# achinastone/Tensorium

Hardware: AMD Instinct MI355X
Metric: fp32 SGEMM GFLOP/s (M=N=K=4096) + YOLOv3 conv-fwd images/s (higher is better)
Workload: dtype fp32; 1 GPU; sgemm_nn_4096x4096x4096; M=4096, N=4096, K=4096, parallelism=1 independent replicas, one process per GPU, no data-path collective

## Files before the change

### include/tns.h

```cpp
#ifndef TNS_H
#define TNS_H

#include <stdint.h>
#include <stddef.h>

#ifdef __cplusplus
extern "C" {
#endif

#define TNS_ABI_VERSION 1

enum { TNS_CblasRowMajor = 101, TNS_CblasColMajor = 102 };
enum { TNS_CblasNoTrans = 111, TNS_CblasTrans = 112 };

enum {
  TNS_acLOGISTIC = 0, TNS_acRELU = 1, TNS_acRELU6 = 2, TNS_acRELIE = 3,
  TNS_acLINEAR = 4, TNS_acRAMP = 5, TNS_acTANH = 6, TNS_acPLSE = 7,
  TNS_acREVLEAKY = 8, TNS_acLEAKY = 9, TNS_acELU = 10, TNS_acLOGGY = 11,
  TNS_acSTAIR = 12, TNS_acHARDTAN = 13, TNS_acLHTAN = 14, TNS_acSELU = 15
};

enum {
  TNS_OK = 0,
  TNS_ERR_ARG = 1,
// ... 128 lines not shown
                       int64_t n, float* biases, float* bias_updates, float* scales,
                       float* scale_updates, float lrOverBatch, float negDecayTimesBatch,
                       float momentum);
int tns_hip_fill(tns_ctx* ctx, int64_t N, float* x, int64_t offset, float val, int64_t stride);
int tns_hip_copy(tns_ctx* ctx, int64_t N, const float* src, int64_t srcOffset, int64_t inca,
                 float* dst, int64_t dstOffset, int64_t incb);
int tns_hip_clamp(tns_ctx* ctx, int64_t N, float alpha, const float* src, float* dst,
                  int64_t stride, int64_t offset);
int tns_hip_addvv(tns_ctx* ctx, int64_t N, const float* src1, int64_t src1Offset, int64_t inca,
                  const float* src2, int64_t src2Offset, int64_t incb, float* dst,
                  int64_t dstOffset, int64_t incc);
int tns_hip_subvv(tns_ctx* ctx, int64_t N, const float* src1, int64_t src1Offset, int64_t inca,
                  const float* src2, int64_t src2Offset, int64_t incb, float* dst,
                  int64_t dstOffset, int64_t incc);
int tns_hip_mulvv(tns_ctx* ctx, int64_t N, const float* src1, int64_t src1Offset, int64_t inca,
                  const float* src2, int64_t src2Offset, int64_t incb, float* dst,
                  int64_t dstOffset, int64_t incc);
int tns_hip_fmavv(tns_ctx* ctx, int64_t N, const float* src1, int64_t src1Offset, int64_t inca,
                  const float* src2, int64_t src2Offset, int64_t incb, const float* src3,
                  int64_t src3Offset, int64_t incc, float* dst, int64_t dstOffset,
                  int64_t incd);
int tns_hip_fmavss(tns_ctx* ctx, int64_t N, const float* src, int64_t offset, float scalar,
                   float bias, float* dst);
int tns_hip_inverse_sqrt(tns_ctx* ctx, int64_t N, float alpha, const float* src, float* dst,
                         int64_t stride, int64_t offset);

int tns_hip_shortcut(tns_ctx* ctx, int64_t N, const float* a, int64_t aOffset, const float* b,
                     int64_t bOffset, float* out, int64_t outOffset, int32_t activation);
int tns_hip_upsample(tns_ctx* ctx, int64_t aBatch, int64_t aChannels, int64_t outHeight,
                     int64_t outWidth, float* in, int64_t stride, int32_t isForward, float scale,
                     float* out, int32_t zeroIn);
int tns_hip_yolo_forward(tns_ctx* ctx, int64_t batch, int64_t anchors, int64_t classes,
                         int64_t hw, const float* in, float* out);
int tns_hip_yolo_loss(tns_ctx* ctx, int64_t batch, int64_t anchors, int64_t classes, int64_t h,
                      int64_t w, int64_t total, const int64_t* mask, const float* biases,
                      int64_t maxBoxes, int64_t netW, int64_t netH, float ignoreThresh,
                      float truthThresh, float iouThresh, float iouNormalizer,
                      float objNormalizer, float* output, const float* truth, float* delta,
                      float* cost, float* stats, int64_t* counters);
int tns_hip_yolo_detections(tns_ctx* ctx, int64_t batch, int64_t anchors, int64_t classes,
                            int64_t h, int64_t w, int64_t total, const int64_t* mask,
                            const float* biases, int64_t netW, int64_t netH, int64_t imW,
                            int64_t imH, float thresh, int32_t relative, int32_t letter,
                            const float* output, int64_t capacity, int64_t* counts, float* boxes,
                            float* objectness, float* probs);
int tns_hip_nms_sort(tns_ctx* ctx, int64_t batch, int64_t capacity, int64_t classes,
                     const int64_t* counts, const float* boxes, const float* objectness,
                     float* probs, float thresh);

int tns_image_bytes_to_input(tns_ctx* ctx, int64_t count, const uint8_t* src, const int64_t* geom,
                             int64_t channels, int64_t pixelStride, int32_t tableKind,
                             const float* table, int64_t netW, int64_t netH, int32_t letter,
                             float* dst, int64_t* placed);
int tns_image_floats_to_input(tns_ctx* ctx, int64_t count, const float* src, const int64_t* geom,
                              int64_t channels, int64_t netW, int64_t netH, int32_t letter,
                              float* dst, int64_t* placed);

int tns_hip_maxpool_forward(tns_ctx* ctx, int64_t aBatch, int64_t outC, int64_t outH,
                            int64_t outW, const float* input, int64_t c, int64_t h, int64_t w,
                            int64_t stride_x, int64_t stride_y, int64_t padding,
                            int64_t kernelSize, int64_t* indexes, float* output);
int tns_hip_maxpool_backward(tns_ctx* ctx, int64_t aBatch, int64_t outC, int64_t outH,
                             int64_t outW, float* output, const int64_t* indexes,
                             const float* delta, int64_t h, int64_t w, int64_t stride_x,
                             int64_t stride_y, int64_t padding, int64_t kernelSize);
int tns_hip_avgpool_forward(tns_ctx* ctx, int64_t aBatch, int64_t outC, int64_t outH,
                            int64_t outW, const float* input, int64_t c, int64_t h, int64_t w,
                            int64_t stride_x, int64_t stride_y, int64_t padding,
                            int64_t kernelSize, float* output);
int tns_hip_avgpool_backward(tns_ctx* ctx, int64_t aBatch, int64_t outC, int64_t outH,
                             int64_t outW, float* output, const float* delta, int64_t h,
                             int64_t w, int64_t stride_x, int64_t stride_y, int64_t padding,
                             int64_t kernelSize);

int tns_hip_dropout_forward(tns_ctx* ctx, int64_t N, int64_t seed, float probability,
                            float scale, const float* src, float* rnd, float* dst);
int tns_hip_dropout_backward(tns_ctx* ctx, int64_t N, float probability, float scale,
                             const float* src, const float* rnd, float* dst);
int tns_hip_cost_l2(tns_ctx* ctx, int64_t N, const float* pred, const float* truth,
                    float* delta, float* error);
int tns_hip_cross_entropy_logistic(tns_ctx* ctx, int64_t N, const float* pred,
                                   const float* truth, float* delta, float* error);

int tns_hip_lstm_gates_forward(tns_ctx* ctx, int64_t N, const float* wf, const float* wi,
                               const float* wg, const float* wo, const float* uf,
                               const float* ui, const float* ug, const float* uo,
                               float* c_state, float* h_state, float* cell_slice,
                               float* out_slice);
int tns_hip_lstm_gates_backward(tns_ctx* ctx, int64_t N, const float* wf, const float* wi,
                                const float* wg, const float* wo, const float* uf,
                                const float* ui, const float* ug, const float* uo,
                                const float* cell_i, const float* cprev, const float* delta_i,
                                float* dc, float* dwf, float* dwi, float* dwg, float* dwo,
                                float* duf, float* dui, float* dug, float* duo);

int tns_hip_rnn_state_forward(tns_ctx* ctx, int64_t N, int64_t H, float* in_slice,
                              const float* in_bias, int32_t in_act, float* self_slice,
                              const float* self_bias, int32_t self_act,
                              const float* state_prev, float* state_next);
int tns_hip_rnn_delta_backward(tns_ctx* ctx, int64_t N, float* delta, const float* out,
                               int32_t act, float* delta2, const float* out2, int32_t act2);

int tns_hip_means_and_vars(tns_ctx* ctx, int64_t srcSize, int64_t dstSize, int64_t groups,
                           const float* src, int64_t offset, float* means, float* vars);
int tns_hip_means(tns_ctx* ctx, int64_t srcSize, int64_t dstSize, int64_t groups,
                  const float* src, int64_t offset, float* means);
int tns_hip_variances(tns_ctx* ctx, int64_t srcSize, int64_t dstSize, int64_t groups,
                      const float* src, int64_t offset, const float* means, float* vars);
int tns_hip_normalize(tns_ctx* ctx, int64_t srcSize, int64_t dstSize, int64_t groups,
                      const float* means, int64_t meansStride, const float* vars,
                      int64_t varsStride, float* dst, int64_t dstOffset);
int tns_hip_forward_scale(tns_ctx* ctx, int64_t dstSize, float* dst, int64_t offset,
                          int64_t scaleSize, const float* scale, int64_t incb, int64_t batch);
int tns_hip_forward_scale_add(tns_ctx* ctx, int64_t dstSize, float* dst, int64_t offset,
                              int64_t scaleSize, const float* scales, const float* biases,
                              int64_t incb, int64_t batch);
int tns_hip_means_and_vars_delta(tns_ctx* ctx, int64_t srcSize, int64_t dstSize, int64_t groups,
                                 const float* delta, const float* x, int64_t offset,
                                 const float* mean, const float* variance, float* mean_delta,
                                 float* variance_delta);
int tns_hip_normalize_delta(tns_ctx* ctx, int64_t deltaSize, int64_t meanSize, int64_t groups,
                            float* delta, const float* x, int64_t offset, const float* mean,
                            const float* variance, const float* mean_delta,
                            const float* variance_delta);
int tns_hip_add_dots(tns_ctx* ctx, int64_t N, int64_t dstSize, int64_t groups,
                     const float* src1, const float* src2, int64_t srcOffset, float* dst);
int tns_hip_softmax_batch(tns_ctx* ctx, int64_t N, const float* input, int64_t iOffset,
                          int64_t batch, int64_t batch_size, int64_t groups, int64_t group_size,
                          int64_t stride, float temp, float* output, int64_t oOffset);
int tns_hip_cross_entropy_softmax(tns_ctx* ctx, int64_t N, const float* pred, const float* truth,
                                  float* delta, float* error);
int tns_hip_sum(tns_ctx* ctx, int64_t N, const float* src, int64_t offset, float* out);

int64_t tns_mlp_buffer_floats(int32_t nlayers, const int64_t* widths, int32_t bn, int64_t batch);
int tns_hip_mlp_train_step(tns_ctx* ctx, int32_t nlayers, const int64_t* widths,
                           const int32_t* acts, int32_t bn, int64_t batch, const float* X,
                           const float* truth, float learningRate, float momentum, float decay,
                           float* buf, float* cost);


int tns_hip_conv2d(tns_ctx* ctx, int64_t batch, int64_t C, int64_t H, int64_t W,
                   const float* input, const float* weights, int64_t filters,
                   int64_t kH, int64_t kW, int64_t wPadding, int64_t hPadding,
                   int64_t xStride, int64_t yStride, int64_t xDilation, int64_t yDilation,
                   float* workspace, float* out);

enum { TNS_CONV_UNFUSED = 0, TNS_CONV_FUSED = 1, TNS_CONV_IM2COL = 2, TNS_CONV_IMPLICIT = 3 };
int tns_hip_conv_forward(tns_ctx* ctx, int64_t batch, int64_t C, int64_t H, int64_t W,
                         const float* input, const float* weights, const float* biases,
                         int64_t filters, int64_t kSize, int64_t stride, int64_t padding,
                         int64_t dilation, int32_t activation, float* workspace,
                         float* out, int32_t fused);

int tns_hip_conv_forward_train(tns_ctx* ctx, int64_t batch, int64_t C, int64_t H, int64_t W,
                               const float* input, const float* weights, int64_t filters,
                               int64_t kSize, int64_t stride, int64_t padding, int64_t dilation,
                               int32_t activation, const float* scales, const float* biases,
                               float* rolling_mean, float* rolling_variance, float bnMomentum,
                               int32_t training, float* mean, float* variance, float* x,
                               float* x_norm, float* workspace, float* out);

int tns_hip_conv_backward(tns_ctx* ctx, int64_t batch, int64_t C, int64_t H, int64_t W,
                          const float* input, const float* weights, int64_t filters,
                          int64_t kSize, int64_t stride, int64_t padding, int64_t dilation,
                          int32_t activation, const float* output, float* delta,
                          float* bias_updates, float* weight_updates, float* workspace,
                          float* state_delta);
int tns_hip_conv_backward_bn(tns_ctx* ctx, int64_t batch, int64_t C, int64_t H, int64_t W,
                             const float* input, const float* weights, int64_t filters,
                             int64_t kSize, int64_t stride, int64_t padding, int64_t dilation,
                             int32_t activation, const float* output, float* delta,
                             const float* scales, const float* x, const float* x_norm,
                             const float* mean, const float* variance, float* scale_updates,
                             float* mean_delta, float* variance_delta, float* weight_updates,
                             float* workspace, float* state_delta);

int tns_hip_sgemm_strided_batched_multi(const int32_t* devices, int32_t n, uint8_t transA,
                                        uint8_t transB, int64_t M, int64_t N, int64_t K,
                                        float alpha, const float* A, int64_t lda,
                                        int64_t strideA, const float* B, int64_t ldb,
                                        int64_t strideB, float beta, float* C, int64_t ldc,
                                        int64_t strideC, int64_t batchCount);
int tns_set_op_devices(const int32_t* devices, int32_t n);

int    tns_hip_set_telemetry(tns_ctx* ctx, int32_t enable);
double tns_hip_op_ms(tns_ctx* ctx, int32_t op);
enum { TNS_OP_GEMM = 0, TNS_OP_IM2COL = 1, TNS_OP_COL2IM = 2, TNS_OP_BIAS = 3,
       TNS_OP_ACTIVATE = 4, TNS_OP_COUNT = 5 };

int         tns_gemm_variant_count(void);
int         tns_conv_dx_tile_count(void);
int         tns_conv_dx_conv_count(void);
int         tns_conv_dw_res_count(void);
int         tns_conv_dw_tile_count(void);
int         tns_conv_tile_variant_count(void);
const char* tns_conv_tile_variant_name(int32_t variant);
int         tns_conv_slab_count(void);
const char* tns_conv_slab_name(int32_t variant);
int         tns_conv1x1_count(void);
const char* tns_conv1x1_name(int32_t variant);
int         tns_sdot_chains_variant_count(void);
const char* tns_sdot_chains_variant_name(int32_t variant);
int         tns_sdot_rc_variant_count(void);
const char* tns_sdot_rc_variant_name(int32_t variant);
const char* tns_gemm_variant_name(int32_t variant);
int tns_hip_gemm_variant(tns_ctx* ctx, int32_t variant, uint8_t transA, uint8_t transB,
                         int64_t M, int64_t N, int64_t K, float ALPHA,
                         const float* A, int64_t aOffset, int64_t lda, int64_t strideA,
                         const float* B, int64_t bOffset, int64_t ldb, int64_t strideB,
                         float BETA, float* C, int64_t cOffset, int64_t ldc, int64_t strideC,
                         int64_t batchCount);
enum { TNS_GP_TRANS_A = 0, TNS_GP_TRANS_B = 1, TNS_GP_M = 2, TNS_GP_N = 3, TNS_GP_K = 4,
       TNS_GP_LDA = 5, TNS_GP_LDB = 6, TNS_GP_LDC = 7, TNS_GP_STRIDE_A = 8, TNS_GP_STRIDE_B = 9,
       TNS_GP_STRIDE_C = 10, TNS_GP_BATCH = 11, TNS_GP_ALPHA_IS_ONE = 12, TNS_GP_BETA_MODE = 13,
       TNS_GP_EPI = 14, TNS_GP_A_ALIGNED16 = 15, TNS_GP_B_ALIGNED16 = 16, TNS_GP_NT_SDOT = 17,
       TNS_GP_TT_EXACT = 18, TNS_GP_SDOT_FORM = 19, TNS_GP_COUNT = 20 };
int         tns_gemm_plan(int32_t variant, const int64_t* in, char* out, int64_t out_len);
int         tns_gemm_plan_leaf_count(void);
const char* tns_gemm_plan_leaf_name(int32_t leaf);

enum { TNS_OPT_STRICT_BETA0 = 0, TNS_OPT_CONV_VARIANT = 1, TNS_OPT_CONV_PAD = 2,
       TNS_OPT_NT_SDOT = 3, TNS_OPT_SRSS_QUIRK = 4, TNS_OPT_TT_EXACT = 5,
       TNS_OPT_SDOT_FORM = 6, TNS_OPT_DX_FUSED = 7, TNS_OPT_DX_TILE = 8,
       TNS_OPT_DW_TILE = 9, TNS_OPT_BWD_OVERLAP = 10, TNS_OPT_DX_CONV = 11,
       TNS_OPT_DW_RES = 12, TNS_OPT_DERIVE_SUMS = 13, TNS_OPT_SCRATCH_CAP = 14 };
int tns_set_option(int32_t opt, int64_t value);

#ifdef __cplusplus
}
#endif
#endif
```

### tensorium_amd/_abi.py

```python
from __future__ import annotations

import ctypes as C
import os
import re
from pathlib import Path

PKG = Path(__file__).resolve().parent
ROOT = PKG.parent
LIB_PATH = PKG / "libtensorium_hip.so"
HEADER = ROOT / "include" / "tns.h"

i32, i64, u8, f32 = C.c_int32, C.c_int64, C.c_uint8, C.c_float
fptr = C.c_void_p
vp = C.c_void_p

CblasRowMajor, CblasColMajor = 101, 102
CblasNoTrans, CblasTrans = 111, 112
ACT = dict(LOGISTIC=0, RELU=1, RELU6=2, RELIE=3, LINEAR=4, RAMP=5, TANH=6, PLSE=7,
           REVLEAKY=8, LEAKY=9, ELU=10, LOGGY=11, STAIR=12, HARDTAN=13, LHTAN=14, SELU=15)
TNS_OK = 0
TNS_OP_GEMM, TNS_OP_IM2COL, TNS_OP_COL2IM, TNS_OP_BIAS, TNS_OP_ACTIVATE = range(5)
TNS_OPT_STRICT_BETA0 = 0
TNS_OPT_CONV_VARIANT, TNS_OPT_CONV_PAD, TNS_OPT_NT_SDOT, TNS_OPT_SRSS_QUIRK = 1, 2, 3, 4
TNS_OPT_TT_EXACT = 5
TNS_OPT_SDOT_FORM = 6
TNS_OPT_DX_FUSED = 7
TNS_OPT_DX_TILE = 8
TNS_OPT_DW_TILE = 9
TNS_OPT_BWD_OVERLAP = 10
TNS_OPT_DX_CONV = 11
TNS_OPT_DW_RES = 12
TNS_OPT_DERIVE_SUMS = 13
TNS_OPT_SCRATCH_CAP = 14

_CONV = [i64] * 11

PROTOTYPES: dict[str, tuple] = {
    "tns_abi_version": (C.c_int, []),
    "tns_last_error": (C.c_char_p, []),
    "tns_clear_error": (None, []),
    "tns_set_error_hook": (None, [vp]),
    "tns_device_count": (C.c_int, []),
    "tns_set_option": (C.c_int, [i32, i64]),
    "tns_cblas_sgemm": (None, [i32, i32, i32, i64, i64, i64, f32, fptr, i64, fptr, i64, f32,
                               fptr, i64]),
    "tns_cblas_sgemm_batch_strided": (None, [i32, i32, i32, i64, i64, i64, f32, fptr, i64, i64,
                                             fptr, i64, i64, f32, fptr, i64, i64, i64]),
    "tns_im2col": (None, [*_CONV, fptr, i64, fptr, i64, u8]),
    "tns_col2im": (None, [*_CONV, fptr, i64, fptr, i64, i64, u8]),
    "tns_im2col_strided_batched": (None, [*_CONV, fptr, i64, i64, fptr, i64, i64, i64]),
    "tns_col2im_strided_batched": (None, [*_CONV, fptr, i64, i64, fptr, i64, i64, i64]),
    "tns_hip_create": (C.c_int, [i32, C.POINTER(vp)]),
    "tns_hip_destroy": (C.c_int, [vp]),
    "tns_hip_set_stream": (C.c_int, [vp, vp]),
    "tns_hip_get_stream": (vp, [vp]),
    "tns_hip_pending_dw": (C.c_int, [vp]),
    "tns_hip_finish": (C.c_int, [vp]),
    "tns_hip_malloc": (C.c_int, [vp, i64, C.POINTER(vp)]),
    "tns_hip_free": (C.c_int, [vp, vp]),
    "tns_hip_write_buffer": (C.c_int, [vp, fptr, i64, vp]),
    "tns_hip_read_buffer": (C.c_int, [vp, fptr, i64, vp]),
    "tns_hip_gemm": (C.c_int, [vp, u8, u8, i64, i64, i64, f32, fptr, i64, i64, fptr, i64, i64,
                               f32, fptr, i64, i64]),
    "tns_hip_gemm_strided_batched": (C.c_int, [vp, u8, u8, i64, i64, i64, f32, fptr, i64, i64,
                                               i64, fptr, i64, i64, i64, f32, fptr, i64, i64,
                                               i64, i64]),
    "tns_hip_im2col": (C.c_int, [vp, *_CONV, fptr, i64, fptr, i64]),
    "tns_hip_im2col_strided_batched": (C.c_int, [vp, *_CONV, fptr, i64, i64, fptr, i64, i64,
                                                 i64]),
    "tns_hip_col2im": (C.c_int, [vp, *_CONV, fptr, i64, fptr, i64]),
    "tns_hip_col2im_strided_batched": (C.c_int, [vp, *_CONV, fptr, i64, i64, fptr, i64, i64,
                                                 i64]),
    "tns_hip_forward_bias": (C.c_int, [vp, i64, fptr, i64, i64, fptr, i64, i64]),
    "tns_hip_backward_bias": (C.c_int, [vp, i64, fptr, i64, fptr, i64, i64, i64]),
    "tns_hip_activate_array": (C.c_int, [vp, i64, fptr, i64, i32]),
    "tns_hip_derive_array": (C.c_int, [vp, i64, fptr, i64, i32, fptr]),
    "tns_hip_axpy": (C.c_int, [vp, i64, f32, fptr, i64, i64, fptr, i64, i64]),
    "tns_hip_sgd_update": (C.c_int, [vp, i64, fptr, fptr, i64, fptr, fptr, fptr, fptr, f32, f32,
                                     f32]),
    "tns_hip_scale": (C.c_int, [vp, i64, f32, fptr, i64]),
    "tns_hip_fill": (C.c_int, [vp, i64, fptr, i64, f32, i64]),
    "tns_hip_copy": (C.c_int, [vp, i64, fptr, i64, i64, fptr, i64, i64]),
    "tns_hip_clamp": (C.c_int, [vp, i64, f32, fptr, fptr, i64, i64]),
    "tns_hip_conv2d": (C.c_int, [vp, i64, i64, i64, i64, fptr, fptr, i64, i64, i64, i64, i64,
                                 i64, i64, i64, i64, fptr, fptr]),
    "tns_hip_conv_forward": (C.c_int, [vp, i64, i64, i64, i64, fptr, fptr, fptr, i64, i64, i64,
                                       i64, i64, i32, fptr, fptr, i32]),
    "tns_hip_conv_backward": (C.c_int, [vp, i64, i64, i64, i64, fptr, fptr, i64, i64, i64, i64,
                                        i64, i32, fptr, fptr, fptr, fptr, fptr, fptr]),
    "tns_hip_conv_forward_train": (C.c_int, [vp, i64, i64, i64, i64, fptr, fptr, i64, i64, i64,
                                             i64, i64, i32, fptr, fptr, fptr, fptr, f32, i32,
                                             fptr, fptr, fptr, fptr, fptr, fptr]),
    "tns_hip_conv_backward_bn": (C.c_int, [vp, i64, i64, i64, i64, fptr, fptr, i64, i64, i64,
                                           i64, i64, i32, fptr, fptr, fptr, fptr, fptr, fptr,
                                           fptr, fptr, fptr, fptr, fptr, fptr, fptr]),
    "tns_hip_set_telemetry": (C.c_int, [vp, i32]),
    "tns_gemm_variant_count": (C.c_int, []),
    "tns_sdot_chains_variant_count": (C.c_int, []),
    "tns_sdot_rc_variant_count": (C.c_int, []),
    "tns_conv_tile_variant_count": (C.c_int, []),
    "tns_conv_dx_tile_count": (C.c_int, []),
    "tns_conv_dx_conv_count": (C.c_int, []),
    "tns_conv_dw_res_count": (C.c_int, []),
    "tns_conv_dw_tile_count": (C.c_int, []),
    "tns_conv_tile_variant_name": (C.c_char_p, [C.c_int32]),
    "tns_conv_slab_count": (C.c_int, []),
    "tns_conv1x1_count": (C.c_int, []),
    "tns_conv1x1_name": (C.c_char_p, [C.c_int32]),
    "tns_conv_slab_name": (C.c_char_p, [C.c_int32]),
    "tns_sdot_chains_variant_name": (C.c_char_p, [C.c_int32]),
    "tns_sdot_rc_variant_name": (C.c_char_p, [C.c_int32]),
    "tns_gemm_variant_name": (C.c_char_p, [i32]),
    "tns_hip_gemm_variant": (C.c_int, [vp, i32, u8, u8, i64, i64, i64, f32, fptr, i64, i64, i64,
                                       fptr, i64, i64, i64, f32, fptr, i64, i64, i64, i64]),
    "tns_hip_op_ms": (C.c_double, [vp, i32]),
    "tns_gemm_plan": (C.c_int, [i32, C.POINTER(i64), C.c_char_p, i64]),
    "tns_gemm_plan_leaf_count": (C.c_int, []),
    "tns_gemm_plan_leaf_name": (C.c_char_p, [i32]),
}


class TnsError(RuntimeError):
    pass


_lib = None


def header_symbols() -> list[str]:
    text = HEADER.read_text()
    text = re.sub(r"/\*.*?\*/", "", text, flags=re.S)
    names = re.findall(r"\b(tns_[a-z0-9_]+)\s*\(", text)
    seen: list[str] = []
    for n in names:
        if n not in seen and not n.endswith("_t"):
            seen.append(n)
    return seen


def load(path: str | os.PathLike | None = None) -> C.CDLL:
    global _lib
    if _lib is not None and path is None:
        return _lib
    p = Path(path) if path else Path(os.environ.get("TNS_LIB") or LIB_PATH)
    if not p.exists():
        raise TnsError(f"{p} not built — run `python -m tensorium_amd.build` "
                       "(the HIP backend has no CPU fallback)")
    lib = C.CDLL(str(p), mode=C.RTLD_GLOBAL)
    older = bool(os.environ.get("TNS_LIB")) and path is None
    for name, (res, args) in PROTOTYPES.items():
        if older and not hasattr(lib, name):
            continue
        fn = getattr(lib, name)
        fn.restype = res
        fn.argtypes = args
    if path is None:
        _lib = lib
    return lib


GEMM_PLAN_FIELDS = ("transA", "transB", "M", "N", "K", "lda", "ldb", "ldc", "strideA", "strideB",
                    "strideC", "batch", "alpha1", "beta_mode", "epi", "a16", "b16", "nt_sdot",
                    "tt_exact", "sdot_form")
_GEMM_PLAN_DEFAULTS = dict(strideA=0, strideB=0, strideC=0, batch=1, alpha1=1, beta_mode=2, epi=0,
                           a16=1, b16=1, nt_sdot=1, tt_exact=1, sdot_form=-1)


def gemm_plan(variant: int = -1, **shape) -> dict:
    import json
    v = dict(_GEMM_PLAN_DEFAULTS, **shape)
    v.setdefault("lda", v["M"] if v["transA"] else v["K"])
    v.setdefault("ldb", v["K"] if v["transB"] else v["N"])
    v.setdefault("ldc", v["N"])
    arr = (i64 * len(GEMM_PLAN_FIELDS))(*(int(v[k]) for k in GEMM_PLAN_FIELDS))
    buf = C.create_string_buffer(1024)
    check(load().tns_gemm_plan(int(variant), arr, buf, len(buf)))
    return json.loads(buf.value.decode())


def check(rc: int) -> None:
    if rc != TNS_OK:
        lib = load()
        msg = lib.tns_last_error().decode(errors="replace")
        lib.tns_clear_error()
        raise TnsError(f"tns status {rc}: {msg}")


PROTOTYPES.update({
    "tns_hip_shortcut": (C.c_int, [vp, i64, fptr, i64, fptr, i64, fptr, i64, i32]),
    "tns_hip_upsample": (C.c_int, [vp, i64, i64, i64, i64, fptr, i64, i32, f32, fptr, i32]),
    "tns_hip_addvv": (C.c_int, [vp, i64, fptr, i64, i64, fptr, i64, i64, fptr, i64, i64]),
    "tns_hip_subvv": (C.c_int, [vp, i64, fptr, i64, i64, fptr, i64, i64, fptr, i64, i64]),
    "tns_hip_mulvv": (C.c_int, [vp, i64, fptr, i64, i64, fptr, i64, i64, fptr, i64, i64]),
    "tns_hip_fmavv": (C.c_int, [vp, i64, fptr, i64, i64, fptr, i64, i64, fptr, i64, i64, fptr,
                                i64, i64]),
    "tns_hip_fmavss": (C.c_int, [vp, i64, fptr, i64, f32, f32, fptr]),
    "tns_hip_inverse_sqrt": (C.c_int, [vp, i64, f32, fptr, fptr, i64, i64]),
    "tns_hip_sgemm_strided_batched_multi": (C.c_int, [C.POINTER(i32), i32, u8, u8, i64, i64, i64,
                                                      f32, fptr, i64, i64, fptr, i64, i64, f32,
                                                      fptr, i64, i64, i64]),
    "tns_set_op_devices": (C.c_int, [C.POINTER(i32), i32]),
    "tns_hip_yolo_forward": (C.c_int, [vp, i64, i64, i64, i64, fptr, fptr]),
    "tns_hip_yolo_loss": (C.c_int, [vp, i64, i64, i64, i64, i64, i64, C.POINTER(i64),
                                    C.POINTER(f32), i64, i64, i64, f32, f32, f32, f32, f32, fptr,
                                    fptr, fptr, fptr, fptr, vp]),
    "tns_hip_yolo_detections": (C.c_int, [vp, i64, i64, i64, i64, i64, i64, C.POINTER(i64),
                                          C.POINTER(f32), i64, i64, i64, i64, f32, i32, i32, fptr,
                                          i64, vp, fptr, fptr, fptr]),
    "tns_hip_nms_sort": (C.c_int, [vp, i64, i64, i64, vp, fptr, fptr, fptr, f32]),
    "tns_image_bytes_to_input": (C.c_int, [vp, i64, vp, C.POINTER(i64), i64, i64, i32,
                                           C.POINTER(f32), i64, i64, i32, fptr, C.POINTER(i64)]),
    "tns_image_floats_to_input": (C.c_int, [vp, i64, fptr, C.POINTER(i64), i64, i64, i64, i32,
                                            fptr, C.POINTER(i64)]),
    "tns_hip_maxpool_forward": (C.c_int, [vp, i64, i64, i64, i64, fptr, i64, i64, i64, i64, i64,
                                          i64, i64, vp, fptr]),
    "tns_hip_maxpool_backward": (C.c_int, [vp, i64, i64, i64, i64, fptr, vp, fptr, i64, i64, i64,
                                           i64, i64, i64]),
    "tns_hip_avgpool_forward": (C.c_int, [vp, i64, i64, i64, i64, fptr, i64, i64, i64, i64, i64,
                                          i64, i64, fptr]),
    "tns_hip_avgpool_backward": (C.c_int, [vp, i64, i64, i64, i64, fptr, fptr, i64, i64, i64,
                                           i64, i64, i64]),
    "tns_hip_dropout_forward": (C.c_int, [vp, i64, i64, f32, f32, fptr, fptr, fptr]),
    "tns_hip_dropout_backward": (C.c_int, [vp, i64, f32, f32, fptr, fptr, fptr]),
    "tns_hip_cost_l2": (C.c_int, [vp, i64, fptr, fptr, fptr, fptr]),
    "tns_hip_cross_entropy_logistic": (C.c_int, [vp, i64, fptr, fptr, fptr, fptr]),
    "tns_hip_lstm_gates_forward": (C.c_int, [vp, i64] + [fptr] * 12),
    "tns_hip_lstm_gates_backward": (C.c_int, [vp, i64] + [fptr] * 20),
    "tns_hip_rnn_state_forward": (C.c_int, [vp, i64, i64, fptr, fptr, i32, fptr, fptr, i32, fptr,
                                            fptr]),
    "tns_hip_rnn_delta_backward": (C.c_int, [vp, i64, fptr, fptr, i32, fptr, fptr, i32]),
    "tns_hip_means_and_vars": (C.c_int, [vp, i64, i64, i64, fptr, i64, fptr, fptr]),
    "tns_hip_means": (C.c_int, [vp, i64, i64, i64, fptr, i64, fptr]),
    "tns_hip_variances": (C.c_int, [vp, i64, i64, i64, fptr, i64, fptr, fptr]),
    "tns_hip_gemm_batched": (C.c_int, [vp, u8, u8, i64, i64, i64, f32, vp, i64, i64, vp, i64, i64,
                                       f32, vp, i64, i64, i64]),
    "tns_hip_normalize": (C.c_int, [vp, i64, i64, i64, fptr, i64, fptr, i64, fptr, i64]),
    "tns_hip_forward_scale": (C.c_int, [vp, i64, fptr, i64, i64, fptr, i64, i64]),
    "tns_hip_forward_scale_add": (C.c_int, [vp, i64, fptr, i64, i64, fptr, fptr, i64, i64]),
    "tns_hip_means_and_vars_delta": (C.c_int, [vp, i64, i64, i64, fptr, fptr, i64, fptr, fptr,
                                               fptr, fptr]),
# ... 12 lines not shown
```

### tensorium_amd/csrc/conv_api.cpp

```cpp
#include <algorithm>
#include <cstdarg>
#include <cstdio>

#include "tns_ctx.hpp"

using namespace tns;

namespace tns {
namespace {
template <class Plan>
Plan& refuse(Plan& p, int code, const char* fmt, ...) {
  va_list ap;
  va_start(ap, fmt);
  vsnprintf(p.msg, sizeof p.msg, fmt, ap);
  va_end(ap);
  p.err = code;
  return p;
}

int64_t images_per_launch(int64_t img, int64_t outImg) {
  return std::max<int64_t>(
      1, std::min<int64_t>(0x7fffffffLL / (4 * img), 0x7fffffffLL / std::max<int64_t>(outImg, 1)));
}

DwArgs dw_tile_args(const ConvBwdPlan& p, const float* delta, const float* input) {
  const ConvShape& s = p.s;
  DwArgs da{};
  da.delta = delta; da.x = input; da.part = nullptr;
  da.M = (int)p.i_m; da.N = (int)p.i_n; da.HW = (int)p.i_k;
  da.C = (int)s.C; da.H = (int)s.H; da.W = (int)s.W; da.oW = (int)p.g.ow;
  da.stride = (int)s.stride; da.pad = (int)(s.padding * s.dilation); da.dil = (int)s.dilation;
  da.va = p.i_k % 4 == 0 && p.delta_aligned16;
  da.alpha = 1.0f;
  da.strideA = p.i_m * p.i_k; da.strideX = s.C * s.H * s.W; da.strideP = p.i_m * p.i_n;
  da.batch = s.batch;
  return da;
}
}

ConvFwdPlan plan_conv_forward(const ConvShape& s, int fused, bool bias_act, const Options& o) {
  ConvFwdPlan p;
  const int64_t batch = s.batch, C = s.C, H = s.H, W = s.W, filters = s.filters, kSize = s.kSize,
                stride = s.stride, padding = s.padding, dilation = s.dilation;
  p.s = s;
  p.oh = out_dim(H, padding, kSize, dilation, stride);
  p.ow = out_dim(W, padding, kSize, dilation, stride);
  p.bias_act = bias_act;
  p.conv_variant = o.conv_variant;
  p.srss_quirk = (int)o.srss_quirk;
  const bool transc = act_transcendental(s.activation);
  p.epi_act = transc ? 4 : s.activation;
  p.act_tail = bias_act && transc;
  if (!fused) {
    p.path = FWD_UNFUSED;
    return p;
  }
  if (fused < TNS_CONV_UNFUSED || fused > TNS_CONV_IMPLICIT)
    return refuse(p, TNS_ERR_ARG, "conv_forward: unknown schedule %d", fused);
  if (const char* m = geom_error(geom(C, H, W, kSize, kSize, padding, padding, stride, stride,
                                      dilation, dilation)))
    return refuse(p, TNS_ERR_ARG, "%s", m);
  const int64_t outImg = p.oh * p.ow, k = C * kSize * kSize, N = batch * outImg;
  if (p.oh <= 0 || p.ow <= 0 || batch <= 0) return p;
  p.needs_col = kSize != 1 || dilation != 1 || stride != 1;
  const bool direct_ok = p.needs_col || padding == 0;
  const int64_t Hpad = H + 2 * padding, Wpad = W + 2 * padding;
  const bool fits = !(k > 0x0fffffffLL - KTAB_PAD || C * Hpad * Wpad * 4 > 0x7fffffffLL ||
                      (kSize - 1) * dilation >= 0x8000);
  if (!(direct_ok && (fused == TNS_CONV_IMPLICIT || (fused == TNS_CONV_FUSED && fits)))) {
    p.path = FWD_IM2COL;
    if (p.needs_col) p.col_elems = batch * k * outImg;
    return p;
  }
  p.implicit = true;
  const int64_t cvar = o.conv_variant;
  if (cvar >= 200 && cvar < 500)
    return refuse(p, TNS_ERR_UNSUPPORTED,
                  "conv variant %lld: the ping-pong, LDS-DMA-ring and input-patch tile "
                  "families (200..499) were removed",
                  (long long)cvar);
  if (cvar < 0 && conv_direct_applies(C, kSize, filters)) {
    p.path = FWD_DIRECT;
    return p;
  }
  if (kSize == 1 && stride == 1 && padding == 0 && dilation == 1) {
    const int cv = cvar >= 600 ? (int)(cvar - 600)
                   : cvar < 0  ? conv1x1_pick(filters, N, k, outImg)
                               : -1;
    if (cv >= 0) {
      p.path = FWD_CONV1X1;
      p.form = cv;
      return p;
    }
  } else if (cvar >= 600) {
    return refuse(p, TNS_ERR_UNSUPPORTED, "conv1x1 forms need a 1x1 stride-1 unpadded layer");
  }
  const int sv = cvar >= 500 && cvar < 600    ? (int)(cvar - 500)
                 : cvar < 0 && dilation == 1 ? conv_slab_pick(filters, N, k, kSize)
                                              : -1;
  if (sv >= 0) {
    p.col_elems = conv_slab_floats(sv, N, k);
    if (p.col_elems < 0) return refuse(p, TNS_ERR_ARG, "no conv slab form %d", sv);
    p.path = FWD_SLAB;
    p.form = sv;
    return p;
  }
  const int64_t img0 = C * H * W;
  if ((kSize == 1 || kSize == 3) && k % 32 == 0 && img0 * 4 <= 0x7fffffffLL) {
    int tv = -1;
    if (cvar >= 100) {
      tv = (int)(cvar - 100);
    } else if (cvar < 0) {
      GemmArgs probe{};
      probe.M = filters; probe.N = N; probe.K = k;
      probe.conv_sY = (int)stride;
      probe.A = reinterpret_cast<const float*>(uintptr_t(s.weights_aligned16 ? 16 : 4));
      probe.lda = k;
      tv = conv_tile_pick(probe, (int)kSize);
    }
    if (tv >= 0) {
      p.path = FWD_TILE;
      p.form = tv;
      p.chunk = images_per_launch(img0, outImg);
      return p;
    }
  }
  const double flops = 2.0 * (double)filters * (double)N * (double)k;
  p.padded = padding == 0 ||
             (o.conv_pad < 0 ? 8.0 * (double)(batch * C * Hpad * Wpad) * 400.0 < flops
                             : o.conv_pad == 1);
  const int64_t img = p.padded ? C * Hpad * Wpad : img0;
  if (k > 0x0fffffffLL - KTAB_PAD || img * 4 > 0x7fffffffLL || (kSize - 1) * dilation >= 0x8000)
    return refuse(p, TNS_ERR_ARG, "conv_forward: image too large for the implicit GEMM");
  p.path = FWD_IMPLICIT;
  p.form = cvar == 99 ? -1 : (int)cvar;
  if (p.padded && padding > 0) p.stage1_elems = batch * img;
  p.chunk = images_per_launch(img, outImg);
  return p;
}

ConvBwdPlan plan_conv_backward(const ConvShape& s, bool has_bn, bool has_state_delta,
                               bool delta_aligned16, const Options& o) {
  ConvBwdPlan p;
  const int64_t batch = s.batch, C = s.C, H = s.H, W = s.W, filters = s.filters, kSize = s.kSize,
                stride = s.stride, padding = s.padding, dilation = s.dilation;
  p.s = s;
  p.has_bn = has_bn; p.has_state_delta = has_state_delta; p.delta_aligned16 = delta_aligned16;
  p.srss_quirk = (int)o.srss_quirk;
  p.sched = o.bwd_overlap == 2 ? BWD_PIPELINED : o.bwd_overlap ? BWD_JOINED : BWD_SEQUENTIAL;
  const ConvGeom g = p.g = geom(C, H, W, kSize, kSize, padding * dilation, padding * dilation,
                                stride, stride, dilation, dilation);
  if (const char* m = geom_error(g)) return refuse(p, TNS_ERR_ARG, "%s", m);
  const int64_t lh = (H + 2 * padding - kSize) / stride + 1;
  const int64_t lw = (W + 2 * padding - kSize) / stride + 1;
  if (g.oh != lh || g.ow != lw)
    return refuse(p, TNS_ERR_UNSUPPORTED,
                  "conv_backward: dilation %lld with padding %lld gives %lldx%lld im2col "
                  "columns but the layer's output is %lldx%lld (nConvolutionLayer.pas:92-100, "
                  "640)",
                  (long long)dilation, (long long)padding, (long long)g.oh, (long long)g.ow,
                  (long long)lh, (long long)lw);
  const int64_t i_m = p.i_m = filters, i_n = p.i_n = kSize * kSize * C, i_k = p.i_k = g.oh * g.ow;
  p.colSize = i_n * i_k;
  if (batch <= 0 || i_k <= 0 || filters <= 0) return p;
  p.empty = false;
  p.bn_elems = 3 * batch * filters;
  p.bn_fused = has_bn && o.bn_fused;
  p.derive_sums = !has_bn && o.derive_sums;
  const bool needs_col = p.needs_col = kSize != 1 || stride != 1 || padding != 0 || dilation != 1;
  const int dx1 = has_state_delta && o.dx_c1 && o.dx_fused != 2 && !needs_col
                      ? conv1x1_pick(C, batch * i_k, filters, i_k)
                      : -1;
  const bool fused_dx =
      dx1 < 0 && has_state_delta && dilation == 1 &&
      ((o.dx_fused == 1 && conv_dx_fused_applies(C, H, W, kSize, stride, filters, g.oh, g.ow)) ||
       (o.dx_fused == 2 && conv_dx_fused_fits(C, H, W, stride, filters, g.oh, g.ow)));
  int dwv = -1;
  if (o.nt_sdot && o.dw_tile != -2 && (kSize == 1 || kSize == 3) && C * H * W < (1LL << 27) &&
      i_n <= 0x7fffffffLL && i_k <= 0x7fffffffLL && batch <= 65535)
    dwv = o.dw_tile >= 0 ? (int)o.dw_tile
                         : dw_tile_pick(dw_tile_args(p, nullptr, nullptr), (int)kSize);
  ConvDwChoice& fb = p.dw_fallback;
  fb.path = dwv >= 0 ? DW_TILE : o.nt_sdot && batch > 1 ? DW_SDOT : DW_GEMM;
  fb.form = dwv;
  fb.col = needs_col && dwv < 0;
  fb.part_elems = fb.path == DW_GEMM ? 0 : batch * i_m * i_n;
  p.dw = fb;
  int dwr = -1;
  if (o.nt_sdot && o.dw_res != -2 && o.dw_tile < 0 && batch <= 65535 && i_k >= 64) {
    if (o.dw_res >= 0)
      dwr = (int)o.dw_res;
    else if (kSize == 3)
      dwr = dw_res_pick(i_m, i_n, i_k, batch);
  }
  if (dwr >= 0) {
    const int64_t rowlen = 8 * dw_res_k4(i_k);
    p.dw = ConvDwChoice{DW_RES, dwr, false,
                        std::max<int64_t>(1, batch * dw_res_groups(dwr) * i_m * i_n)};
    p.dw_res_forced = o.dw_res >= 0;
    p.res_a_elems = batch * i_m * rowlen + 32;
    p.res_b_elems = batch * dw_res_b_rows(dwr, i_n) * rowlen + 32;
  }
  if (has_state_delta) {
    p.dx_direct = !needs_col && !fused_dx;
    int dxc = -1;
    if (!fused_dx && kSize == 3 && (stride == 1 || stride == 2) && dilation == 1 &&
        o.dx_conv != -2)
      dxc = o.dx_conv >= 0 ? (int)o.dx_conv
            : stride == 2  ? conv_tile4_dx3s2_pick(batch, C, H, W, filters, kSize, padding)
                           : conv_tile4_dx3_pick(batch, C, H, W, filters, kSize, padding);
    p.dx_col = !fused_dx && !p.dx_direct && dxc < 0;
    if (fused_dx) {
      p.dx = DX_FUSED;
    } else if (dxc >= 0) {
      p.dx = stride == 2 ? DX_CONV3S2 : DX_CONV3;
      p.dx_form = dxc;
    } else {
      if (o.dx_tile != -2)
        p.dx_tile = o.dx_tile >= 0 ? (int)o.dx_tile
                                   : conv_tile4_dx_pick(i_n, batch * i_k, i_m, kSize);
      p.dx_tile_forced = o.dx_tile >= 0;
      p.dx = dx1 >= 0 ? DX_CONV1X1 : p.dx_tile >= 0 ? DX_TILE : DX_TN;
      p.dx_form = dx1 >= 0 ? dx1 : p.dx_tile;
    }
    if (fused_dx || dxc >= 0 || dx1 >= 0) p.wt_elems = filters * C * kSize * kSize;
  }
  if (p.dw.col || fb.col || p.dx_col) p.col_elems = batch * p.colSize;
  return p;
}

}

int tns_hip_conv2d(tns_ctx* c, int64_t batch, int64_t C, int64_t H, int64_t W,
                   const float* input, const float* weights, int64_t filters, int64_t kH,
                   int64_t kW, int64_t wPadding, int64_t hPadding, int64_t xStride,
                   int64_t yStride, int64_t xDilation, int64_t yDilation, float* workspace,
                   float* out) {
  if (int r = check_ctx(c)) return r;
  if (wPadding < 0) wPadding = xDilation + kW / 2 - 1;
  if (hPadding < 0) hPadding = yDilation + kH / 2 - 1;
  ConvGeom g = geom(C, H, W, kH, kW, hPadding, wPadding, yStride, xStride, xDilation, yDilation);
  if (int r = check_geom(g)) return r;
  const int64_t oh = out_dim(H, hPadding, kH, yDilation, yStride);
  const int64_t ow = out_dim(W, wPadding, kW, xDilation, xStride);
  const int64_t outImg = oh * ow, kSize = kH * kW, k = C * kSize;
  if (g.oh != oh || g.ow != ow)
    return set_error(TNS_ERR_UNSUPPORTED,
                     "conv2d: xDilation %lld, yDilation %lld give %lldx%lld im2col columns but "
                     "the layer's output is %lldx%lld (ntensors.pas:8303)",
                     (long long)xDilation, (long long)yDilation, (long long)g.oh,
                     (long long)g.ow, (long long)oh, (long long)ow);
  if (oh <= 0 || ow <= 0 || batch <= 0) return TNS_OK;
  const float* Bp;
  int64_t strideB;
  if (kSize != 1 || xDilation * yDilation != 1 || xStride * yStride != 1) {
    strideB = k * outImg;
    float* ws = workspace;
    if (!ws)
      if (int r = ensure_scratch(c, SLOT_COL, batch * strideB, &ws)) return r;
    {
      OpTimer t(c, TNS_OP_IM2COL);
      if (int r = hip_status(launch_im2col(g, input, C * H * W, ws, strideB, batch, c->stream),
                             "im2col launch"))
        return r;
    }
    Bp = ws;
  } else {
    strideB = C * H * W;
    Bp = input;
  }
  return do_gemm(c, false, false, filters, outImg, k, 1.0f, weights, k, 0, Bp, outImg, strideB,
                 0.0f, out, outImg, outImg * filters, batch, EPI_NONE, nullptr, 0, true);
}

namespace {
struct ConvFwdOps {
  const float *input, *weights, *biases;
  float *workspace, *out;
};

int activate_tail(tns_ctx* c, const ConvFwdPlan& p, const ConvFwdOps& o) {
  if (!p.act_tail) return TNS_OK;
  OpTimer t(c, TNS_OP_ACTIVATE);
  return hip_status(launch_activate(o.out, p.s.batch * p.s.filters * p.oh * p.ow, p.s.activation,
                                    c->stream),
                    "activate launch");
}

GemmArgs conv_args(const ConvFwdPlan& p, const ConvFwdOps& o, const float* src, int64_t img,
                   int64_t Hs, int64_t Ws, int mode, const int* kt, int64_t pad, int64_t b0,
                   int64_t nb) {
  const int64_t outImg = p.oh * p.ow, k = p.s.C * p.s.kSize * p.s.kSize;
  GemmArgs a{};
  a.M = p.s.filters; a.N = nb * outImg; a.K = k;
  a.alpha = 1.0f; a.beta = 0.0f; a.beta_mode = BETA_ZERO;
  a.A = o.weights; a.lda = k; a.strideA = 0;
  a.B = src + b0 * img; a.ldb = outImg; a.strideB = img;
  a.C = o.out + b0 * outImg * p.s.filters; a.ldc = outImg; a.strideC = outImg * p.s.filters;
  a.batch = 1; a.epi = p.bias_act ? EPI_BIAS_ACT : EPI_NONE; a.bias = o.biases;
  a.act = p.epi_act;
  a.conv = mode; a.ktab = kt; a.ktab_n = kt ? (int)(k + KTAB_PAD) : 0;
  a.conv_H = (int)Hs; a.conv_W = (int)Ws; a.conv_ow = (int)p.ow; a.conv_ohw = (int)outImg;
  a.conv_sY = (int)p.s.stride; a.conv_sX = (int)p.s.stride;
  a.conv_pH = (int)pad; a.conv_pW = (int)pad;
  a.conv_bytes = (int)(4 * nb * img);
  return a;
}

int run_fwd_unfused(tns_ctx* c, const ConvFwdPlan& p, const ConvFwdOps& o) {
  const ConvShape& s = p.s;
  if (int r = tns_hip_conv2d(c, s.batch, s.C, s.H, s.W, o.input, o.weights, s.filters, s.kSize,
                             s.kSize, s.padding, s.padding, s.stride, s.stride, s.dilation,
                             s.dilation, o.workspace, o.out))
    return r;
  if (!p.bias_act) return TNS_OK;
  OpTimer t(c, TNS_OP_BIAS);
  return hip_status(launch_bias_activate(o.out, s.filters, p.oh * p.ow, o.biases, s.batch,
                                         s.activation, c->stream),
                    "bias+activate launch");
}

int run_fwd_direct(tns_ctx* c, const ConvFwdPlan& p, const ConvFwdOps& o) {
  const ConvShape& s = p.s;
  OpTimer t(c, TNS_OP_GEMM);
  return hip_status(launch_conv_direct(o.input, o.weights, o.biases, o.out, s.batch, s.C, s.H, s.W,
                                       s.filters, s.kSize, s.stride, s.padding, s.dilation, p.oh,
                                       p.ow, s.activation, c->stream),
                    "direct conv launch");
}

int run_fwd_conv1x1(tns_ctx* c, const ConvFwdPlan& p, const ConvFwdOps& o) {
  {
    OpTimer t(c, TNS_OP_GEMM);
    const hipError_t e = launch_conv1x1(p.form, o.weights, o.input, o.biases, o.out, p.s.batch,
                                        p.s.filters, p.s.C, p.oh * p.ow, p.epi_act, c->stream);
    if (e == hipErrorInvalidValue)
      return set_error(TNS_ERR_UNSUPPORTED, "conv1x1 form %d does not fit this layer", p.form);
    if (int r = hip_status(e, "conv1x1 launch")) return r;
  }
  return activate_tail(c, p, o);
}

int run_fwd_slab(tns_ctx* c, const ConvFwdPlan& p, const ConvFwdOps& o) {
  const ConvShape& s = p.s;
  float* slab = nullptr;
  if (int r = ensure_scratch(c, SLOT_COL, p.col_elems, &slab)) return r;
  ConvSlabArgs sa{};
  sa.input = o.input; sa.weights = o.weights; sa.bias = o.biases; sa.out = o.out;
  sa.batch = s.batch; sa.C = s.C; sa.H = s.H; sa.W = s.W; sa.M = s.filters;
  sa.K = s.C * s.kSize * s.kSize; sa.ks = s.kSize;
  sa.stride = s.stride; sa.pad = s.padding; sa.dil = s.dilation; sa.ow = p.ow; sa.ohw = p.oh * p.ow;
  sa.act = p.epi_act;
  {
    OpTimer t(c, TNS_OP_GEMM);
    const hipError_t e = launch_conv_slab(p.form, sa, slab, c->stream);
    if (e == hipErrorInvalidValue)
      return set_error(TNS_ERR_UNSUPPORTED, "conv slab form %d does not fit this layer", p.form);
    if (int r = hip_status(e, "conv slab launch")) return r;
  }
  return activate_tail(c, p, o);
}

int run_fwd_tile(tns_ctx* c, const ConvFwdPlan& p, const ConvFwdOps& o) {
  const ConvShape& s = p.s;
  for (int64_t b0 = 0; b0 < s.batch; b0 += p.chunk) {
    const GemmArgs a = conv_args(p, o, o.input, s.C * s.H * s.W, s.H, s.W, 2, nullptr, s.padding,
                                 b0, std::min(p.chunk, s.batch - b0));
    OpTimer t(c, TNS_OP_GEMM);
    const hipError_t e = launch_conv_tile(p.form, a, (int)s.kSize, (int)s.dilation, c->stream);
    if (e == hipErrorInvalidValue)
      return set_error(TNS_ERR_UNSUPPORTED, "conv tile %d does not fit this layer", p.form);
    if (int r = hip_status(e, "conv tile launch")) return r;
  }
  return activate_tail(c, p, o);
}

int run_fwd_implicit(tns_ctx* c, const ConvFwdPlan& p, const ConvFwdOps& o) {
  const ConvShape& s = p.s;
  const int64_t border = p.padded ? 2 * s.padding : 0;
  const int64_t Hs = s.H + border, Ws = s.W + border, img = s.C * Hs * Ws;
  const int* kt = nullptr;
  if (int r = get_ktab(c, s.C, Hs, Ws, s.kSize, s.kSize, s.dilation, s.dilation, &kt)) return r;
  const float* src = o.input;
  if (p.stage1_elems) {
    float* pbuf = nullptr;
    if (int r = ensure_scratch(c, SLOT_STAGE1, p.stage1_elems, &pbuf)) return r;
    OpTimer t(c, TNS_OP_IM2COL);
    if (int r = hip_status(launch_pad_images(o.input, s.batch, s.C, s.H, s.W, s.padding, s.padding,
                                             pbuf, c->stream), "pad launch"))
      return r;
    src = pbuf;
  }
  for (int64_t b0 = 0; b0 < s.batch; b0 += p.chunk) {
    const GemmArgs a = conv_args(p, o, src, img, Hs, Ws, p.padded ? 1 : 2, kt,
                                 p.padded ? 0 : s.padding, b0, std::min(p.chunk, s.batch - b0));
    OpTimer t(c, TNS_OP_GEMM);
    hipError_t e = launch_sgemm_conv_variant(p.form, a, c->stream);
    if (e == hipErrorInvalidValue)
      return set_error(TNS_ERR_UNSUPPORTED, "conv variant %lld unsupported",
                       (long long)p.conv_variant);
    if (int r = hip_status(e, "implicit conv launch")) return r;
  }
  return activate_tail(c, p, o);
}

int run_fwd_im2col(tns_ctx* c, const ConvFwdPlan& p, const ConvFwdOps& o) {
  const ConvShape& s = p.s;
  const int64_t outImg = p.oh * p.ow, k = s.C * s.kSize * s.kSize;
  const float* Bp = o.input;
  int64_t strideB = s.C * s.H * s.W;
  if (p.needs_col) {
    strideB = k * outImg;
    float* ws = o.workspace;
    if (!ws)
      if (int r = ensure_scratch(c, SLOT_COL, p.col_elems, &ws)) return r;
    OpTimer t(c, TNS_OP_IM2COL);
    const ConvGeom g = geom(s.C, s.H, s.W, s.kSize, s.kSize, s.padding, s.padding, s.stride,
                            s.stride, s.dilation, s.dilation);
    if (int r = hip_status(launch_im2col(g, o.input, s.C * s.H * s.W, ws, strideB, s.batch,
                                         c->stream), "im2col launch"))
      return r;
    Bp = ws;
  }
  if (int r = do_gemm(c, false, false, s.filters, outImg, k, 1.0f, o.weights, k, 0, Bp, outImg,
                      strideB, 0.0f, o.out, outImg, outImg * s.filters, s.batch,
                      p.bias_act ? EPI_BIAS_ACT : EPI_NONE, o.biases, p.epi_act, true))
    return r;
  return activate_tail(c, p, o);
}

int exec_conv_forward(tns_ctx* c, const ConvFwdPlan& p, const ConvFwdOps& o) {
  if (p.path == FWD_UNFUSED) return run_fwd_unfused(c, p, o);
  if (p.err && !p.implicit) return set_error(p.err, "%s", p.msg);
  if (p.implicit && (!o.input || !o.weights || !o.out || (p.bias_act && !o.biases)))
    return set_error(TNS_ERR_ARG, "conv_forward: null operand");
  if (p.err) return set_error(p.err, "%s", p.msg);
  switch (p.path) {
    case FWD_IM2COL: return run_fwd_im2col(c, p, o);
    case FWD_DIRECT: return run_fwd_direct(c, p, o);
    case FWD_CONV1X1: return run_fwd_conv1x1(c, p, o);
    case FWD_SLAB: return run_fwd_slab(c, p, o);
    case FWD_TILE: return run_fwd_tile(c, p, o);
    case FWD_IMPLICIT: return run_fwd_implicit(c, p, o);
    default: return TNS_OK;
  }
}

bool aligned16(const void* p) { return (reinterpret_cast<uintptr_t>(p) & 15) == 0; }
}

int tns_hip_conv_forward(tns_ctx* c, int64_t batch, int64_t C, int64_t H, int64_t W,
                         const float* input, const float* weights, const float* biases,
                         int64_t filters, int64_t kSize, int64_t stride, int64_t padding,
                         int64_t dilation, int32_t activation, float* workspace, float* out,
                         int32_t fused) {
  if (int r = check_ctx(c)) return r;
  if (!act_supported(activation))
    return set_error(TNS_ERR_UNSUPPORTED, "activation %d not implemented", activation);
  const ConvShape s{batch, C, H, W, filters, kSize, stride, padding, dilation, activation,
                    aligned16(weights)};
  return exec_conv_forward(c, plan_conv_forward(s, fused, true, g_opt),
                           ConvFwdOps{input, weights, biases, workspace, out});
}

int tns_hip_conv_forward_train(tns_ctx* c, int64_t batch, int64_t C, int64_t H, int64_t W,
                               const float* input, const float* weights, int64_t filters,
                               int64_t kSize, int64_t stride, int64_t padding, int64_t dilation,
                               int32_t activation, const float* scales, const float* biases,
                               float* rolling_mean, float* rolling_variance, float bnMomentum,
                               int32_t training, float* mean, float* variance, float* x,
                               float* x_norm, float* workspace, float* out) {
  if (int r = check_ctx(c)) return r;
  if (!act_supported(activation))
    return set_error(TNS_ERR_UNSUPPORTED, "activation %d not implemented", activation);
  if (!scales || !biases || !rolling_mean || !rolling_variance || !out ||
      (training && (!mean || !variance || !x || !x_norm)))
    return set_error(TNS_ERR_ARG, "conv_forward_train: null operand");
  const int64_t oh = out_dim(H, padding, kSize, dilation, stride);
  const int64_t ow = out_dim(W, padding, kSize, dilation, stride);
  if (oh <= 0 || ow <= 0 || batch <= 0 || filters <= 0) return TNS_OK;
  const int64_t bs = oh * ow;
  const ConvShape s{batch, C, H, W, filters, kSize, stride, padding, dilation, activation,
                    aligned16(weights)};
  const ConvFwdPlan p = plan_conv_forward(s, TNS_CONV_FUSED, false, g_opt);
  if (int r = exec_conv_forward(c, p, ConvFwdOps{input, weights, nullptr, workspace, out}))
    return r;
  OpTimer t(c, TNS_OP_BIAS);
  if (!training)
    return hip_status(launch_bn_apply(out, nullptr, nullptr, out, batch, filters, bs,
                                      rolling_mean, rolling_variance, scales, biases, activation,
                                      c->stream),
                      "batchNorm launch");
  float* part;
  if (int r = ensure_scratch(c, SLOT_BN, 2 * batch * filters, &part)) return r;
  if (int r = hip_status(launch_means_vars(out, batch, filters, bs, mean, variance, p.srss_quirk,
                                           part, c->stream),
                         "meansAndVars launch"))
    return r;
  if (int r = hip_status(launch_rolling_update(filters, rolling_mean, rolling_variance, mean,
                                               variance, bnMomentum, c->stream),
                         "rolling update launch"))
    return r;
  return hip_status(launch_bn_apply(out, x, x_norm, out, batch, filters, bs, mean, variance,
                                    scales, biases, activation, c->stream),
                    "batchNorm launch");
}

namespace {
struct ConvBN {
  const float *scales, *x, *x_norm, *mean, *variance;
  float *scale_updates, *mean_delta, *variance_delta;
};
struct ConvBwdOps {
  const float *input, *weights, *output;
  float *delta, *bias_updates, *weight_updates, *workspace, *state_delta;
  ConvBN bn;
};
struct ConvBwdRun {
  bool pipe = false, overlap = false;
  const ConvDwChoice* dw = nullptr;
  DwResArgs dres{};
  float* part = nullptr;
  float* ws = nullptr;
  float* dx_ws = nullptr;
  float* wt = nullptr;
};

int run_bwd_prologue(tns_ctx* c, const ConvBwdPlan& p, const ConvBwdOps& o, float* part) {
  const ConvBN& bn = o.bn;
  const int64_t batch = p.s.batch, filters = p.s.filters, i_k = p.i_k;
  const int act = p.s.activation;
  float* delta = o.delta;
  hipError_t fe = hipErrorNotSupported;
  if (p.bn_fused)
    fe = launch_bn_backward_fused(bn.scale_updates, bn.x_norm, delta, o.output, act, bn.x, bn.mean,
                                  bn.variance, bn.scales, bn.mean_delta, bn.variance_delta, batch,
                                  filters, i_k, p.srss_quirk, part, c->stream);
  if (fe != hipErrorNotSupported) return hip_status(fe, "batchNormBack launch");
  if (p.has_bn) {
    if (int r = hip_status(launch_add_dots_derive(bn.scale_updates, bn.x_norm, delta, o.output, act,
                                                  batch, filters, i_k, part, c->stream),
                           "derive + addDots launch"))
      return r;
    const float* fold = bn_folds_scale(i_k) ? bn.scales : nullptr;
    if (!fold)
      if (int r = hip_status(launch_scale_add(delta, batch, filters, i_k, bn.scales, nullptr, 1,
                                              c->stream), "forwardScale launch"))
        return r;
    if (int r = hip_status(launch_mean_var_delta(delta, bn.x, bn.mean, bn.variance, batch, filters,
                                                 i_k, bn.mean_delta, bn.variance_delta,
                                                 p.srss_quirk, part, c->stream, fold),
                           "meansAndVarsDelta launch"))
      return r;
    return hip_status(launch_normalize_delta(bn.x, bn.mean, bn.variance, bn.mean_delta,
                                             bn.variance_delta, delta, batch, filters, i_k,
                                             c->stream, fold), "normalizeDelta launch");
  }
  if (p.derive_sums)
    return hip_status(launch_derive_add_sums(o.bias_updates, delta, o.output, act, batch, filters,
                                             i_k, part, c->stream),
                      "derive + addSums launch");
  if (int r = hip_status(launch_derive(o.output, batch * filters * i_k, act, delta, c->stream),
                         "derive launch"))
    return r;
  return hip_status(launch_add_sums(o.bias_updates, delta, batch, filters, i_k, part, c->stream),
                    "addSums launch");
}

int acquire_bwd_scratch(tns_ctx* c, const ConvBwdPlan& p, const ConvBwdOps& o, ConvBwdRun& r) {
  r.dw = &p.dw;
  if (p.dw.path == DW_RES) {
    int e = ensure_scratch(c, SLOT_RES_A, p.res_a_elems, &r.dres.dA, r.pipe);
    if (!e) e = ensure_scratch(c, SLOT_RES_B, p.res_b_elems, &r.dres.dB, r.pipe);
    if (!e) e = ensure_scratch(c, SLOT_DW, p.dw.part_elems, &r.dres.part, r.pipe);
    if (e) {
      if (p.dw_res_forced) return e;
      tns_clear_error();
      release_scratch(c, SLOT_RES_A);
      release_scratch(c, SLOT_RES_B);
      r.dw = &p.dw_fallback;
    }
  }
  r.overlap = !r.pipe && p.has_state_delta && p.sched != BWD_SEQUENTIAL && !c->telemetry &&
              ensure_side_stream(c);
  if (r.overlap && r.dw->col && p.dx_col &&
      ensure_scratch(c, SLOT_COL_DX, p.col_elems, &r.dx_ws)) {
    tns_clear_error();
    r.overlap = false;
  }
  if (r.pipe && p.dx_col && ensure_scratch(c, SLOT_COL_DX, p.col_elems, &r.dx_ws)) {
    tns_clear_error();
    r.dx_ws = nullptr;
    r.pipe = false;
    if (int e = join_side(c)) return e;
  }
  r.ws = o.workspace;
  if (!r.ws && (r.dw->col || (p.dx_col && !r.dx_ws && !(r.overlap && r.dw->col))))
    if (int e = ensure_scratch(c, SLOT_COL, p.col_elems, &r.ws, r.pipe)) return e;
  if (!r.dx_ws) r.dx_ws = r.ws;
  if (p.wt_elems)
    if (int e = ensure_scratch(c, SLOT_WT, p.wt_elems, &r.wt)) return e;
  return TNS_OK;
}

int run_dw(tns_ctx* c, const ConvBwdPlan& p, const ConvBwdOps& o, const ConvBwdRun& r) {
  const ConvShape& s = p.s;
  const int64_t batch = s.batch, i_m = p.i_m, i_n = p.i_n, i_k = p.i_k;
  const ConvDwChoice& dw = *r.dw;
  if (dw.path == DW_RES) {
    DwResArgs d = r.dres;
    d.g = p.g;
    d.x = o.input; d.xStride = s.C * s.H * s.W;
    d.delta = o.delta; d.weight_updates = o.weight_updates;
    d.M = i_m; d.N = i_n; d.K = i_k; d.batch = batch;
    d.direct = !p.needs_col; d.alpha = 1.0f;
// ... 237 lines not shown
```

### tensorium_amd/csrc/conv_slab.hip

```cpp
#include <algorithm>
#include <type_traits>

#include "tns_act.hpp"
#include "tns_internal.hpp"

namespace tns {
namespace {

typedef float floatx4 __attribute__((ext_vector_type(4)));

__device__ __forceinline__ void slab_dma16(const float* sbase, unsigned voff, unsigned lds) {
  unsigned keep;
  asm volatile(
      "s_mov_b32 %0, m0\n\ts_mov_b32 m0, %3\n\ts_nop 0\n\t"
      "global_load_lds_dwordx4 %1, %2\n\ts_mov_b32 m0, %0"
      : "=&s"(keep)
      : "v"(voff), "s"(sbase), "s"(lds)
      : "memory");
}

struct SlabFillArgs {
  const float* x;
  int64_t strideX;
  float* slab;
// ... 14 lines not shown
__global__ __launch_bounds__(256) void slab_fill_kernel(SlabFillArgs a) {
  constexpr int NG = BK / 16, KK = KS * KS;
  const int64_t x = (int64_t)blockIdx.x * 256 + threadIdx.x;
  if (x >= a.units) return;
  const int c = (int)(x % BN);
  const int64_t r1 = x / BN;
  const int g = (int)(r1 % NG);
  const int64_t r2 = r1 / NG;
  const int t = (int)(r2 % a.KT), ct = (int)(r2 / a.KT);
  const int n = ct * BN + c;
  float v[16];
  const __amdgpu_buffer_rsrc_t rsrc =
      __builtin_amdgcn_make_buffer_rsrc(const_cast<float*>(a.x), 0, a.bytes, 0x00020000);
  {
    const int nn = n < a.N ? n : a.N - 1;
    const int img = slab_div(nn, a.ohw, a.inv_ohw), pix = nn - img * a.ohw;
    const int oy = slab_div(pix, a.ow, a.inv_ow), ox = pix - oy * a.ow;
    const int iy0 = oy * a.stride - a.pad, ix0 = ox * a.stride - a.pad;
    const int HW = a.H * a.W;
    unsigned mask = 0;
    int toff[KK];
#pragma unroll
    for (int kr = 0; kr < KS; ++kr)
#pragma unroll
      for (int kc = 0; kc < KS; ++kc) {
        const int iy = iy0 + kr * a.dil, ix = ix0 + kc * a.dil;
        mask |= (unsigned)(((unsigned)iy < (unsigned)a.H) & ((unsigned)ix < (unsigned)a.W))
                << (kr * KS + kc);
        toff[kr * KS + kc] = 4 * (kr * a.dil * a.W + kc * a.dil);
      }
    if (n >= a.N) mask = 0;
    const unsigned base = 4u * (unsigned)(img * (int)a.strideX + iy0 * a.W + ix0);
    const int k0 = t * BK + 16 * g;
    int ch = k0 / KK, tap = k0 - ch * KK;
#pragma unroll
    for (int e = 0; e < 16; ++e) {
      int off = toff[0];
#pragma unroll
      for (int u = 1; u < KK; ++u) off = tap == u ? toff[u] : off;
      const unsigned o = ((mask >> tap) & 1u) ? base + 4u * (unsigned)(ch * HW) + (unsigned)off
                                              : 0x80000000u;
      v[e] = __builtin_bit_cast(float, __builtin_amdgcn_raw_buffer_load_b32(rsrc, o, 0, 0));
      if (++tap == KK) {
        tap = 0;
        ++ch;
      }
    }
  }
  float* dst = a.slab + ((r2 * NG + g) * 4 * BN + c) * 4;
#pragma unroll
  for (int q = 0; q < 4; ++q)
    *reinterpret_cast<floatx4*>(dst + q * BN * 4) = floatx4{v[q], v[4 + q], v[8 + q], v[12 + q]};
}

template <int KS, int BK, int BN>
__global__ __launch_bounds__((BN + 63) / 64 * 64) void slab_fill_u_kernel(SlabFillArgs a) {
  constexpr int NG = BK / 16, KK = KS * KS;
  const int c = threadIdx.x;
  if (c >= BN) return;
  const int64_t r1 = blockIdx.x;
  const int g = (int)(r1 % NG);
  const int64_t r2 = r1 / NG;
  const int t = (int)(r2 % a.KT), ct = (int)(r2 / a.KT);
  const int n = ct * BN + c;
  float v[16];
  const __amdgpu_buffer_rsrc_t rsrc =
      __builtin_amdgcn_make_buffer_rsrc(const_cast<float*>(a.x), 0, a.bytes, 0x00020000);
  {
    const int nn = n < a.N ? n : a.N - 1;
    const int img = slab_div(nn, a.ohw, a.inv_ohw), pix = nn - img * a.ohw;
    const int oy = slab_div(pix, a.ow, a.inv_ow), ox = pix - oy * a.ow;
    const int iy0 = oy * a.stride - a.pad, ix0 = ox * a.stride - a.pad;
    const int HW = a.H * a.W;
    unsigned mask = 0;
#pragma unroll
    for (int kr = 0; kr < KS; ++kr)
#pragma unroll
      for (int kc = 0; kc < KS; ++kc) {
        const int iy = iy0 + kr * a.dil, ix = ix0 + kc * a.dil;
        mask |= (unsigned)(((unsigned)iy < (unsigned)a.H) & ((unsigned)ix < (unsigned)a.W))
                << (kr * KS + kc);
      }
    if (n >= a.N) mask = 0;
    const unsigned base = 4u * (unsigned)(img * (int)a.strideX + iy0 * a.W + ix0);
    const int k0 = __builtin_amdgcn_readfirstlane(t * BK + 16 * g);
    int ch = k0 / KK, tap = k0 - ch * KK;
    int kr = tap / KS, kc = tap - kr * KS;
#pragma unroll
    for (int e = 0; e < 16; ++e) {
      const unsigned uoff = 4u * (unsigned)(ch * HW + kr * a.dil * a.W + kc * a.dil);
      const unsigned o = ((mask >> tap) & 1u) ? base + uoff : 0x80000000u;
      v[e] = __builtin_bit_cast(float, __builtin_amdgcn_raw_buffer_load_b32(rsrc, o, 0, 0));
      ++tap;
      if (++kc == KS) {
        kc = 0;
        ++kr;
      }
      if (tap == KK) {
        tap = 0;
        kr = 0;
        ++ch;
      }
    }
  }
  float* dst = a.slab + ((r2 * NG + g) * 4 * BN + c) * 4;
#pragma unroll
  for (int q = 0; q < 4; ++q)
    *reinterpret_cast<floatx4*>(dst + q * BN * 4) = floatx4{v[q], v[4 + q], v[8 + q], v[12 + q]};
}

struct SlabGemmArgs {
  const float* A;
  const float* slab;
  float* C;
  const float* bias;
  int M, N, K, KT, tiles_m, ohw, act;
  bool fuse;
};

template <int BM_, int BN_, int BK_, int WM_, int WN_, int JA_, int NA_, int NS_, int DG_ = 0,
          int MAP_ = 0>
struct SG {
  static constexpr int BM = BM_, BN = BN_, BK = BK_, WM = WM_, WN = WN_, JA = JA_, NA = NA_;
  static constexpr int NS = NS_;
  static constexpr int DG = DG_, MAP = MAP_;
  static constexpr int NW = WM * WN, NT = 64 * NW, J = BN / 16, NG = BK / 16, ROWS = BK / 4;
  static constexpr int JB = NA < WN ? (J - NA * JA) / (WN - NA) : 0;
  static constexpr int A_TILE = ROWS * BM * 4, B_TILE = ROWS * BN * 4, STAGE = A_TILE + B_TILE;
  static constexpr int AU = BM * BK / 4 / NT;
  static constexpr int BDMA = 4 * BK * BN / 1024;
  static constexpr int DPW = (BDMA + NW - 1) / NW;
  static_assert(BM == 16 * WM && BN % 16 == 0 && BK % 16 == 0, "geometry");
  static_assert(NA * JA + (WN - NA) * JB == J && NA >= 1 && NA <= WN, "wave column split");
  static_assert(AU >= 1 && BM * BK / 4 % NT == 0, "A units");
  static_assert(4 * BK * BN % 1024 == 0, "whole DMA instructions");
  static_assert(NS >= 2 && NS * STAGE * 4 <= 163840, "LDS");
  static_assert(NG >= 2 && NG % 2 == 0, "groups: f0 holds group 0 at every tile start");
  static_assert(DPW * (NS - 2) <= 63 && DPW <= 63, "vmcnt immediates");
};

template <int JW>
struct SFrag {
  floatx4 a, b[JW];
};

template <int N>
__device__ __forceinline__ void wait_vm(bool keep_n) {
  if (keep_n)
    asm volatile("s_waitcnt vmcnt(%0)" ::"n"(N) : "memory");
  else
    asm volatile("s_waitcnt vmcnt(0)" ::: "memory");
}

template <class G>
__global__ __launch_bounds__(G::NT, 1) void slab_gemm_kernel(SlabGemmArgs p) {
  constexpr int BM = G::BM, BN = G::BN, BK = G::BK, NG = G::NG, NS = G::NS;
  constexpr int A_TILE = G::A_TILE, STAGE = G::STAGE, AU = G::AU, DPW = G::DPW;
  __shared__ __attribute__((aligned(16))) float smem[NS * STAGE];
  const int tid = threadIdx.x, lane = tid & 63;
  const int w = __builtin_amdgcn_readfirstlane(tid >> 6), wm = w % G::WM, wn = w / G::WM;
  const int r16 = lane & 15, q = lane >> 4;
  int tm, tn;
  {
    const int nb = gridDim.x, bid = blockIdx.x;
    const int xcd = bid & 7, qq = nb >> 3, rr = nb & 7;
    const int wg = (xcd < rr ? xcd * (qq + 1) : rr * (qq + 1) + (xcd - rr) * qq) + (bid >> 3);
    if constexpr (G::MAP == 1) {
      const int tiles_n = (p.N + BN - 1) / BN;
      tn = wg % tiles_n;
      tm = wg / tiles_n;
    } else {
      tm = wg % p.tiles_m;
      tn = wg / p.tiles_m;
    }
  }
  const int m0 = tm * BM, n0 = tn * BN;
  const int N = p.N, K = p.K, nt = p.KT;
  const float* slabT = p.slab + (int64_t)tn * K * BN;
  const unsigned lds0 = (unsigned)(uintptr_t)(__attribute__((address_space(3))) float*)smem;
  const unsigned voff = 16u * (unsigned)lane;
  auto dma_b = [&](int t, int st, int v) {
    if constexpr (G::DG & 1) return;
    int u = w + G::NW * v;
    if (G::BDMA % G::NW != 0 && u >= G::BDMA) u -= G::NW;
    slab_dma16(slabT + (int64_t)t * (BK * BN) + 256 * u, voff,
               lds0 + 4u * (unsigned)(st * STAGE + A_TILE) + 1024u * (unsigned)u);
  };
  auto dma_all = [&](int t, int st) {
#pragma unroll
    for (int v = 0; v < DPW; ++v) dma_b(t, st, v);
  };
  unsigned a_off[AU];
  int a_dst[AU];
#pragma unroll
  for (int u = 0; u < AU; ++u) {
    const int idx = tid + G::NT * u;
    const int lo = idx & 7, rest = idx >> 3;
    const int m = rest % BM, kq4 = lo + 8 * (rest / BM);
    a_off[u] = 4u * (unsigned)(m * K + 4 * kq4);
    a_dst[u] = (4 * (kq4 >> 2)) * BM * 4 + m * 4 + (kq4 & 3);
  }
  const float* a_row0 = p.A + (int64_t)m0 * K;
  floatx4 ra[AU];
  auto load_a = [&](int t) {
    if constexpr (G::DG & 2) return;
    const float* sb = a_row0 + t * BK;
#pragma unroll
    for (int u = 0; u < AU; ++u)
      asm volatile("global_load_dwordx4 %0, %1, %2" : "=v"(ra[u]) : "v"(a_off[u]), "s"(sb) : "memory");
  };
  auto store_a = [&](int st) {
    if constexpr (G::DG & 2) return;
    float* as = smem + st * STAGE;
#pragma unroll
    for (int u = 0; u < AU; ++u) {
      asm volatile("" : "+v"(ra[u]));
      as[a_dst[u]] = ra[u][0];
      as[a_dst[u] + BM * 4] = ra[u][1];
      as[a_dst[u] + 2 * BM * 4] = ra[u][2];
      as[a_dst[u] + 3 * BM * 4] = ra[u][3];
    }
  };

  auto run = [&](auto JWC, const int coff) {
    constexpr int JW = decltype(JWC)::value;
    floatx4 acc[JW];
#pragma unroll
    for (int j = 0; j < JW; ++j) acc[j] = floatx4{0.f, 0.f, 0.f, 0.f};
    using Frag = SFrag<JW>;
    auto frag = [&](int st, int g, Frag& f) {
      const float* ap = smem + st * STAGE + ((4 * g + q) * BM + wm * 16 + r16) * 4;
      f.a = *reinterpret_cast<const floatx4*>(ap);
      const float* bp = smem + st * STAGE + A_TILE + ((4 * g + q) * BN + coff * 16 + r16) * 4;
#pragma unroll
      for (int j = 0; j < JW; ++j) f.b[j] = *reinterpret_cast<const floatx4*>(bp + 64 * j);
    };
    auto mma = [&](const Frag& f) {
#pragma unroll
      for (int i = 0; i < 4; ++i)
#pragma unroll
        for (int j = 0; j < JW; ++j)
          acc[j] = __builtin_amdgcn_mfma_f32_16x16x4f32(f.a[i], f.b[j][i], acc[j], 0, 0, 0);
    };
    auto mma_dma = [&](const Frag& f, int tb, int st) {
      constexpr int NM = 4 * JW, STEP = NM / DPW > 0 ? NM / DPW : 1;
#pragma unroll
      for (int x = 0; x < NM; ++x) {
        const int i = x / JW, j = x % JW;
        acc[j] = __builtin_amdgcn_mfma_f32_16x16x4f32(f.a[i], f.b[j][i], acc[j], 0, 0, 0);
        if (x % STEP == 0 && x / STEP < DPW) dma_b(tb, st, x / STEP);
        __builtin_amdgcn_sched_barrier(0);
      }
      if constexpr (NM / STEP < DPW) {
#pragma unroll
        for (int v = NM / STEP; v < DPW; ++v) dma_b(tb, st, v);
      }
    };

    Frag f0, f1;
    load_a(0);
#pragma unroll
    for (int t = 0; t < NS; ++t) {
      if (t == 1 && nt > 1) {
        wait_vm<0>(false);
        store_a(0);
        load_a(1);
      }
      if (t < nt) dma_all(t, t);
    }
    if (nt == 1) {
      wait_vm<0>(false);
      store_a(0);
    } else {
      if (nt >= NS)
        asm volatile("s_waitcnt vmcnt(%0)" ::"n"(AU + (NS - 1) * DPW) : "memory");
      else
        wait_vm<0>(false);
    }
    __syncthreads();
    frag(0, 0, f0);
    for (int t = 0; t < nt; ++t) {
      const int cur = t % NS;
#pragma unroll
      for (int g = 0; g + 1 < NG; ++g) {
        Frag& fc = (g & 1) ? f1 : f0;
        Frag& fn = (g & 1) ? f0 : f1;
        frag(cur, g + 1, fn);
        __builtin_amdgcn_sched_barrier(0);
        mma(fc);
        __builtin_amdgcn_sched_barrier(0);
      }
      if (t + 1 < nt) {
        const int nxt = (t + 1) % NS;
        if constexpr (NS == 2)
          wait_vm<0>(false);
        else
          wait_vm<DPW>(t + NS - 1 < nt);
        store_a(nxt);
        if constexpr (!(G::DG & 4))
          __syncthreads();
        frag(nxt, 0, f0);
        if (t + 2 < nt) load_a(t + 2);
        __builtin_amdgcn_sched_barrier(0);
        if (t + NS < nt)
          mma_dma(f1, t + NS, cur);
        else
          mma(f1);
      } else {
        mma(f1);
      }
    }

    const int row0 = m0 + wm * 16 + 4 * q;
    float bias[4];
#pragma unroll
    for (int e = 0; e < 4; ++e) bias[e] = p.fuse ? p.bias[row0 + e] : 0.0f;
#pragma unroll
    for (int j = 0; j < JW; ++j) {
      const int n = n0 + coff * 16 + 16 * j + r16;
      if (n >= N) continue;
      const int img = n / p.ohw, pix = n - img * p.ohw;
      float* cp = p.C + ((int64_t)img * p.M + row0) * p.ohw + pix;
#pragma unroll
      for (int e = 0; e < 4; ++e) {
        float v = acc[j][e];
        if (p.fuse) v = act_apply_cheap(v + bias[e], p.act);
        cp[(int64_t)e * p.ohw] = v;
      }
    }
  };
  if constexpr (G::NA == G::WN) {
    run(std::integral_constant<int, G::JA>{}, wn * G::JA);
  } else {
    if (wn < G::NA)
      run(std::integral_constant<int, G::JA>{}, wn * G::JA);
    else
      run(std::integral_constant<int, G::JB>{}, G::NA * G::JA + (wn - G::NA) * G::JB);
  }
}

struct SlabForm {
  int bm, bn, bk;
  hipError_t (*gemm)(const SlabGemmArgs&, hipStream_t);
  hipError_t (*fill)(const SlabFillArgs&, int ks, hipStream_t);
  const char* name;
};

template <class G>
hipError_t launch_slab_gemm(const SlabGemmArgs& a, hipStream_t s) {
  const int64_t blocks = (int64_t)(a.M / G::BM) * ((a.N + G::BN - 1) / G::BN);
  hipLaunchKernelGGL((slab_gemm_kernel<G>), dim3((unsigned)blocks), dim3(G::NT), 0, s, a);
  return hipGetLastError();
}

template <int BK, int BN>
hipError_t launch_slab_fill(const SlabFillArgs& a, int ks, hipStream_t s) {
#ifndef TNS_SLAB_FILL_LANE
  {
    constexpr int NT = (BN + 63) / 64 * 64;
    const int64_t nb = a.units / BN;
    if (nb > 0x7fffffffLL) return hipErrorInvalidValue;
    if (ks == 3)
      hipLaunchKernelGGL((slab_fill_u_kernel<3, BK, BN>), dim3((unsigned)nb), dim3(NT), 0, s, a);
    else if (ks == 1)
      hipLaunchKernelGGL((slab_fill_u_kernel<1, BK, BN>), dim3((unsigned)nb), dim3(NT), 0, s, a);
    else
      return hipErrorInvalidValue;
    return hipGetLastError();
  }
#endif
  const unsigned blocks = (unsigned)((a.units + 255) / 256);
  if (ks == 3)
    hipLaunchKernelGGL((slab_fill_kernel<3, BK, BN>), dim3(blocks), dim3(256), 0, s, a);
  else if (ks == 1)
    hipLaunchKernelGGL((slab_fill_kernel<1, BK, BN>), dim3(blocks), dim3(256), 0, s, a);
  else
    return hipErrorInvalidValue;
  return hipGetLastError();
}

#define TNS_SLAB(BMv, BNv, BKv, WMv, WNv, JAv, NAv, NSv)                                       \
  {BMv, BNv, BKv, launch_slab_gemm<SG<BMv, BNv, BKv, WMv, WNv, JAv, NAv, NSv>>,                   \
   launch_slab_fill<BKv, BNv>,                                                                   \
   "conv_slab<" #BMv "x" #BNv "x" #BKv ",w" #WMv "x" #WNv ",j" #JAv "x" #NAv ",s" #NSv ">"}
#define TNS_SLABD(BMv, BNv, BKv, WMv, WNv, JAv, NAv, NSv, DGv, MAPv)                             \
  {BMv, BNv, BKv, launch_slab_gemm<SG<BMv, BNv, BKv, WMv, WNv, JAv, NAv, NSv, DGv, MAPv>>,       \
   launch_slab_fill<BKv, BNv>,                                                                   \
   "conv_slab<" #BMv "x" #BNv "x" #BKv ",w" #WMv "x" #WNv ",j" #JAv "x" #NAv ",s" #NSv ",dg" #DGv \
   ",map" #MAPv ">"}
const SlabForm kSlab[] = {
    TNS_SLAB(32, 176, 64, 2, 4, 3, 3, 3),
    TNS_SLAB(64, 176, 32, 4, 2, 6, 1, 3),
    TNS_SLAB(64, 176, 32, 4, 2, 6, 1, 4),
    TNS_SLAB(32, 176, 64, 2, 4, 3, 3, 2),
    TNS_SLAB(64, 176, 64, 4, 2, 6, 1, 2),
    TNS_SLAB(32, 176, 32, 2, 2, 6, 1, 4),
    TNS_SLABD(32, 176, 64, 2, 4, 3, 3, 2, 0, 1),
    TNS_SLABD(64, 176, 64, 4, 2, 6, 1, 2, 0, 1),
};
#undef TNS_SLAB
#undef TNS_SLABD
constexpr int kNumSlab = sizeof(kSlab) / sizeof(kSlab[0]);

}

int conv_slab_count() { return kNumSlab; }
const char* conv_slab_name(int v) { return v >= 0 && v < kNumSlab ? kSlab[v].name : ""; }

int conv_slab_pick(int64_t M, int64_t N, int64_t K, int64_t ks) {
  if (ks != 3 || K % 64) return -1;
  if (M == 1024 && N >= 1024) return 3;
  if (M == 512 && N >= 4096) return 4;
  return -1;
}

int64_t conv_slab_floats(int v, int64_t N, int64_t K) {
  if (v < 0 || v >= kNumSlab) return -1;
  const int64_t bn = kSlab[v].bn;
  return (N + bn - 1) / bn * bn * K;
}

hipError_t launch_conv_slab(int v, const ConvSlabArgs& c, float* slab, hipStream_t s) {
  if (v < 0 || v >= kNumSlab) return hipErrorInvalidValue;
  const SlabForm& f = kSlab[v];
  const int64_t N = c.batch * c.ohw;
  if (c.M % f.bm || c.K % f.bk || (c.ks != 1 && c.ks != 3) || N >= (1LL << 22) ||
      4 * c.batch * c.C * c.H * c.W > 0x7fffffffLL ||
      c.K > 0x7fffffffLL / f.bn || (reinterpret_cast<uintptr_t>(c.weights) & 15) || c.K % 4 ||
      (reinterpret_cast<uintptr_t>(slab) & 15) || c.M * c.K > 0x7fffffffLL)
    return hipErrorInvalidValue;
  const int64_t CT = (N + f.bn - 1) / f.bn, KT = c.K / f.bk;
  if (CT * (c.M / f.bm) > 0x7fffffffLL) return hipErrorInvalidValue;
  SlabFillArgs fa{};
  fa.x = c.input; fa.strideX = c.C * c.H * c.W; fa.slab = slab;
  fa.C = (int)c.C; fa.H = (int)c.H; fa.W = (int)c.W; fa.stride = (int)c.stride;
  fa.pad = (int)c.pad; fa.dil = (int)c.dil; fa.ow = (int)c.ow; fa.ohw = (int)c.ohw;
  fa.N = (int)N; fa.K = (int)c.K; fa.KT = (int)KT;
  fa.inv_ohw = (float)((1.0 + 1.0 / 1048576.0) / (double)c.ohw);
  fa.inv_ow = (float)((1.0 + 1.0 / 1048576.0) / (double)c.ow);
  fa.bytes = (unsigned)(4 * c.batch * c.C * c.H * c.W);
  fa.units = CT * KT * (f.bk / 16) * f.bn;
  if (hipError_t e = f.fill(fa, (int)c.ks, s)) return e;
  SlabGemmArgs ga{};
  ga.A = c.weights; ga.slab = slab; ga.C = c.out; ga.bias = c.bias;
  ga.M = (int)c.M; ga.N = (int)N; ga.K = (int)c.K; ga.KT = (int)KT;
  ga.tiles_m = (int)(c.M / f.bm); ga.ohw = (int)c.ohw; ga.act = c.act; ga.fuse = c.bias != nullptr;
  return f.gemm(ga, s);
}

}
```

### tensorium_amd/csrc/conv_tile.hip

```cpp
#include <type_traits>

#include "tns_act.hpp"
#include "tns_internal.hpp"

namespace tns {
namespace {

typedef float floatx4 __attribute__((ext_vector_type(4)));

constexpr int BK = 32;

template <int BM_, int BN_, int WM_, int SS_, bool PIN_ = true>
struct CGeo {
  static constexpr int BM = BM_, BN = BN_, WM = WM_;
  static constexpr bool PIN = PIN_;
  static constexpr int SS = SS_;
  static constexpr int NT = 64 * WM;
  static constexpr int WTM = BM / WM, TM = WTM / 16, J = BN / 16;
  static constexpr int LDA = BM + (TM == 2 ? 32 : 16);
  static constexpr int LDB = BN % 32 == 16 ? BN : BN + 16;
  static constexpr int A_TILE = BK * LDA, STAGE = BK * (LDA + LDB);
  static constexpr int AU = BM * BK / 4 / NT;
  static constexpr int KI = BK / 4 / WM;
  static_assert(TM == 1 || TM == 2, "strips read as one b32 / b64");
// ... 145 lines not shown
    const float* bp = st + A_TILE + k * LDB + r16;
#pragma unroll
    for (int j = 0; j < J; ++j) b[j] = bp[16 * j];
  };
  auto mma = [&](const float (&a)[TM], const float (&b)[J]) {
#pragma unroll
    for (int i = 0; i < TM; ++i)
#pragma unroll
      for (int j = 0; j < J; ++j)
        acc[i][j] = __builtin_amdgcn_mfma_f32_16x16x4f32(a[i], b[j], acc[i][j], 0, 0, 0);
  };

  const int nt = K / BK;
  if (nt > 0) {
    load_a(0);
    gather_b(0);
    store_a(smem);
    store_b(smem + A_TILE);
    __syncthreads();
  }
  auto tile = [&](int t, auto MORE) {
    constexpr bool more = decltype(MORE)::value;
    const float* cur = smem + (t & 1) * STAGE;
    float* nxt = smem + ((t + 1) & 1) * STAGE;
    if constexpr (more) {
      advance();
      load_a((t + 1) * BK);
      gather_b((t + 1) * BK);
      __builtin_amdgcn_sched_barrier(0);
    }
    float a0[TM], b0[J], a1[TM], b1[J];
    frag(cur, 0, a0, b0);
#pragma unroll
    for (int s = 0; s < BK / 4; s += 2) {
      frag(cur, s + 1, a1, b1);
      if constexpr (G::PIN) __builtin_amdgcn_sched_barrier(0);
      mma(a0, b0);
      if (s + 2 < BK / 4) frag(cur, s + 2, a0, b0);
      if constexpr (G::PIN) __builtin_amdgcn_sched_barrier(0);
      if constexpr (more)
        if (s == G::SS) {
          __builtin_amdgcn_sched_barrier(0);
#if !defined(TNS_CT_NOSTORE)
          store_a(nxt);
          store_b(nxt + A_TILE);
#endif
        }
      mma(a1, b1);
    }
#if !defined(TNS_CT_NOBAR)
    if constexpr (more) __syncthreads();
#endif
  };
  for (int t = 0; t + 1 < nt; ++t) tile(t, std::true_type{});
  if (nt > 0) tile(nt - 1, std::false_type{});

  const bool fuse = p.epi == EPI_BIAS_ACT;
  const int act = p.act;
#pragma unroll
  for (int i = 0; i < TM; ++i)
#pragma unroll
    for (int e = 0; e < 4; ++e) {
      const int64_t row = m0 + wm * WTM + 16 * i + 4 * q + e;
      const float bias = fuse ? p.bias[row] : 0.0f;
      float* crow = p.C + row * p.ldc;
#pragma unroll
      for (int j = 0; j < J; ++j) {
        if (n0 + 16 * j + r16 >= N) continue;
        float v = acc[i][j][e];
        if (fuse) v = act_apply_cheap(v + bias, act);
        crow[cofs[j]] = v;
      }
    }
}

template <class G>
hipError_t launch_g(const GemmArgs& a, int ks, int dil, hipStream_t s) {
  if (a.M % G::BM || a.K % BK || a.K <= 0 || a.lda % 4 ||
      (reinterpret_cast<uintptr_t>(a.A) & 15))
    return hipErrorInvalidValue;
  const int64_t tiles = (a.M / G::BM) * ((a.N + G::BN - 1) / G::BN);
  if (tiles > 0x7fffffff || a.N > 0x7fffffff || a.K > 0x7fffffff) return hipErrorInvalidValue;
  if (ks == 3)
    hipLaunchKernelGGL((conv_tile_kernel<G, 3>), dim3((unsigned)tiles), dim3(G::NT), 0, s, a, dil);
  else if (ks == 1)
    hipLaunchKernelGGL((conv_tile_kernel<G, 1>), dim3((unsigned)tiles), dim3(G::NT), 0, s, a, dil);
  else
    return hipErrorInvalidValue;
  return hipGetLastError();
}

struct TileInfo {
  int bm, bn;
  hipError_t (*fn)(const GemmArgs&, int, int, hipStream_t);
  const char* name;
};
#define TNS_CT(BMv, BNv, WMv, SSv, PINv)                                               \
  {BMv, BNv, launch_g<CGeo<BMv, BNv, WMv, SSv, PINv>>,                                 \
   "conv_tile<" #BMv "x" #BNv ",w" #WMv ",s" #SSv ">"}
const TileInfo kTiles[] = {
    TNS_CT(128, 176, 8, 4, true),
    TNS_CT(64, 96, 4, 6, false),
    TNS_CT(128, 96, 8, 4, true),
    TNS_CT(128, 176, 4, 4, true),
};
#undef TNS_CT
constexpr int kNumTiles = sizeof(kTiles) / sizeof(kTiles[0]);
#ifndef TNS_CT4_NO_PF
constexpr int kT4Big = 3;
constexpr int kT4Small = 8;
constexpr int kT4OneByOne = 13;
constexpr int kT4Uneven = 27;
constexpr int kT4UnevenS2 = 26;
constexpr int kT4OneByOnePF = 25;
constexpr int kT4Narrow = 21;
#else
constexpr int kT4OneByOnePF = 13;
constexpr int kT4UnevenS2 = 18;
constexpr int kT4Big = 3;
constexpr int kT4Small = 8;
constexpr int kT4OneByOne = 13;
constexpr int kT4Uneven = 18;
constexpr int kT4Narrow = 21;
#endif

}

int conv_tile_count() { return kNumTiles + conv_tile4_count(); }
const char* conv_tile_name(int v) {
  return v >= 0 && v < kNumTiles ? kTiles[v].name : conv_tile4_name(v - kNumTiles);
}

int conv_tile_pick(const GemmArgs& a, int ks) {
  if (a.K % BK || a.lda % 4 || (reinterpret_cast<uintptr_t>(a.A) & 15)) return -1;
  if (ks == 1) {
    if (a.M % 64 || a.M > 256 || a.N < 5408) return -1;
    return kNumTiles + (a.N < 16384 ? kT4OneByOnePF : kT4OneByOne);
  }
  if (ks != 3) return -1;
  if ((a.M == 128 || a.M == 256) && a.K % conv_tile4_bk(kT4Big) == 0) return kNumTiles + kT4Big;
  if ((a.M == 128 || a.M == 256) && a.conv_sY == 1) return 0;
  if (a.M == 64) return kNumTiles + kT4Small;
  if (a.M == 512) return kNumTiles + (a.conv_sY == 1 ? kT4Uneven : kT4UnevenS2);
  if (a.M == 1024 && a.K % conv_tile4_bk(kT4Narrow) == 0) return kNumTiles + kT4Narrow;
  return -1;
}

hipError_t launch_conv_tile(int v, const GemmArgs& a, int ks, int dil, hipStream_t s) {
  if (v >= kNumTiles) return launch_conv_tile4(v - kNumTiles, a, ks, dil, s);
  if (v < 0) return hipErrorInvalidValue;
  return kTiles[v].fn(a, ks, dil, s);
}

}
```

### tensorium_amd/csrc/conv_tile4.hip

```cpp
#include <type_traits>

#include "tns_act.hpp"
#include "tns_internal.hpp"

namespace tns {
namespace {

typedef float floatx4 __attribute__((ext_vector_type(4)));

template <int I, int N, class F>
__device__ __forceinline__ void cfor(F&& f) {
  if constexpr (I < N) {
    f(std::integral_constant<int, I>{});
    cfor<I + 1, N>(f);
  }
}

template <int JW>
struct Frag4 {
  floatx4 a, b[JW];
};

template <int BM_, int BN_, int WM_, int WN_, int BK_, int SG_, int IL_ = 0, bool SI_ = false,
          int RI_ = 0, bool ST_ = false, int JA_ = 0, int NA_ = 0, bool TA_ = false,
          bool DX_ = false, bool PF_ = false>
struct Geo4 {
  static constexpr bool PF = PF_;
  static constexpr bool DX = DX_;
  static constexpr bool TA = TA_;
  static constexpr int BM = BM_, BN = BN_, WM = WM_, WN = WN_, BK = BK_, SG = SG_;
  static constexpr int IL = IL_, RI = RI_;
  static constexpr bool SI = SI_, ST = ST_;
  static constexpr int NW = WM * WN, NT = 64 * NW;
  static constexpr int J = BN / 16;
  static constexpr int JA = JA_ > 0 ? JA_ : J / WN;
  static constexpr int NA = JA_ > 0 ? NA_ : WN;
  static constexpr int JB = NA < WN ? (J - NA * JA) / (WN - NA) : 0;
  static constexpr int NG = BK / 16;
  static constexpr int ROWS = BK / 4;
  static constexpr int A_TILE = ROWS * BM * 4;
  static constexpr int STAGE = ROWS * (BM + BN) * 4;
  static constexpr int AU = BM * BK / 4 / NT;
  static constexpr int KI = BK / 4 / NW;
  static_assert(BM == 16 * WM, "one 16-row strip per wave");
  static_assert(BM % 16 == 0 && BN % 16 == 0, "b128 slot rows: 64-dword multiples");
  static_assert(BK % 16 == 0 && SG <= NG - 2, "stores precede the barrier");
  static_assert(!(IL && SI) || SG >= 1 || PF_, "interleaved stores need a group after the loads");
  static_assert(!ST || (!IL && !SI && SG + 1 <= NG - 2 && NW % 2 == 0), "staggered staging");
  static_assert(AU >= 1 && BM * BK / 4 % NT == 0 && KI >= 1 && BK / 4 % NW == 0, "geometry");
  static_assert(NA * JA + (WN - NA) * JB == J && NA >= 1 && NA <= WN, "wave column split");
  static_assert(2 * STAGE * 4 + 64 <= 163840, "LDS");
  static_assert(!DX || TA, "DX: k-major weights");
  static_assert(!PF || !ST, "PF: register staging, no staggered halves");
  static constexpr int AST = 4 * AU;
  static constexpr int BLD = KI * J;
  static constexpr int BST = KI * J;
};

template <class G, int KS>
__global__ __launch_bounds__(G::NT) void conv_tile4_kernel(GemmArgs p, int dil) {
  constexpr int BM = G::BM, BN = G::BN, BK = G::BK, J = G::J, NG = G::NG;
  constexpr int A_TILE = G::A_TILE, STAGE = G::STAGE, AU = G::AU, KI = G::KI;
  __shared__ __attribute__((aligned(16))) float smem[2 * STAGE];
#ifdef TNS_CT4_STAMPS
  const unsigned long long rt_entry = __builtin_amdgcn_s_memrealtime();
#endif
  auto a_st = [&](int st) -> float* { return smem + st * STAGE; };
  auto b_st = [&](int st) -> float* { return smem + st * STAGE + A_TILE; };

  const int tid = threadIdx.x, lane = tid & 63, w = tid >> 6, wm = w % G::WM, wn = w / G::WM;
  const int half = __builtin_amdgcn_readfirstlane(w >= G::NW / 2 ? 1 : 0);
  const int r16 = lane & 15, q = lane >> 4;
  const int tiles_m = (int)(p.M / BM);
  int tm, tn;
  {
    const int nb = gridDim.x, bid = blockIdx.x;
    const int xcd = bid & 7, qq = nb >> 3, rr = nb & 7;
    const int wg = (xcd < rr ? xcd * (qq + 1) : rr * (qq + 1) + (xcd - rr) * qq) + (bid >> 3);
#if defined(TNS_CT4_MAP) && TNS_CT4_MAP == 1
    const int tiles_n = (int)((p.N + BN - 1) / BN);
    tn = wg % tiles_n;
    tm = wg / tiles_n;
#elif defined(TNS_CT4_MAP) && TNS_CT4_MAP == 2
    const int tiles_n = (int)((p.N + BN - 1) / BN);
    const int gm = min(4, tiles_m), per = gm * tiles_n, grp = wg / per;
    const int gs = min(gm, tiles_m - grp * gm), in = wg - grp * per;
    tm = grp * gm + in % gs;
    tn = in / gs;
#else
    tm = wg % tiles_m;
    tn = wg / tiles_m;
#endif
  }
  const int64_t m0 = (int64_t)tm * BM;
  const int n0 = tn * BN;
  const int N = (int)p.N, K = (int)p.K;
  const int H = p.conv_H, W = p.conv_W, HW = H * W;
  auto dx_pix = [&](int pix) -> int {
    if (!p.dx_cls) return pix;
    const int qy = pix / p.conv_ow, qx = pix - qy * p.conv_ow;
    return (2 * qy + ((p.dx_cls >> 1) & 1)) * p.dx_imgW + 2 * qx + ((p.dx_cls >> 2) & 1);
  };

  auto col_geo = [&](int n, unsigned& vb, unsigned& m) {
    n = n < N ? n : N - 1;
    const int img = n / p.conv_ohw, pix = n - img * p.conv_ohw;
    const int orow = pix / p.conv_ow, ocol = pix - orow * p.conv_ow;
    const int ir0 = orow * p.conv_sY - p.conv_pH, ic0 = ocol * p.conv_sX - p.conv_pW;
    vb = 4u * (unsigned)(img * (int)p.strideB + ir0 * W + ic0);
    m = 0;
#pragma unroll
    for (int kr = 0; kr < KS; ++kr)
#pragma unroll
      for (int kc = 0; kc < KS; ++kc)
        m |= (unsigned)(((unsigned)(ir0 + kr * dil) < (unsigned)H) &
                        ((unsigned)(ic0 + kc * dil) < (unsigned)W))
             << (kr * KS + kc);
  };
  unsigned vbase[J], tmask[J];
#pragma unroll
  for (int j = 0; j < J; ++j) col_geo(n0 + (16 * j + r16), vbase[j], tmask[j]);
  const __amdgpu_buffer_rsrc_t rsrc =
      __builtin_amdgcn_make_buffer_rsrc(const_cast<float*>(p.B), 0, p.conv_bytes, 0x00020000);

  int kc_[KI], kr_[KI], cc_[KI];
#pragma unroll
  for (int ii = 0; ii < KI; ++ii) {
    const int sl = w * KI + ii;
    const int k = 16 * (sl >> 2) + 4 * q + (sl & 3);
    if constexpr (G::DX) {
      cc_[ii] = k;
      kr_[ii] = kc_[ii] = 0;
      continue;
    }
    cc_[ii] = k / (KS * KS);
    const int rem = k - cc_[ii] * KS * KS;
    kr_[ii] = rem / KS;
    kc_[ii] = rem - kr_[ii] * KS;
  }
  const int F_ = G::DX ? K / (p.dx_cls ? (p.dx_taps >> 16) : KS * KS) : 0;
  int d_f0 = 0, d_t = 0;
  auto advance = [&]() {
    if constexpr (G::DX) {
      d_f0 += BK;
      if (d_f0 == F_) {
        d_f0 = 0;
        ++d_t;
      }
      return;
    }
#pragma unroll
    for (int ii = 0; ii < KI; ++ii) {
      if constexpr (KS == 1) {
        cc_[ii] += BK;
      } else {
        constexpr int DC = BK / (KS * KS), DR = BK % (KS * KS);
        int rem = kr_[ii] * KS + kc_[ii] + DR;
        int c = cc_[ii] + DC;
        if (rem >= KS * KS) { rem -= KS * KS; ++c; }
        cc_[ii] = c;
        kr_[ii] = rem >= 2 * KS ? 2 : (rem >= KS ? 1 : 0);
        kc_[ii] = rem - kr_[ii] * KS;
      }
    }
  };
  using S0 = std::integral_constant<int, 0>;
  using S1 = std::integral_constant<int, 1>;
  float rbs[G::PF ? 2 : 1][KI][J];
  auto gather_b = [&](auto SET) {
    auto& rb = rbs[decltype(SET)::value];
#pragma unroll
    for (int ii = 0; ii < KI; ++ii) {
      int y = kr_[ii] * dil, z = kc_[ii] * dil, tap = kr_[ii] * KS + kc_[ii], cc = cc_[ii];
      if constexpr (G::DX) {
        int fr = KS - 1 - d_t / KS, fc = KS - 1 - d_t % KS;
        if (p.dx_cls) {
          const int fb = (p.dx_taps >> (4 * d_t)) & 15;
          fr = fb / KS;
          fc = fb - fr * KS;
        }
        y = fr;
        z = fc;
        tap = fr * KS + fc;
        cc = d_f0 + cc_[ii];
      }
      const unsigned x = 4u * (unsigned)(cc * HW + y * W + z);
#pragma unroll
      for (int j = 0; j < J; ++j) {
#if defined(TNS_CT4_DIAG) && (TNS_CT4_DIAG & 1)
        rb[ii][j] = (float)(x + j);
#else
        const bool ok = __builtin_amdgcn_ubfe(tmask[j], tap, 1) != 0;
        const unsigned off = ok ? vbase[j] + x : 0x80000000u;
        rb[ii][j] = __builtin_bit_cast(float, __builtin_amdgcn_raw_buffer_load_b32(rsrc, off, 0, 0));
#endif
      }
    }
  };
  int b_dst[KI];
#pragma unroll
  for (int ii = 0; ii < KI; ++ii) b_dst[ii] = (w * KI + ii) * BN * 4 + r16 * 4 + q;
  auto store_b = [&](float* bs, auto SET) {
    auto& rb = rbs[decltype(SET)::value];
#if defined(TNS_CT4_DIAG) && (TNS_CT4_DIAG & 2)
    return;
#endif
#pragma unroll
    for (int ii = 0; ii < KI; ++ii)
#pragma unroll
      for (int j = 0; j < J; ++j) bs[b_dst[ii] + 64 * j] = rb[ii][j];
  };

  const float* a_src[AU];
// ... 128 lines not shown
    store_b(b_st(0), S0{});
    __syncthreads();
    frag(0, 0, f0);
  }
  auto tile = [&](int t, auto MORE, auto PAR) {
    constexpr bool more = decltype(MORE)::value;
    constexpr int par = decltype(PAR)::value;
    using SL = std::integral_constant<int, G::PF ? par : 0>;
    using SS = std::integral_constant<int, G::PF ? par ^ 1 : 0>;
    const int tc = t & 1, tx = (t + 1) & 1;
    TNS_PH(5);
    if constexpr (more && G::PF && !G::IL) {
      advance();
      load_a(min((t + 2) * BK, K - BK), SL{});
      gather_b(SL{});
      __builtin_amdgcn_sched_barrier(0);
    } else if constexpr (more && !G::IL && !G::ST && !G::PF) {
      advance();
      load_a((t + 1) * BK, S0{});
      gather_b(S0{});
      __builtin_amdgcn_sched_barrier(0);
    }
    TNS_PH(0);
#pragma unroll
    for (int g = 0; g < NG; ++g) {
      Frag& fc = (g & 1) ? f1 : f0;
      Frag& fn = (g & 1) ? f0 : f1;
      if constexpr (more)
        if (g == NG - 1) {
          TNS_PH(3);
#ifdef TNS_CT4_STAMPS
          if (t == 8 && lane == 0 && p.stamps != nullptr && blockIdx.x < (1u << 16) && w < 16)
            p.stamps[32 * blockIdx.x + 16 + w] =
                (unsigned)(__builtin_amdgcn_s_memtime() & 0xffffffffu);
#endif
          __syncthreads();
          TNS_PH(4);
        }
      __builtin_amdgcn_sched_barrier(0);
      if constexpr (more && G::ST)
        if (g < 2 && half == g) {
          advance();
          load_a((t + 1) * BK, S0{});
          gather_b(S0{});
          __builtin_amdgcn_sched_barrier(0);
        }
      const bool reads = g + 1 < NG || more;
      if (g + 1 < NG)
        frag(tc, g + 1, fn);
      else if (more)
        frag(tx, 0, fn);
      if constexpr (more && G::IL) {
        if (g == 0) {
          advance();
          if constexpr (G::PF) {
            load_a(min((t + 2) * BK, K - BK), SL{});
            gather_b(SL{});
          } else {
            load_a((t + 1) * BK, S0{});
            gather_b(S0{});
          }
        }
      }
      if constexpr (more && G::SI) {
        if (g == G::SG) {
          store_a(a_st(tx), SS{});
          store_b(b_st(tx), SS{});
        }
      }
      mma(fc);
      if constexpr (G::RI > 0 || G::IL > 0 || G::SI) {
#pragma unroll
        for (int i = 0; i < 4 * JW; ++i) {
          __builtin_amdgcn_sched_group_barrier(0x008, 1, 0);
          if constexpr (G::RI > 0)
            if (reads && i % G::RI == 0 && i / G::RI < JW + 1)
              __builtin_amdgcn_sched_group_barrier(0x100, 1, 0);
          if constexpr (more && G::IL > 0)
            if (g == 0) {
              __builtin_amdgcn_sched_group_barrier(0x002, G::IL, 0);
              if (i < AU + G::BLD) __builtin_amdgcn_sched_group_barrier(0x020, 1, 0);
            }
          if constexpr (more && G::SI)
            if (g == G::SG && i < G::AST + G::BST)
              __builtin_amdgcn_sched_group_barrier(0x200, 1, 0);
        }
      }
      __builtin_amdgcn_sched_barrier(0);
      if constexpr (more && G::ST)
        if (g >= G::SG && g <= G::SG + 1 && g == G::SG + half) {
          store_a(a_st(tx), S0{});
          store_b(b_st(tx), S0{});
          __builtin_amdgcn_sched_barrier(0);
        }
      if constexpr (more && !G::SI && !G::ST)
        if (g == G::SG) {
          TNS_PH(1);
          store_a(a_st(tx), SS{});
          store_b(b_st(tx), SS{});
          __builtin_amdgcn_sched_barrier(0);
          TNS_PH(2);
        }
    }
    if constexpr (G::DX) flush();
  };
  static_assert(NG % 2 == 0, "f0 holds group 0 at every tile start");
  if constexpr (G::PF) {
    int t = 0;
    for (; t + 2 < nt; t += 2) {
      tile(t, std::true_type{}, S0{});
      tile(t + 1, std::true_type{}, S1{});
    }
    if (t + 1 < nt) {
      tile(t, std::true_type{}, S0{});
      tile(t + 1, std::false_type{}, S1{});
    } else if (t < nt) {
      tile(t, std::false_type{}, S0{});
    }
  } else {
    for (int t = 0; t + 1 < nt; ++t) tile(t, std::true_type{}, S0{});
    if (nt > 0) tile(nt - 1, std::false_type{}, S0{});
  }

#ifdef TNS_CT4_STAMPS
  TNS_PH(5);
  if (tid == 0 && p.stamps != nullptr && blockIdx.x < (1u << 16)) {
    unsigned* st = p.stamps + 32 * blockIdx.x;
    for (int i = 0; i < 6; ++i) st[i] = (unsigned)ph[i];
    st[6] = (unsigned)(tl - tk0);
    const unsigned long long rt_loop = __builtin_amdgcn_s_memrealtime();
    st[7] = (unsigned)nt | (unsigned)(rt_loop - rt0) << 8;
    st[8] = (unsigned)rt_entry;
    st[9] = (unsigned)(rt_entry >> 32);
    st[10] = (unsigned)(rt0 - rt_entry);
    st[12] = (unsigned)(rt_loop - rt_entry);
  }
#endif
#undef TNS_PH
  const bool fuse = p.epi == EPI_BIAS_ACT;
  const int act = p.act;
  if constexpr (G::DX) {
    const int64_t row0 = m0 + wm * 16 + 4 * q;
#pragma unroll
    for (int j = 0; j < JW; ++j) {
      const int n = n0 + coff * 16 + 16 * j + r16;
      if (n >= N) continue;
      const int img = n / p.conv_ohw, pix = dx_pix(n - img * p.conv_ohw);
      float* cp = p.C + (int64_t)img * p.strideC + pix + row0 * p.ldc;
#pragma unroll
      for (int e = 0; e < 4; ++e) cp[e * p.ldc] = rs[j][e];
    }
    return;
  }
  const bool add = p.epi == EPI_ADD;
  const int64_t row0 = m0 + wm * 16 + 4 * q;
  float bias[4];
#pragma unroll
  for (int e = 0; e < 4; ++e) bias[e] = fuse ? p.bias[row0 + e] : 0.0f;
#pragma unroll
  for (int j = 0; j < JW; ++j) {
    const int n = n0 + coff * 16 + 16 * j + r16;
    if (n >= N) continue;
    const int img = n / p.conv_ohw, pix = n - img * p.conv_ohw;
    float* cp = p.C + (int64_t)img * p.strideC + pix + row0 * p.ldc;
#pragma unroll
    for (int e = 0; e < 4; ++e) {
      float v = acc[j][e];
      if (fuse) v = act_apply_cheap(v + bias[e], act);
      if (add) v = cp[e * p.ldc] + v;
      cp[e * p.ldc] = v;
    }
  }
#ifdef TNS_CT4_STAMPS
  if (tid == 0 && p.stamps != nullptr && blockIdx.x < (1u << 16)) {
    asm volatile("s_waitcnt vmcnt(0)" ::: "memory");
    p.stamps[32 * blockIdx.x + 11] = (unsigned)(__builtin_amdgcn_s_memrealtime() - rt_entry);
  }
#endif
  };
  if constexpr (G::NA == G::WN) {
    run(std::integral_constant<int, G::JA>{}, wn * G::JA);
  } else {
    if (__builtin_amdgcn_readfirstlane(wn) < G::NA)
      run(std::integral_constant<int, G::JA>{}, wn * G::JA);
    else
      run(std::integral_constant<int, G::JB>{}, G::NA * G::JA + (wn - G::NA) * G::JB);
  }
}

#ifdef TNS_CT4_STAMPS
unsigned* g_ct4_stamps = nullptr;
#endif

template <class G>
hipError_t launch_g4(const GemmArgs& a_in, int ks, int dil, hipStream_t s) {
  GemmArgs a = a_in;
#ifdef TNS_CT4_STAMPS
  a.stamps = g_ct4_stamps;
#endif
  if (a.M % G::BM || a.K % G::BK || a.K <= 0) return hipErrorInvalidValue;
  if (!G::TA && (a.lda % 4 || (reinterpret_cast<uintptr_t>(a.A) & 15))) return hipErrorInvalidValue;
  if (G::TA && (a.lda < a.M || a.K * a.lda > 0x7fffffffLL)) return hipErrorInvalidValue;
  const int64_t tiles = (a.M / G::BM) * ((a.N + G::BN - 1) / G::BN);
  if (tiles > 0x7fffffff || a.N > 0x7fffffff || a.K > 0x7fffffff) return hipErrorInvalidValue;
  if (ks == 3)
    hipLaunchKernelGGL((conv_tile4_kernel<G, 3>), dim3((unsigned)tiles), dim3(G::NT), 0, s, a, dil);
  else if (ks == 1)
    hipLaunchKernelGGL((conv_tile4_kernel<G, 1>), dim3((unsigned)tiles), dim3(G::NT), 0, s, a, dil);
  else
    return hipErrorInvalidValue;
  return hipGetLastError();
}

struct TileInfo4 {
  int bm, bn, bk;
  hipError_t (*fn)(const GemmArgs&, int, int, hipStream_t);
  const char* name;
};
#define TNS_CT4(BMv, BNv, WMv, WNv, BKv, SGv, ILv, SIv, RIv, STv)                      \
  {BMv, BNv, BKv, launch_g4<Geo4<BMv, BNv, WMv, WNv, BKv, SGv, ILv, SIv, RIv, STv>>,    \
   "conv_tile4<" #BMv "x" #BNv "x" #BKv ",w" #WMv "x" #WNv ",g" #SGv ",il" #ILv ",si" #SIv \
   ",ri" #RIv ",st" #STv ">"}
#define TNS_CT4U(BMv, BNv, WMv, WNv, BKv, SGv, SIv, RIv, JAv, NAv)                      \
  {BMv, BNv, BKv, launch_g4<Geo4<BMv, BNv, WMv, WNv, BKv, SGv, 0, SIv, RIv, false, JAv, NAv>>, \
   "conv_tile4<" #BMv "x" #BNv "x" #BKv ",w" #WMv "x" #WNv ",g" #SGv ",si" #SIv ",ri" #RIv    \
   ",j" #JAv "x" #NAv ">"}
#define TNS_CT4P(BMv, BNv, WMv, WNv, BKv, SGv, SIv, RIv, JAv, NAv)                           \
  {BMv, BNv, BKv,                                                                             \
   launch_g4<Geo4<BMv, BNv, WMv, WNv, BKv, SGv, 0, SIv, RIv, false, JAv, NAv, false, false,  \
                  true>>,                                                                    \
   "conv_tile4_pf<" #BMv "x" #BNv "x" #BKv ",w" #WMv "x" #WNv ",g" #SGv ",si" #SIv ",ri" #RIv \
   ",j" #JAv "x" #NAv ">"}
#define TNS_CT4PI(BMv, BNv, WMv, WNv, BKv, SGv, ILv, SIv, RIv, JAv, NAv)                     \
  {BMv, BNv, BKv,                                                                             \
   launch_g4<Geo4<BMv, BNv, WMv, WNv, BKv, SGv, ILv, SIv, RIv, false, JAv, NAv, false, false, \
                  true>>,                                                                    \
   "conv_tile4_pf<" #BMv "x" #BNv "x" #BKv ",w" #WMv "x" #WNv ",g" #SGv ",il" #ILv ",si" #SIv  \
   ",ri" #RIv ",j" #JAv "x" #NAv ">"}
const TileInfo4 kTiles4[] = {
    TNS_CT4(128, 176, 8, 1, 32, 0, 0, false, 0, false),
    TNS_CT4(128, 176, 8, 1, 64, 2, 0, false, 0, false),
    TNS_CT4(128, 176, 8, 1, 64, 1, 0, true, 3, false),
    TNS_CT4(128, 176, 8, 1, 64, 1, 0, true, 2, false),
    TNS_CT4(128, 176, 8, 1, 64, 1, 0, false, 3, true),
    TNS_CT4(128, 176, 8, 1, 64, 1, 0, false, 0, true),
    TNS_CT4(128, 176, 8, 1, 64, 1, 0, false, 2, true),
    TNS_CT4(64, 96, 4, 1, 32, 0, 0, false, 0, false),
    TNS_CT4(64, 96, 4, 1, 32, 0, 0, false, 3, false),
    TNS_CT4(64, 192, 4, 2, 64, 1, 0, false, 3, true),
    TNS_CT4(64, 96, 4, 2, 64, 1, 0, false, 3, true),
    TNS_CT4(64, 64, 4, 2, 32, 0, 0, false, 0, false),
    TNS_CT4(64, 64, 4, 1, 32, 0, 0, false, 0, false),
    TNS_CT4(64, 32, 4, 1, 32, 0, 0, false, 0, false),
    TNS_CT4(64, 32, 4, 2, 32, 0, 0, false, 0, false),
    TNS_CT4(64, 64, 4, 1, 64, 2, 0, false, 0, false),
    TNS_CT4(64, 32, 4, 1, 64, 2, 0, false, 0, false),
    TNS_CT4U(64, 176, 4, 2, 64, 1, true, 2, 6, 1),
    TNS_CT4U(64, 176, 4, 2, 32, 0, false, 3, 6, 1),
    TNS_CT4U(32, 176, 2, 4, 64, 1, true, 2, 3, 3),
    TNS_CT4(128, 48, 8, 1, 32, 0, 0, false, 3, false),
    TNS_CT4(128, 48, 8, 1, 64, 1, 0, true, 2, false),
    TNS_CT4(64, 48, 4, 1, 32, 0, 0, false, 3, false),
    TNS_CT4(64, 48, 4, 1, 64, 1, 0, true, 2, false),
    TNS_CT4(128, 96, 8, 1, 64, 1, 0, true, 2, false),
    TNS_CT4P(64, 32, 4, 1, 32, 0, false, 0, 0, 0),
    TNS_CT4PI(64, 176, 4, 2, 32, 0, 2, false, 3, 6, 1),
    TNS_CT4PI(64, 176, 4, 2, 32, 0, 0, true, 3, 6, 1),
};
#define TNS_CT4T(BMv, BNv, WMv, WNv, BKv, SGv, SIv, RIv, JAv, NAv)                      \
  {BMv, BNv, BKv,                                                                      \
   launch_g4<Geo4<BMv, BNv, WMv, WNv, BKv, SGv, 0, SIv, RIv, false, JAv, NAv, true>>,  \
   "conv_tile4_ta<" #BMv "x" #BNv "x" #BKv ",w" #WMv "x" #WNv ",g" #SGv ",si" #SIv     \
   ",ri" #RIv ",j" #JAv "x" #NAv ">"}
#define TNS_CT4TP(BMv, BNv, WMv, WNv, BKv, SGv, SIv, RIv, JAv, NAv)                      \
  {BMv, BNv, BKv,                                                                      \
   launch_g4<Geo4<BMv, BNv, WMv, WNv, BKv, SGv, 0, SIv, RIv, false, JAv, NAv, true, false, \
                  true>>,                                                               \
   "conv_tile4_ta_pf<" #BMv "x" #BNv "x" #BKv ",w" #WMv "x" #WNv ",g" #SGv ",si" #SIv   \
   ",ri" #RIv ",j" #JAv "x" #NAv ">"}
const TileInfo4 kTiles4T[] = {
    TNS_CT4T(128, 176, 8, 1, 64, 1, true, 2, 0, 0),
    TNS_CT4T(128, 96, 8, 1, 64, 1, true, 2, 0, 0),
    TNS_CT4T(128, 48, 8, 1, 64, 1, true, 2, 0, 0),
    TNS_CT4T(64, 176, 4, 2, 32, 0, false, 3, 6, 1),
    TNS_CT4T(64, 96, 4, 1, 32, 0, false, 3, 0, 0),
    TNS_CT4T(64, 32, 4, 1, 32, 0, false, 0, 0, 0),
    TNS_CT4T(128, 176, 8, 1, 32, 0, false, 3, 0, 0),
    TNS_CT4T(64, 64, 4, 2, 32, 0, false, 3, 0, 0),
    TNS_CT4T(64, 64, 4, 1, 32, 0, false, 3, 0, 0),
    TNS_CT4T(128, 64, 8, 1, 32, 0, false, 3, 0, 0),
    TNS_CT4T(64, 128, 4, 2, 32, 0, false, 3, 0, 0),
    TNS_CT4TP(64, 96, 4, 1, 32, 0, false, 3, 0, 0),
    TNS_CT4TP(64, 64, 4, 2, 32, 0, false, 3, 0, 0),
    TNS_CT4TP(128, 48, 8, 1, 64, 1, true, 2, 0, 0),
};
constexpr int kNumTiles4T = sizeof(kTiles4T) / sizeof(kTiles4T[0]);
#define TNS_CT4DX(BMv, BNv, WMv, WNv, BKv, SGv, SIv, RIv, JAv, NAv)                          \
  {BMv, BNv, BKv,                                                                          \
   launch_g4<Geo4<BMv, BNv, WMv, WNv, BKv, SGv, 0, SIv, RIv, false, JAv, NAv, true, true>>, \
   "conv_tile4_dx<" #BMv "x" #BNv "x" #BKv ",w" #WMv "x" #WNv ",g" #SGv ",si" #SIv         \
   ",ri" #RIv ",j" #JAv "x" #NAv ">"}
#define TNS_CT4DXP(BMv, BNv, WMv, WNv, BKv, SGv, SIv, RIv, JAv, NAv)                         \
  {BMv, BNv, BKv,                                                                          \
   launch_g4<Geo4<BMv, BNv, WMv, WNv, BKv, SGv, 0, SIv, RIv, false, JAv, NAv, true, true,   \
                  true>>,                                                                  \
   "conv_tile4_dx_pf<" #BMv "x" #BNv "x" #BKv ",w" #WMv "x" #WNv ",g" #SGv ",si" #SIv      \
   ",ri" #RIv ",j" #JAv "x" #NAv ">"}
const TileInfo4 kTiles4DX[] = {
    TNS_CT4DX(64, 176, 4, 2, 32, 0, false, 3, 6, 1),
    TNS_CT4DX(64, 96, 4, 1, 32, 0, false, 3, 0, 0),
    TNS_CT4DX(64, 48, 4, 1, 32, 0, false, 3, 0, 0),
    TNS_CT4DX(128, 96, 8, 1, 64, 1, true, 2, 0, 0),
    TNS_CT4DX(64, 64, 4, 2, 32, 0, false, 3, 0, 0),
    TNS_CT4DX(128, 48, 8, 1, 64, 1, true, 2, 0, 0),
    TNS_CT4DX(32, 176, 2, 4, 64, 1, true, 2, 3, 3),
    TNS_CT4DXP(64, 176, 4, 2, 32, 0, false, 3, 6, 1),
    TNS_CT4DXP(64, 64, 4, 2, 32, 0, false, 3, 0, 0),
    TNS_CT4DXP(32, 176, 2, 4, 64, 1, true, 2, 3, 3),
    TNS_CT4DXP(64, 48, 4, 1, 32, 0, false, 3, 0, 0),
};
constexpr int kNumTiles4DX = sizeof(kTiles4DX) / sizeof(kTiles4DX[0]);
#undef TNS_CT4DX
#undef TNS_CT4DXP
#undef TNS_CT4
#undef TNS_CT4U
#undef TNS_CT4T
#undef TNS_CT4TP
#undef TNS_CT4P
#undef TNS_CT4PI
constexpr int kNumTiles4 = sizeof(kTiles4) / sizeof(kTiles4[0]);

}

int conv_tile4_count() { return kNumTiles4; }
const char* conv_tile4_name(int v) { return v >= 0 && v < kNumTiles4 ? kTiles4[v].name : ""; }
int conv_tile4_bk(int v) { return v >= 0 && v < kNumTiles4 ? kTiles4[v].bk : 0; }

#ifdef TNS_CT4_STAMPS
extern "C" int tns_debug_ct4_stamps(unsigned* dev_buf) {
  g_ct4_stamps = dev_buf;
  return 0;
}
#endif

int conv_tile4_ta_count() { return kNumTiles4T; }
const char* conv_tile4_ta_name(int v) { return v >= 0 && v < kNumTiles4T ? kTiles4T[v].name : ""; }

int conv_tile4_dx_pick(int64_t M, int64_t N, int64_t K, int64_t ks) {
#ifndef TNS_CT4_TA_NO_PF
  if (N < 4096 && K % 32 == 0 && M % 64 == 0) return 12;
#endif
  if (ks == 1) {
    if (N >= 4096) return (M % 64 == 0 && K % 32 == 0) ? 7 : -1;
    return (K % 64 == 0 && M % 128 == 0) ? 2 : -1;
  }
  if (K % 32 == 0 && M % 64 == 0) {
    if (N < 4096) return 4;
// ... 9 lines not shown
  if (add_into && ks != 1) return hipErrorInvalidValue;
  const int64_t M = C * ks * ks, hw = oh * ow;
  if (batch * F * hw * 4 > 0x7fffffffLL || batch * hw > 0x7fffffffLL) return hipErrorInvalidValue;
  GemmArgs a{};
  a.M = M; a.N = batch * hw; a.K = F;
  a.alpha = 1.0f; a.beta = 0.0f; a.beta_mode = BETA_ZERO;
  a.A = w; a.lda = M; a.strideA = 0;
  a.B = delta; a.ldb = hw; a.strideB = F * hw;
  a.C = col; a.ldc = hw; a.strideC = M * hw;
  a.batch = 1; a.epi = add_into ? EPI_ADD : EPI_NONE; a.bias = nullptr; a.act = 0;
  a.conv = 2;
  a.conv_H = (int)oh; a.conv_W = (int)ow; a.conv_ow = (int)ow; a.conv_ohw = (int)hw;
  a.conv_sY = 1; a.conv_sX = 1; a.conv_pH = 0; a.conv_pW = 0;
  a.conv_bytes = (int)(4 * batch * F * hw);
  return kTiles4T[v].fn(a, 1, 1, s);
}

int conv_tile4_dx3_count() { return kNumTiles4DX; }
const char* conv_tile4_dx3_name(int v) { return v >= 0 && v < kNumTiles4DX ? kTiles4DX[v].name : ""; }

namespace {
bool dx3_fits(int v, int64_t batch, int64_t C, int64_t H, int64_t W, int64_t F, int64_t ks,
              int64_t pad, int64_t oh, int64_t ow) {
  if (v < 0 || v >= kNumTiles4DX || ks != 3 || pad < 0 || pad > ks - 1) return false;
  if (oh != H + 2 * pad - ks + 1 || ow != W + 2 * pad - ks + 1 || oh <= 0 || ow <= 0) return false;
  if (F % kTiles4DX[v].bk || C % kTiles4DX[v].bm || batch <= 0) return false;
  return batch * F * oh * ow * 4 <= 0x7fffffffLL && batch * C * H * W <= 0x7fffffffLL &&
         ks * ks * F * C <= 0x7fffffffLL;
}
}

int conv_tile4_dx3_pick(int64_t batch, int64_t C, int64_t H, int64_t W, int64_t F, int64_t ks,
                        int64_t pad) {
  const int64_t N = batch * H * W, oh = H + 2 * pad - ks + 1, ow = W + 2 * pad - ks + 1;
  int v = -1;
  if (C % 64 && N >= 50000)
    v = 6;
  else if (N >= 50000)
    v = 4;
  else if (N >= 16384)
    v = 0;
  return v >= 0 && dx3_fits(v, batch, C, H, W, F, ks, pad, oh, ow) ? v : -1;
}

hipError_t launch_conv_tile4_dx3(int v, const float* wt, const float* delta, float* im,
                                 int64_t batch, int64_t C, int64_t H, int64_t W, int64_t F,
                                 int64_t ks, int64_t pad, int64_t oh, int64_t ow, hipStream_t s) {
  if (!dx3_fits(v, batch, C, H, W, F, ks, pad, oh, ow)) return hipErrorInvalidValue;
  GemmArgs a{};
  a.M = C; a.N = batch * H * W; a.K = ks * ks * F;
  a.alpha = 1.0f; a.beta = 0.0f; a.beta_mode = BETA_ZERO;
  a.A = wt; a.lda = C; a.strideA = 0;
  a.B = delta; a.ldb = oh * ow; a.strideB = F * oh * ow;
  a.C = im; a.ldc = H * W; a.strideC = C * H * W;
  a.batch = 1; a.epi = EPI_NONE; a.bias = nullptr; a.act = 0;
  a.conv = 2;
  a.conv_H = (int)oh; a.conv_W = (int)ow; a.conv_ow = (int)W; a.conv_ohw = (int)(H * W);
  a.conv_sY = 1; a.conv_sX = 1; a.conv_pH = (int)(ks - 1 - pad); a.conv_pW = (int)(ks - 1 - pad);
  a.conv_bytes = (int)(4 * batch * F * oh * ow);
  return kTiles4DX[v].fn(a, 3, 1, s);
}

namespace {
int s2_taps(int64_t pad, int py, int px, int* ref, int* fwd) {
  int n = 0;
  for (int kr = 0; kr < 3; ++kr) {
    const int dr = py + (int)pad - kr;
    if (dr & 1) continue;
    for (int kc = 0; kc < 3; ++kc) {
      const int dc = px + (int)pad - kc;
      if (dc & 1) continue;
      ref[n] = kr * 3 + kc;
      fwd[n] = (dr / 2 + 1) * 3 + (dc / 2 + 1);
      ++n;
    }
  }
  return n;
}

bool dx3s2_fits(int v, int64_t batch, int64_t C, int64_t H, int64_t W, int64_t F, int64_t pad,
                int64_t oh, int64_t ow) {
  if (v < 0 || v >= kNumTiles4DX || pad < 0 || pad > 2 || H < 2 || W < 2) return false;
  if (oh != (H + 2 * pad - 3) / 2 + 1 || ow != (W + 2 * pad - 3) / 2 + 1 || oh <= 0 || ow <= 0)
    return false;
  if (F % kTiles4DX[v].bk || C % kTiles4DX[v].bm || batch <= 0) return false;
  return batch * F * oh * ow * 4 <= 0x7fffffffLL && batch * C * H * W <= 0x7fffffffLL &&
         9 * F * C <= 0x7fffffffLL;
}
}

unsigned long long conv_tile4_dx3s2_order(int64_t pad) {
  unsigned long long o = 0;
  int sl = 0, ref[9], fwd[9];
  for (int cls = 0; cls < 4; ++cls) {
    const int n = s2_taps(pad, cls >> 1, cls & 1, ref, fwd);
    for (int i = 0; i < n; ++i, ++sl) o |= (unsigned long long)ref[i] << (4 * sl);
  }
  return o;
}

int conv_tile4_dx3s2_pick(int64_t batch, int64_t C, int64_t H, int64_t W, int64_t F, int64_t ks,
                          int64_t pad) {
  if (ks != 3) return -1;
  const int64_t N = batch * (H / 2) * (W / 2), oh = (H + 2 * pad - 3) / 2 + 1,
                ow = (W + 2 * pad - 3) / 2 + 1;
  int v = -1;
  if (C % 64 && N >= 50000)
    v = 6;
  else if (N >= 50000)
    v = 2;
  return v >= 0 && dx3s2_fits(v, batch, C, H, W, F, pad, oh, ow) ? v : -1;
}

hipError_t launch_conv_tile4_dx3s2(int v, const float* wt, const float* delta, float* im,
                                   int64_t batch, int64_t C, int64_t H, int64_t W, int64_t F,
                                   int64_t pad, int64_t oh, int64_t ow, hipStream_t s) {
  if (!dx3s2_fits(v, batch, C, H, W, F, pad, oh, ow)) return hipErrorInvalidValue;
  int sl = 0;
  for (int cls = 0; cls < 4; ++cls) {
    const int py = cls >> 1, px = cls & 1;
    int ref[9], fwd[9];
    const int T = s2_taps(pad, py, px, ref, fwd);
    const int64_t ohc = (H - py + 1) / 2, owc = (W - px + 1) / 2;
    if (T == 0 || ohc <= 0 || owc <= 0) {
      sl += T;
      continue;
    }
    GemmArgs a{};
    a.M = C; a.N = batch * ohc * owc; a.K = T * F;
    a.alpha = 1.0f; a.beta = 0.0f; a.beta_mode = BETA_ZERO;
    a.A = wt + (int64_t)sl * F * C; a.lda = C; a.strideA = 0;
    a.B = delta; a.ldb = oh * ow; a.strideB = F * oh * ow;
    a.C = im; a.ldc = H * W; a.strideC = C * H * W;
    a.batch = 1; a.epi = EPI_NONE; a.bias = nullptr; a.act = 0;
    a.conv = 2;
    a.conv_H = (int)oh; a.conv_W = (int)ow; a.conv_ow = (int)owc; a.conv_ohw = (int)(ohc * owc);
    a.conv_sY = 1; a.conv_sX = 1; a.conv_pH = 1; a.conv_pW = 1;
    a.conv_bytes = (int)(4 * batch * F * oh * ow);
    a.dx_cls = 1 | py << 1 | px << 2;
    a.dx_taps = T << 16;
    for (int i = 0; i < T; ++i) a.dx_taps |= fwd[i] << (4 * i);
    a.dx_imgW = (int)W;
    if (hipError_t e = kTiles4DX[v].fn(a, 3, 1, s); e != hipSuccess) return e;
    sl += T;
  }
  return hipSuccess;
}

hipError_t launch_conv_tile4(int v, const GemmArgs& a, int ks, int dil, hipStream_t s) {
  if (v < 0 || v >= kNumTiles4) return hipErrorInvalidValue;
  return kTiles4[v].fn(a, ks, dil, s);
}

}
```

### tensorium_amd/csrc/tns_internal.hpp

```cpp
#pragma once
#include <hip/hip_runtime.h>
#include <stdint.h>

#include "../../include/tns.h"
#include "gemm_plan.hpp"

namespace tns {

int set_error(int code, const char* fmt, ...);
const char* hip_err_str(hipError_t e);

#define TNS_HIP_TRY(expr)                                                              \
  do {                                                                                 \
    hipError_t _e = (expr);                                                            \
    if (_e != hipSuccess)                                                              \
      return ::tns::set_error(TNS_ERR_HIP, "%s failed: %s (%s:%d)", #expr,            \
                              ::tns::hip_err_str(_e), __FILE__, __LINE__);             \
  } while (0)

enum EpiKind { EPI_NONE = 0, EPI_BIAS_ACT = 1, EPI_ADD = 2 };
constexpr bool act_transcendental(int act) { return act == 0 || act == 6; }

enum BetaMode { BETA_ZERO = 0, BETA_ONE = 1, BETA_SCALE = 2, BETA_STORE = 3 };

struct GemmArgs {
  int64_t M, N, K;
  float alpha, beta;
  int beta_mode;
  const float* A;
  int64_t lda, strideA;
  const float* B;
  int64_t ldb, strideB;
  float* C;
  int64_t ldc, strideC;
  int64_t batch;
  int epi;
  const float* bias;
  int act;
  int conv;
  const int* ktab;
  int ktab_n;
  int conv_H, conv_W, conv_ow, conv_ohw, conv_sY, conv_sX, conv_pH, conv_pW;
  int conv_bytes;
  int dx_cls, dx_taps, dx_imgW;
  unsigned* stamps;
};

inline GemmShape gemm_shape(const GemmArgs& a, bool transA, bool transB) {
  GemmShape s;
  s.ta = transA; s.tb = transB;
  s.M = a.M; s.N = a.N; s.K = a.K;
  s.lda = a.lda; s.ldb = a.ldb; s.ldc = a.ldc;
  s.strideA = a.strideA; s.strideB = a.strideB; s.strideC = a.strideC;
  s.batch = a.batch;
  s.alpha1 = a.alpha == 1.0f;
  s.beta_mode = a.beta_mode;
  s.epi = a.epi;
  s.conv = a.conv != 0;
  s.a16 = (reinterpret_cast<uintptr_t>(a.A) & 15) == 0;
  s.b16 = (reinterpret_cast<uintptr_t>(a.B) & 15) == 0;
  return s;
}
hipError_t launch_gemm_plan(const GemmPlan& p, const GemmArgs& a, hipStream_t s);
hipError_t launch_sgemm(const GemmArgs& a, bool transA, bool transB, hipStream_t s);
int sgemm_nn_big_count();
const char* sgemm_nn_big_name(int v);
hipError_t launch_sgemm_nn_big(const GemmPlan& p, const GemmArgs& a, hipStream_t s);
hipError_t launch_sgemm_nn_pp(const GemmArgs& a, hipStream_t s);
hipError_t launch_sgemm_nn_w4(const GemmPlan& p, const GemmArgs& a, hipStream_t s);
hipError_t launch_sgemm_nt_sdot(const GemmArgs& a, hipStream_t s);
hipError_t launch_sdot_chains(const GemmArgs& a, int variant, hipStream_t s);
int sdot_chains_variant_count();
const char* sdot_chains_variant_name(int v);
int sdot_rc_variant_count();
const char* sdot_rc_variant_name(int v);
hipError_t launch_sdot_rc(int v, const GemmArgs& a, hipStream_t s);
void set_sdot_form(int form);
int get_sdot_form();
hipError_t launch_sgemm_nt_sdot_tn(const GemmPlan& p, const GemmArgs& a, hipStream_t s);
hipError_t launch_sgemm_tt(const GemmArgs& a, hipStream_t s);
hipError_t launch_sgemm_tt_plan(const GemmPlan& p, const GemmArgs& a, hipStream_t s);
hipError_t launch_add_in_order(float* C, const float* part, int64_t n, int64_t batch,
                               hipStream_t s);
hipError_t launch_sgemm_conv(const GemmArgs& a, hipStream_t s);
hipError_t launch_sgemm_conv_variant(int variant, const GemmArgs& a, hipStream_t s);
int conv_tile_count();
const char* conv_tile_name(int v);
int conv_tile_pick(const GemmArgs& a, int ks);
hipError_t launch_conv_tile(int v, const GemmArgs& a, int ks, int dil, hipStream_t s);
struct ConvSlabArgs {
  const float* input;
  const float* weights;
  const float* bias;
  float* out;
  int64_t batch, C, H, W, M, K, ks, stride, pad, dil, ow, ohw;
  int act;
};
int conv1x1_count();
const char* conv1x1_name(int v);
int conv1x1_pick(int64_t M, int64_t N, int64_t K, int64_t P);
hipError_t launch_conv1x1(int v, const float* weights, const float* x, const float* bias,
                          float* out, int64_t batch, int64_t M, int64_t K, int64_t P, int act,
                          hipStream_t s, bool add = false);
hipError_t launch_transpose(const float* in, float* out, int64_t rows, int64_t cols,
                            hipStream_t s);
int conv_slab_count();
const char* conv_slab_name(int v);
int conv_slab_pick(int64_t M, int64_t N, int64_t K, int64_t ks);
int64_t conv_slab_floats(int v, int64_t N, int64_t K);
hipError_t launch_conv_slab(int v, const ConvSlabArgs& c, float* slab, hipStream_t s);
int conv_tile4_count();
const char* conv_tile4_name(int v);
int conv_tile4_bk(int v);
hipError_t launch_conv_tile4(int v, const GemmArgs& a, int ks, int dil, hipStream_t s);
int conv_tile4_ta_count();
const char* conv_tile4_ta_name(int v);
int conv_tile4_dx_pick(int64_t M, int64_t N, int64_t K, int64_t ks);
hipError_t launch_conv_tile4_dx(int v, const float* w, const float* delta, float* col,
                                int64_t batch, int64_t C, int64_t ks, int64_t F, int64_t oh,
                                int64_t ow, hipStream_t s, bool add_into = false);
int conv_tile4_dx3_count();
const char* conv_tile4_dx3_name(int v);
int conv_tile4_dx3_pick(int64_t batch, int64_t C, int64_t H, int64_t W, int64_t F, int64_t ks,
                        int64_t pad);
hipError_t launch_conv_tile4_dx3(int v, const float* wt, const float* delta, float* im,
                                 int64_t batch, int64_t C, int64_t H, int64_t W, int64_t F,
                                 int64_t ks, int64_t pad, int64_t oh, int64_t ow, hipStream_t s);
hipError_t launch_transpose_taps(const float* w, float* wt, int64_t F, int64_t C, int64_t K2,
                                 hipStream_t s, unsigned long long order = ~0ULL);
unsigned long long conv_tile4_dx3s2_order(int64_t pad);
int conv_tile4_dx3s2_pick(int64_t batch, int64_t C, int64_t H, int64_t W, int64_t F, int64_t ks,
                          int64_t pad);
hipError_t launch_conv_tile4_dx3s2(int v, const float* wt, const float* delta, float* im,
                                   int64_t batch, int64_t C, int64_t H, int64_t W, int64_t F,
                                   int64_t pad, int64_t oh, int64_t ow, hipStream_t s);
struct DwArgs {
  const float* delta;
  const float* x;
  float* part;
  int M, N, HW, C, H, W, oW, stride, pad, dil;
  int va;
  float alpha;
  int64_t strideA, strideX, strideP, batch;
};
int dw_tile_count();
const char* dw_tile_name(int v);
int dw_tile_pick(const DwArgs& a, int ks);
hipError_t launch_dw_tile(int v, const DwArgs& a, int ks, hipStream_t s);
bool conv_direct_applies(int64_t C, int64_t ks, int64_t filters);
hipError_t launch_conv_direct(const float* in, const float* w, const float* bias, float* out,
                              int64_t batch, int64_t C, int64_t H, int64_t W, int64_t filters,
                              int64_t ks, int64_t stride, int64_t pad, int64_t dil, int64_t oh,
                              int64_t ow, int act, hipStream_t s);
bool conv_dx_fused_applies(int64_t C, int64_t H, int64_t W, int64_t ks, int64_t stride, int64_t F,
                           int64_t oh, int64_t ow);
bool conv_dx_fused_fits(int64_t C, int64_t H, int64_t W, int64_t stride, int64_t F, int64_t oh,
                        int64_t ow);
hipError_t launch_conv_dx_col2im(const float* w, float* wt, const float* delta, float* im,
                                 int64_t batch, int64_t C, int64_t H, int64_t W, int64_t F,
                                 int64_t ks, int64_t pad, int64_t dil, int64_t oh, int64_t ow,
                                 hipStream_t s);
constexpr int KTAB_PAD = 256;
hipError_t launch_build_ktab(int* ktab, int C, int Hs, int Ws, int kH, int kW, int dY, int dX,
                             hipStream_t s);
hipError_t launch_pad_images(const float* im, int64_t batch, int64_t C, int64_t H, int64_t W,
                             int64_t pH, int64_t pW, float* out, hipStream_t s);
hipError_t launch_sgemm_variant(int variant, const GemmArgs& a, bool transA, bool transB,
                                hipStream_t s);
int sgemm_variant_count();
const char* sgemm_variant_name(int v);

struct ConvGeom {
  int64_t C, H, W, kH, kW, padH, padW, sY, sX, dY, dX;
  int64_t oh, ow;
};
int64_t out_dim(int64_t in, int64_t pad, int64_t k, int64_t dil, int64_t stride);
hipError_t launch_im2col(const ConvGeom& g, const float* im, int64_t imStride, float* col,
                         int64_t colStride, int64_t batch, hipStream_t s);
hipError_t launch_col2im(const ConvGeom& g, const float* col, int64_t colStride, float* im,
                         int64_t imStride, int64_t batch, hipStream_t s);
struct DwResArgs {
  ConvGeom g;
  const float* x;
  int64_t xStride;
  const float* delta;
  float* weight_updates;
  float *dA, *dB, *part;
  int64_t M, N, K, batch;
  bool direct;
  float alpha;
};
int dw_res_count();
const char* dw_res_name(int v);
int64_t dw_res_k4(int64_t K);
int64_t dw_res_groups(int v);
int64_t dw_res_b_rows(int v, int64_t N);
int dw_res_pick(int64_t M, int64_t N, int64_t K, int64_t batch);
hipError_t launch_dw_res(int v, const DwResArgs& d, hipStream_t s);

bool act_supported(int act);
hipError_t launch_forward_bias(float* dst, int64_t nFilters, int64_t blockSize,
                               const float* bias, int64_t incb, int64_t batch, hipStream_t s);
hipError_t launch_backward_bias(float* dst, int64_t nDst, const float* src, int64_t blockSize,
                                int64_t batch, int64_t incb, hipStream_t s);
hipError_t launch_activate(float* x, int64_t n, int act, hipStream_t s);
hipError_t launch_shortcut(int64_t n, const float* a, const float* b, float* out, int act,
                           hipStream_t s);
hipError_t launch_upsample(int64_t planes, int H, int W, int stride, float scale, const float* in,
                           float* out, hipStream_t s);
hipError_t launch_upsample_backward(int64_t planes, int H, int W, int stride, float scale,
                                   float* in, const float* out, int zero, hipStream_t s);
struct PoolGeom {
  int h, w, outH, outW, size, sx, sy, off;
};
hipError_t launch_maxpool_forward(int64_t planes, const PoolGeom& g, const float* in, float* out,
                                  int64_t* indexes, hipStream_t s);
hipError_t launch_avgpool_forward(int64_t planes, const PoolGeom& g, const float* in, float* out,
                                  hipStream_t s);
hipError_t launch_maxpool_backward(int64_t planes, const PoolGeom& g, float* state_delta,
                                   const int64_t* indexes, const float* delta, hipStream_t s);
hipError_t launch_avgpool_backward(int64_t planes, const PoolGeom& g, float* state_delta,
                                   const float* delta, hipStream_t s);
hipError_t launch_dropout_forward(int64_t n, uint32_t seed, float probability, float scale,
                                  const float* src, float* rnd, float* dst, hipStream_t s);
hipError_t launch_dropout_backward(int64_t n, float probability, float scale, const float* src,
                                   const float* rnd, float* dst, hipStream_t s);
hipError_t launch_cost_l2(int64_t n, const float* pred, const float* truth, float* delta,
                          float* error, hipStream_t s);
hipError_t launch_xent_logistic(int64_t n, const float* pred, const float* truth, float* delta,
                                float* error, hipStream_t s);
hipError_t launch_lstm_gates_forward(int64_t n, const float* const w[4], const float* const u[4],
                                     float* c_state, float* h_state, float* cell_slice,
                                     float* out_slice, hipStream_t s);
hipError_t launch_lstm_gates_backward(int64_t n, const float* const w[4], const float* const u[4],
                                      const float* cell_i, const float* cprev,
                                      const float* delta_i, float* dc, float* const dw[4],
                                      float* const du[4], hipStream_t s);
hipError_t launch_rnn_state_forward(int64_t n, int64_t H, float* in_slice, const float* in_bias,
                                    int in_act, float* self_slice, const float* self_bias,
                                    int self_act, const float* state_prev, float* state_next,
                                    hipStream_t s);
hipError_t launch_rnn_delta_backward(int64_t n, float* delta, const float* out, int act,
                                     float* delta2, const float* out2, int act2, hipStream_t s);
hipError_t launch_vv(int op, int64_t n, const float* a, int64_t inca, const float* b, int64_t incb,
                     const float* c, int64_t incc, float* d, int64_t incd, hipStream_t s);
hipError_t launch_fmavss(int64_t n, const float* src, float scalar, float bias, float* dst,
                         hipStream_t s);
hipError_t launch_inverse_sqrt(int64_t n, const float* src, float* dst, int64_t stride,
                               hipStream_t s);
hipError_t launch_yolo(int64_t batch, int anchors, int classes, int64_t hw, const float* in,
                       float* out, hipStream_t s);
constexpr int kYoloMaxAnchors = 32;
constexpr int kYoloMaxBoxes = 2048;
struct YoloLossParams {
  int batch, n, classes, h, w, total, maxBoxes, netW, netH;
  float ignoreThresh, truthThresh, iouThresh, iouNormalizer, objNormalizer;
  int mask[kYoloMaxAnchors];
  float biases[2 * kYoloMaxAnchors];
};
int64_t yolo_loss_scratch_floats(int64_t n);
hipError_t launch_yolo_loss(const YoloLossParams& p, float* out, const float* truth, float* delta,
                            float* cost, float* stats, unsigned long long* counters,
                            float* scratch, hipStream_t s);
constexpr int kDetMaxCapacity = 1 << 22;
struct DetParams {
  int batch, n, classes, h, w, netW, netH, imW, imH, relative, letter, capacity;
  float thresh;
  int mask[kYoloMaxAnchors];
  float biases[2 * kYoloMaxAnchors];
};
int64_t detections_scratch_floats(const DetParams& p);
hipError_t launch_yolo_detections(const DetParams& p, const float* out, int64_t* counts,
                                  float* boxes, float* objectness, float* probs, float* scratch,
                                  hipStream_t s);
hipError_t launch_nms_sort(int batch, int capacity, int classes, const int64_t* counts,
                           const float* boxes, const float* objectness, float* probs,
                           float thresh, hipStream_t s);
constexpr int kImagePerLaunch = 32;
constexpr int64_t kImageMaxExtent = 32768;
struct ImageGeom {
  int64_t off, rs;
  int w, h, nw, nh, dx, dy;
  float ws, hs;
};
hipError_t launch_image_to_input(bool bytes, const ImageGeom* geom, int64_t count, const void* src,
                                 int channels, int pixelStride, const float* table, int netW,
                                 int netH, float* dst, hipStream_t s);
hipError_t launch_bias_activate(float* dst, int64_t nFilters, int64_t blockSize,
                                const float* bias, int64_t batch, int act, hipStream_t s);
hipError_t launch_derive(const float* x, int64_t n, int act, float* delta, hipStream_t s);
hipError_t launch_sgd_update(int64_t nw, float* w, float* dw, int64_t n, float* b, float* db,
                             float* sc, float* dsc, float lrb, float ndb, float mom,
                             hipStream_t s);
hipError_t launch_axpy(int64_t n, float a, const float* x, int64_t incx, float* y, int64_t incy,
                       hipStream_t s);
hipError_t launch_scale(int64_t n, float a, float* x, int64_t stride, hipStream_t s);
hipError_t launch_fill(int64_t n, float* x, float v, int64_t stride, hipStream_t s);
hipError_t launch_copy(int64_t n, const float* src, int64_t inca, float* dst, int64_t incb,
                       hipStream_t s);
hipError_t launch_clamp(int64_t n, float alpha, const float* src, float* dst, int64_t stride,
                        hipStream_t s);

hipError_t launch_means_vars(const float* x, int64_t groups, int64_t N, int64_t bs, float* means,
                             float* vars, int quirk, float* part, hipStream_t s, int what = 3);
hipError_t launch_normalize(float* x, int64_t groups, int64_t N, int64_t bs, const float* means,
                            int64_t mstride, const float* vars, int64_t vstride, hipStream_t s);
hipError_t launch_scale_add(float* x, int64_t groups, int64_t N, int64_t bs, const float* scales,
                            const float* biases, int64_t incb, hipStream_t s);
hipError_t launch_add_dots(float* dst, const float* a, const float* b, int64_t groups, int64_t N,
                           int64_t bs, float* part, hipStream_t s);
hipError_t launch_add_sums(float* dst, const float* src, int64_t groups, int64_t N, int64_t bs,
                           float* part, hipStream_t s);
hipError_t launch_derive_add_sums(float* dst, float* delta, const float* output, int act,
                                  int64_t groups, int64_t N, int64_t bs, float* part,
                                  hipStream_t s);
hipError_t launch_mean_var_delta(const float* delta, const float* x, const float* mean,
                                 const float* var, int64_t groups, int64_t N, int64_t bs,
                                 float* mean_delta, float* var_delta, int quirk, float* part,
                                 hipStream_t s, const float* scales = nullptr);
hipError_t launch_normalize_delta(const float* x, const float* mean, const float* var,
                                  const float* mean_delta, const float* var_delta, float* delta,
                                  int64_t groups, int64_t N, int64_t bs, hipStream_t s, const float* scales = nullptr); 
bool bn_folds_scale(int64_t bs);
hipError_t launch_bn_backward_fused(float* scale_updates, const float* x_norm, float* delta,
                                    const float* output, int act, const float* x,
                                    const float* mean, const float* var, const float* scales,
                                    float* mean_delta, float* var_delta, int64_t groups,
                                    int64_t N, int64_t bs, int quirk, float* part, hipStream_t s);
hipError_t launch_add_dots_derive(float* dst, const float* x_norm, float* delta,
                                  const float* output, int act, int64_t groups, int64_t N,
                                  int64_t bs, float* part, hipStream_t s);
hipError_t launch_bn_apply(const float* y, float* x, float* xn, float* out, int64_t groups,
                           int64_t N, int64_t bs, const float* means, const float* vars,
                           const float* scales, const float* biases, int act, hipStream_t s);
hipError_t launch_rolling_update(int64_t n, float* rm, float* rv, const float* mean,
                                 const float* var, float momentum, hipStream_t s);
hipError_t launch_softmax_batch(int64_t n, const float* in, int64_t batch, int64_t batch_size,
                                int64_t groups, int64_t group_size, int64_t stride, float temp,
                                float* out, hipStream_t s);
hipError_t launch_xent_softmax(int64_t n, const float* pred, const float* truth, float* delta,
                               float* error, hipStream_t s);
hipError_t launch_vssum(int64_t n, const float* a, float* out, hipStream_t s);

constexpr int MLP_MAX_LAYERS = 16;
struct MlpArgs {
  int nlayers;
  int64_t widths[MLP_MAX_LAYERS + 1];
  int acts[MLP_MAX_LAYERS];
  int bn;
  int64_t batch;
  const float* X;
  const float* truth;
  float lr, momentum, decay;
  float* buf;
  float* cost;
  int64_t off[MLP_MAX_LAYERS][16];
  int64_t softmax_off;
  int64_t stamp_off;
  int lds_chunks;
  int64_t act_off;
  float* l0part;
};
int64_t mlp_buffer_floats(int nlayers, const int64_t* widths, int bn, int64_t batch);
hipError_t launch_mlp_train_step(const MlpArgs& a, hipStream_t s);

struct Options;
struct ConvShape {
  int64_t batch, C, H, W, filters, kSize, stride, padding, dilation;
  int32_t activation;
  bool weights_aligned16;
};
constexpr int kPlanMsg = 256;

enum ConvFwdPath {
  FWD_EMPTY = 0,
  FWD_UNFUSED,
  FWD_IM2COL,
  FWD_DIRECT,
  FWD_CONV1X1,
  FWD_SLAB,
  FWD_TILE,
  FWD_IMPLICIT
};
struct ConvFwdPlan {
  int err = 0;
  char msg[kPlanMsg] = {};
  ConvShape s{};
  int64_t oh = 0, ow = 0;
  int path = FWD_EMPTY;
  int form = -1;
  bool implicit = false;
  bool bias_act = false;
  int epi_act = 0;
  bool act_tail = false;
  bool needs_col = false;
  bool padded = false;
  int64_t chunk = 0;
  int64_t col_elems = 0, stage1_elems = 0;
  int64_t conv_variant = -1;
  int srss_quirk = 0;
};
ConvFwdPlan plan_conv_forward(const ConvShape& s, int fused, bool bias_act, const Options& o);

enum ConvDwPath { DW_RES = 0, DW_TILE, DW_SDOT, DW_GEMM };
struct ConvDwChoice {
  int path = DW_GEMM;
  int form = -1;
  bool col = false;
  int64_t part_elems = 0;
};
enum ConvDxPath {
  DX_NONE = 0,
  DX_CONV1X1,
  DX_FUSED,
  DX_CONV3,
  DX_CONV3S2,
  DX_TILE,
  DX_TN
};
enum ConvBwdSched { BWD_SEQUENTIAL = 0, BWD_JOINED, BWD_PIPELINED };
struct ConvBwdPlan {
  int err = 0;
  char msg[kPlanMsg] = {};
  ConvShape s{};
  ConvGeom g{};
  bool empty = true;
  bool has_bn = false, has_state_delta = false, delta_aligned16 = false;
  int64_t i_m = 0, i_n = 0, i_k = 0, colSize = 0;
  bool bn_fused = false;
  bool derive_sums = false;
  int srss_quirk = 0;
  ConvDwChoice dw;
  ConvDwChoice dw_fallback;
  bool dw_res_forced = false;
  int dx = DX_NONE;
  int dx_form = -1;
  int dx_tile = -1;
  bool dx_tile_forced = false;
  bool dx_direct = false;
  bool needs_col = false;
  bool dx_col = false;
  int sched = BWD_SEQUENTIAL;
  int64_t bn_elems = 0, res_a_elems = 0, res_b_elems = 0, col_elems = 0, wt_elems = 0;
};
ConvBwdPlan plan_conv_backward(const ConvShape& s, bool has_bn, bool has_state_delta,
                               bool delta_aligned16, const Options& o);

}
```

### tensorium_amd/darknet.py

```python
from __future__ import annotations

import struct
from dataclasses import dataclass, field
from pathlib import Path

import numpy as np

from ._abi import ACT, TnsError

SEPS = np.float32(0.000001)


@dataclass
class Section:
    kind: str
    opts: dict = field(default_factory=dict)

    def get(self, key, default=None):
        return self.opts.get(key, default)

    def int(self, key, default=0):
        return int(self.opts.get(key, default))


# ... 875 lines not shown
                if training:
                    self._sub_bn_forward(l, L, si, i, True, activate=False)
                self._sub_bn_forward(l, L, ss, i, training, activate=False)
            hip.rnnStateForward(n, H, at(si["out"], off), None if l.bn else si["b"], si["act"],
                                at(ss["out"], off), None if l.bn else ss["b"], ss["act"],
                                at(state, off) if l.shortcut else None, at(state, off + j0 * n))
        hip.gemm(False, True, T * S, O, H, 1.0, state, j0 * n, H, so["w"], 0, H, 0.0, so["out"], 0,
                 O)
        if not l.bn:
            hip.forwardBias(T * m, so["out"], 0, O, so["b"], 1, T * S)
        elif training:
            for i in range(T):
                self._sub_bn_forward(l, L, so, i, True, activate=False)
        else:
            hip.normalize(O, T * m, T * S, so["rm"], 1, so["rv"], 1, so["out"], 0)
            hip.forwardScaleAdd(T * m, so["out"], 0, O, so["scales"], so["b"], 1, T * S)
        hip.ActivateArray(T * m, so["out"], 0, so["act"])

    def _rnn_backward(self, l, inp, sd):
        hip, L, at = self.hip, self.rnn[l.index], self._at
        S, T, n, m, H, I = L["S"], L["T"], L["n"], L["m"], l.hidden, l.in_size
        si, ss, so = (L["sub"][g] for g in RNN_SUBS)
        state = L["state"]
        inp = inp.reshape(-1)
        fused = self.rnn_fused
        for i in range(T - 1, -1, -1):
            off, offm = i * n, i * m
            hip.addvv(n, si["out"], off, 1, ss["out"], off, 1, state, off + n, 1)
            if fused:
                hip.rnnDeltaBackward(m, at(so["delta"], offm), at(so["out"], offm), so["act"])
            self._sub_backward(l, L, so, i, state, i + 1, ss["delta"], i, clamp=not fused)
            if fused:
                chain = not l.bn
                hip.rnnDeltaBackward(n, at(ss["delta"], off), at(ss["out"], off), ss["act"],
                                     at(si["delta"], off) if chain else None,
                                     at(si["out"], off) if chain else None, si["act"])
            self._sub_backward(l, L, ss, i, state, i, ss["delta"] if i else None, i - 1,
                               clamp=not fused)
            if not fused or l.bn:
                hip.copy(n, ss["delta"], off, 1, si["delta"], off, 1)
            if fused and l.bn:
                hip.rnnDeltaBackward(n, at(si["delta"], off), at(si["out"], off), si["act"])
            if i and l.shortcut:
                hip.addvv(n, ss["delta"], off - n, 1, ss["delta"], off, 1, ss["delta"], off - n, 1)
            self._sub_backward(l, L, si, i, inp, i, None if fused else sd, i, clamp=not fused)
        if not fused:
            return
        if sd is not None:
            hip.gemm(False, False, T * S, I, H, 1.0, si["delta"], 0, H, si["w"], 0, I, 1.0, sd, 0,
                     I)
        if l.bn and T > 1:
            hip.clamp((T - 1) * m, 1.0, so["delta"], so["delta"], 1, m)

    def _rnn_update(self, l, learning_rate, momentum, decay):
        for g in RNN_SUBS:
            st = self.rnn[l.index]["sub"][g]
            self.hip.sgdUpdate(st["w"], st["wu"], st["b"], st["bu"], learning_rate,
                               self.net.batch, decay, momentum, st.get("scales"), st.get("su"))


def detection_rows_to_host(torch, taken, cap, classes, boxes, obj, probs, pin=None):
    total = sum(taken)
    need = max(total * (5 + classes), 1)
    if pin is None or pin.numel() < need:
        pin = torch.empty(need, dtype=torch.float32).pin_memory()
    hb, ho, hp = pin[:4 * total], pin[4 * total:5 * total], pin[5 * total:need]
    at = 0
    for b, n in enumerate(taken):
        if n:
            hb[4 * at:4 * (at + n)].copy_(boxes[b * cap * 4:(b * cap + n) * 4], non_blocking=True)
            ho[at:at + n].copy_(obj[b * cap:b * cap + n], non_blocking=True)
            if classes:
                hp[classes * at:classes * (at + n)].copy_(
                    probs[b * cap * classes:(b * cap + n) * classes], non_blocking=True)
        at += n
    torch.cuda.current_stream().synchronize()
    res, at = [], 0
    for n in taken:
        res.append((hb[4 * at:4 * (at + n)].numpy().reshape(n, 4).copy(),
                    ho[at:at + n].numpy().copy(),
                    hp[classes * at:classes * (at + n)].numpy().reshape(n, classes).copy()))
        at += n
    return res, pin


@dataclass
class Placement:
    new_w: int
    new_h: int
    dx: int
    dy: int
    w: int
    h: int
    ratio: object = None


def images_to_input(hip, torch, images, channels, net_w, net_h, dst, letter=False, table="fpc"):
    if not images:
        return []
    on_dev = [hasattr(im, "is_cuda") for im in images]
    if any(on_dev) and not all(on_dev):
        raise ValueError("images: NumPy arrays and tensors in one call")
    kinds = {str(im.dtype).replace("torch.", "") for im in images}
    if len(kinds) != 1 or kinds & {"uint8", "float32"} != kinds:
        raise ValueError(f"images: one of uint8 / float32 for all of them, got {sorted(kinds)}")
    as_bytes = kinds == {"uint8"}
    geom, at, ps = [], 0, None
    for n, im in enumerate(images):
        if im.ndim != 3:
            raise ValueError(f"image {n}: shape {tuple(im.shape)}")
        h, w, c = im.shape if as_bytes else (im.shape[1], im.shape[2], im.shape[0])
        if (c < channels or c > 4) if as_bytes else c != channels:
            raise ValueError(f"image {n}: {c} channels for a network of {channels}")
        if as_bytes and ps not in (None, c):
            raise ValueError(f"image {n}: {c} bytes a pixel after images of {ps}")
        ps = c
        geom.append((at, w, h, w * c if as_bytes else w))
        at += h * w * c
    if all(on_dev):
        src = torch.cat([im.contiguous().reshape(-1) for im in images])
    else:
        src = torch.from_numpy(np.concatenate(
            [np.ascontiguousarray(im).reshape(-1) for im in images])).cuda()
    placed = hip.imageToInput(src, geom, channels, net_w, net_h, dst, letter=letter, table=table,
                              pixelStride=ps if as_bytes else None)
    res = []
    for (nw, nh, dx, dy), (_, w, h, _) in zip(placed, geom):
        ratio = None
        if letter:
            ratio = np.float32(net_w / w) if net_w * h < net_h * w else np.float32(net_h / h)
        res.append(Placement(nw, nh, dx, dy, w, h, ratio))
    return res


def letterbox_truth(boxes, placements, net_w, net_h, max_boxes):
    F = np.float32
    out = np.zeros((len(boxes), max_boxes, 6), F)
    for b, (objs, p) in enumerate(zip(boxes, placements)):
        if len(objs) > max_boxes:
            raise ValueError(f"image {b}: {len(objs)} objects, max_boxes {max_boxes}")
        for j, o in enumerate(objs):
            if o is None:
                continue
            left, top, right, bottom = (d + int(np.trunc(F(v) * p.ratio))
                                        for d, v in zip((p.dx, p.dy, p.dx, p.dy), o[:4]))
            out[b, j] = (F((left + right) / (2 * net_w)), F((top + bottom) / (2 * net_h)),
                         F((right - left) / net_w), F((bottom - top) / net_h), F(o[4]), 0)
    return out


class HipDarknet(_RnnLayers, _LstmLayers):

    def __init__(self, hip, net: Network, params: list[ConvParams], torch,
                 lstm_fused: bool = True, rnn_fused: bool = True):
        self.hip, self.net, self.torch = hip, net, torch
        self.lstm_fused = bool(lstm_fused)
        self.rnn_fused = bool(rnn_fused)
        B = net.batch
        dev = "cuda"
        t = lambda a: torch.from_numpy(np.ascontiguousarray(a, dtype=np.float32)).to(dev)
        self.out = []
        for l in net.layers:
            alias = l.kind == "dropout" and l.index > 0
            self.out.append(self.out[-1] if alias else torch.empty(B * l.out_size, device=dev))
        self.conv_params, self.fc_params = {}, {}
        blocks = list(zip(net.param_layers(), params))
        kind = lambda b: net.layers[b[0].index].kind if b[0].gate else ""
        self._lstm_init([b for b in blocks if kind(b) == "lstm"], training=False)
        self._rnn_init([b for b in blocks if kind(b) == "rnn"], training=False)
        for l, p in blocks:
            if l.gate:
                continue
            if l.kind == "connected":
                st = {"w": t(p.weights), "b": t(p.biases)}
                if l.bn:
                    st.update(scales=t(p.scales), rm=t(p.rolling_mean), rv=t(p.rolling_var))
                self.fc_params[l.index] = st
                continue
            f = fuse_batchnorm(l, p)
            self.conv_params[l.index] = (t(f.weights), t(f.biases))

    def forward(self, x):
        hip, B = self.hip, self.net.batch
        prev = x
        for l in self.net.layers:
            out = self.out[l.index]
            if l.kind == "convolutional":
                w, b = self.conv_params[l.index]
                hip.convForward(B, l.c, l.h, l.w, prev, w, b, l.filters, l.size, l.stride, l.pad,
                                1, l.activation, None, out, fused=True)
            elif l.kind == "shortcut":
                src = self.out[l.inputs[0]]
                hip.shortcut(B * l.out_size, prev, 0, src, 0, out, 0, l.activation)
            elif l.kind == "route":
                off = 0
                for s in l.inputs:
                    n = B * self.net.layers[s].out_size
                    hip.copy(n, self.out[s], 0, 1, out, off, 1)
                    off += n
            elif l.kind == "upsample":
                hip.upSample(B, l.c, l.h, l.w, prev, l.stride, 1, 1.0, out)
            elif l.kind == "yolo":
                hip.yoloForward(B, l.anchors, l.classes, l.h * l.w, prev, out)
            elif l.kind == "maxpool":
                hip.forwardMaxPool(B, l.out_c, l.out_h, l.out_w, prev, l.c, l.h, l.w, l.stride_x,
                                   l.stride_y, l.pad, l.size, None, out)
            elif l.kind == "local_avgpool":
                hip.forwardAvgPool(B, l.out_c, l.out_h, l.out_w, prev, l.c, l.h, l.w, l.stride_x,
                                   l.stride_y, l.pad, l.size, out)
            elif l.kind == "connected":
                st, n = self.fc_params[l.index], B * l.filters
                hip.gemm(False, True, B, l.filters, l.in_size, 1.0, prev, 0, l.in_size, st["w"], 0,
                         l.in_size, 0.0, out, 0, l.filters)
                if l.bn:
                    hip.normalize(l.filters, n, B, st["rm"], 1, st["rv"], 1, out, 0)
                    hip.forwardScaleAdd(n, out, 0, l.filters, st["scales"], st["b"], 1, B)
                else:
                    hip.forwardBias(n, out, 0, l.filters, st["b"], 1, B)
                hip.ActivateArray(n, out, 0, l.activation)
            elif l.kind == "lstm":
                self._lstm_forward(l, prev, False)
            elif l.kind == "rnn":
                self._rnn_forward(l, prev, False)
            elif l.kind == "dropout":
                out = self.out[l.index] = prev.reshape(-1)
            elif l.kind == "softmax":
                g = l.in_size // l.groups
                hip.softmaxBatch(g, prev, 0, B, l.in_size, l.groups, g, 1, l.temperature, out, 0)
            elif l.kind == "logistic":
                hip.copy(B * l.in_size, prev, 0, 1, out, 0, 1)
                hip.ActivateArray(B * l.in_size, out, 0, l.activation)
            prev = out
        return self.out

    def detections(self, im_w, im_h, thresh=0.5, relative=False, letter=False, nms=None,
                   capacity=None):
        hip, torch, B = self.hip, self.torch, self.net.batch
        yolos = [l for l in self.net.layers if l.kind == "yolo"]
        if not yolos:
            raise ValueError("detections: the network has no [yolo] layer")
        if len({l.classes for l in yolos}) > 1:
            raise ValueError("detections: the [yolo] layers disagree on classes: "
                             f"{[l.classes for l in yolos]}")
        bad = [f"layer {l.index} {k}" for l in yolos for k in l.unbuilt
               if k in ("new_coords", "embedding_layer")]
        if bad:
            raise ValueError("detections: not built: " + ", ".join(bad))
        classes = yolos[0].classes
        cap = sum(l.anchors * l.h * l.w for l in yolos) if capacity is None else int(capacity)
        if cap < 1:
            raise ValueError(f"detections: capacity {cap}")
        key = (cap, classes)
        if getattr(self, "_det_key", None) != key:
            self._det_key = key
            self._det = (torch.zeros(B, dtype=torch.int64, device="cuda"),
                         torch.empty(B * cap * 4, device="cuda"),
                         torch.empty(B * cap, device="cuda"),
                         torch.empty(B * cap * max(classes, 1), device="cuda"))
        counts, boxes, obj, probs = self._det
        hip.fill(2 * B, counts.data_ptr(), 0, 0.0, 1)
        for l in yolos:
            hip.yoloDetections(B, l.anchors, classes, l.h, l.w, l.total, l.mask, l.biases,
                               self.net.w, self.net.h, im_w, im_h, thresh, relative, letter,
                               self.out[l.index], cap, counts, boxes, obj, probs)
        if nms is not None:
            hip.nmsSort(B, cap, classes, counts, boxes, obj, probs, nms)
        hip.finish()
        taken = counts.cpu().tolist()
        for b, n in enumerate(taken):
            if n > cap:
                raise TnsError(f"detections: image {b} has {n} taken candidates, capacity {cap}")
        res, self._det_pin = detection_rows_to_host(torch, taken, cap, classes, boxes, obj, probs,
                                                    getattr(self, "_det_pin", None))
        return res

    def load_images(self, images, letter=False, table="fpc"):
        net = self.net
        if len(images) != net.batch:
            raise ValueError(f"{len(images)} images for a batch of {net.batch}")
        if getattr(self, "_input", None) is None:
            self._input = self.torch.empty((net.batch, net.c, net.h, net.w), device="cuda")
        placed = images_to_input(self.hip, self.torch, images, net.c, net.w, net.h, self._input,
                                 letter=letter, table=table)
        return self._input, placed

    def detect_images(self, images, thresh=0.5, nms=None, letter=False, relative=True,
                      table="fpc"):
        x, placed = self.load_images(images, letter=letter, table=table)
        sizes = {(p.w, p.h) for p in placed}
        if len(sizes) > 1 and (letter or not relative):
            raise ValueError("detect_images: images of differing sizes "
                             f"{sorted(sizes)} with letter=True or relative=False: the boxes' "
                             "correction takes one image extent for the whole batch")
        self.forward(x)
        im_w, im_h = (placed[0].w, placed[0].h)
        return self.detections(im_w, im_h, thresh=thresh, relative=relative, letter=letter,
                               nms=nms)


class HipDarknetTrain(_RnnLayers, _LstmLayers):

    LOSS_KINDS = ("softmax", "cost", "logistic")

    def __init__(self, hip, net: Network, params: list[ConvParams], torch, loss_scale: float = 1.0,
                 seed: int = 0, lstm_fused: bool = True, rnn_fused: bool = True,
                 yolo_loss: bool = False):
        self.hip, self.net, self.torch = hip, net, torch
        self.lstm_fused = bool(lstm_fused)
        self.rnn_fused = bool(rnn_fused)
        self.loss_scale = float(loss_scale)
        self.yolo_loss = bool(yolo_loss)
        yolos = [l for l in net.layers if l.kind == "yolo"]
        if self.yolo_loss:
            bad = [f"[net] {k}" for k in net.yolo_unbuilt]
            bad += [f"[yolo] layer {l.index} {k}" for l in yolos for k in l.unbuilt]
            if bad:
                raise ValueError("yolo_loss=True: the device loss does not build "
                                 + ", ".join(bad))
            if len({l.max_boxes for l in yolos}) > 1:
                raise ValueError("yolo_loss=True: the [yolo] layers disagree on max: "
                                 f"{[l.max_boxes for l in yolos]} (one truth tensor feeds all)")
        self.rng = np.random.default_rng(seed)
        B = net.batch
        dev = "cuda"
        t = lambda a: torch.from_numpy(np.ascontiguousarray(a, dtype=np.float32)).to(dev)
        self.out, self.delta = [], []
        for l in net.layers:
            alias = l.kind == "dropout" and l.index > 0
            self.out.append(self.out[-1] if alias else torch.zeros(B * l.out_size, device=dev))
            self.delta.append(self.delta[-1] if alias
                              else torch.zeros(B * l.out_size, device=dev))
        self.rnd = {l.index: torch.zeros(B * l.out_size, device=dev)
                    for l in net.layers if l.kind == "dropout"}
        self.loss = {l.index: torch.zeros(B * l.out_size, device=dev)
                     for l in net.layers if l.kind in ("softmax", "logistic")}
        self.costs = {l.index: torch.zeros(1, device=dev)
                      for l in net.layers if l.kind in self.LOSS_KINDS}
        self.yolo_stats = {}
        if self.yolo_loss:
            for l in yolos:
                self.costs[l.index] = torch.zeros(1, device=dev)
                self.yolo_stats[l.index] = torch.zeros(2 * B, device=dev)
            self.yolo_counters = torch.zeros(2, dtype=torch.int64, device=dev)
# ... 258 lines not shown
```

### tensorium_amd/nnhip.py

```python
from __future__ import annotations

import ctypes as C

import numpy as np

from ._abi import TnsError, check, load

try:
    import torch
except Exception:
    torch = None


CONV_UNFUSED, CONV_FUSED, CONV_IM2COL, CONV_IMPLICIT = 0, 1, 2, 3


def _ptr(x):
    if x is None:
        return None
    if isinstance(x, int):
        return x
    if torch is not None and isinstance(x, torch.Tensor):
        if not x.is_cuda:
            raise TnsError("TNNHip expects device (cuda) tensors")
# ... 171 lines not shown

    def copy(self, N, src, srcOffset, inca, dst, dstOffset, incb):
        check(self.lib.tns_hip_copy(self.ctx, N, _ptr(src), srcOffset, inca, _ptr(dst), dstOffset,
                                    incb))

    def clamp(self, N, alpha, src, dst, stride=1, offset=0):
        check(self.lib.tns_hip_clamp(self.ctx, N, float(alpha), _ptr(src), _ptr(dst), stride,
                                     offset))

    def shortcut(self, N, a, aOffset, b, bOffset, out, outOffset=0, activation=4):
        check(self.lib.tns_hip_shortcut(self.ctx, N, _ptr(a), aOffset, _ptr(b), bOffset, _ptr(out),
                                        outOffset, int(activation)))

    def upSample(self, aBatch, aChannels, outHeight, outWidth, in_, stride, isForward, scale,
                 out, zeroIn=0):
        check(self.lib.tns_hip_upsample(self.ctx, aBatch, aChannels, outHeight, outWidth,
                                        _ptr(in_), stride, int(isForward), float(scale),
                                        _ptr(out), int(zeroIn)))

    def forwardMaxPool(self, aBatch, outC, outH, outW, input, c, h, w, stride_x, stride_y, padding,
                       kernelSize, indexes, output):
        check(self.lib.tns_hip_maxpool_forward(self.ctx, aBatch, outC, outH, outW, _ptr(input), c,
                                               h, w, stride_x, stride_y, padding, kernelSize,
                                               _iptr(indexes), _ptr(output)))

    def backwardMaxPool(self, aBatch, outC, outH, outW, output, indexes, delta, h, w, stride_x,
                        stride_y, padding, kernelSize):
        check(self.lib.tns_hip_maxpool_backward(self.ctx, aBatch, outC, outH, outW, _ptr(output),
                                                _iptr(indexes), _ptr(delta), h, w, stride_x,
                                                stride_y, padding, kernelSize))

    def forwardAvgPool(self, aBatch, outC, outH, outW, input, c, h, w, stride_x, stride_y, padding,
                       kernelSize, output):
        check(self.lib.tns_hip_avgpool_forward(self.ctx, aBatch, outC, outH, outW, _ptr(input), c,
                                               h, w, stride_x, stride_y, padding, kernelSize,
                                               _ptr(output)))

    def backwardAvgPool(self, aBatch, outC, outH, outW, output, delta, h, w, stride_x, stride_y,
                        padding, kernelSize):
        check(self.lib.tns_hip_avgpool_backward(self.ctx, aBatch, outC, outH, outW, _ptr(output),
                                                _ptr(delta), h, w, stride_x, stride_y, padding,
                                                kernelSize))

    def addvv(self, N, src1, src1Offset, inca, src2, src2Offset, incb, dst, dstOffset, incc):
        check(self.lib.tns_hip_addvv(self.ctx, N, _ptr(src1), src1Offset, inca, _ptr(src2),
                                     src2Offset, incb, _ptr(dst), dstOffset, incc))

    def subvv(self, N, src1, src1Offset, inca, src2, src2Offset, incb, dst, dstOffset, incc):
        check(self.lib.tns_hip_subvv(self.ctx, N, _ptr(src1), src1Offset, inca, _ptr(src2),
                                     src2Offset, incb, _ptr(dst), dstOffset, incc))

    def mulvv(self, N, src1, src1Offset, inca, src2, src2Offset, incb, dst, dstOffset, incc):
        check(self.lib.tns_hip_mulvv(self.ctx, N, _ptr(src1), src1Offset, inca, _ptr(src2),
                                     src2Offset, incb, _ptr(dst), dstOffset, incc))

    def fmavv(self, N, src1, src1Offset, inca, src2, src2Offset, incb, src3, src3Offset, incc,
              dst, dstOffset, incd):
        check(self.lib.tns_hip_fmavv(self.ctx, N, _ptr(src1), src1Offset, inca, _ptr(src2),
                                     src2Offset, incb, _ptr(src3), src3Offset, incc, _ptr(dst),
                                     dstOffset, incd))

    def fmavss(self, N, src, offset, scalar, bias, dst):
        check(self.lib.tns_hip_fmavss(self.ctx, N, _ptr(src), offset, float(scalar), float(bias),
                                      _ptr(dst)))

    def inverseSqrt(self, N, alpha, src, dst, stride=1, offset=0):
        check(self.lib.tns_hip_inverse_sqrt(self.ctx, N, float(alpha), _ptr(src), _ptr(dst),
                                            stride, offset))

    def yoloForward(self, batch, anchors, classes, hw, inp, out):
        check(self.lib.tns_hip_yolo_forward(self.ctx, batch, anchors, classes, hw, _ptr(inp),
                                            _ptr(out)))

    def yoloLoss(self, batch, anchors, classes, h, w, total, mask, biases, maxBoxes, netW, netH,
                 ignoreThresh, truthThresh, iouThresh, iouNormalizer, objNormalizer, output, truth,
                 delta, cost, stats=None, counters=None):
        mask = [int(m) for m in mask]
        biases = [float(v) for v in biases]
        if len(mask) != anchors or len(biases) != 2 * total:
            raise TnsError(f"yoloLoss: {len(mask)} mask entries for {anchors} anchors, "
                           f"{len(biases)} biases for total={total}")
        m = (C.c_int64 * max(len(mask), 1))(*mask)
        bs = (C.c_float * max(len(biases), 1))(*biases)
        check(self.lib.tns_hip_yolo_loss(
            self.ctx, batch, anchors, classes, h, w, total, m, bs, maxBoxes, netW, netH,
            float(ignoreThresh), float(truthThresh), float(iouThresh), float(iouNormalizer),
            float(objNormalizer), _ptr(output), _ptr(truth), _ptr(delta), _ptr(cost), _ptr(stats),
            _iptr(counters)))

    def yoloDetections(self, batch, anchors, classes, h, w, total, mask, biases, netW, netH, imW,
                       imH, thresh, relative, letter, output, capacity, counts, boxes,
                       objectness, probs):
        mask = [int(m) for m in mask]
        biases = [float(v) for v in biases]
        if len(mask) != anchors or len(biases) != 2 * total:
            raise TnsError(f"yoloDetections: {len(mask)} mask entries for {anchors} anchors, "
                           f"{len(biases)} biases for total={total}")
        m = (C.c_int64 * max(len(mask), 1))(*mask)
        bs = (C.c_float * max(len(biases), 1))(*biases)
        check(self.lib.tns_hip_yolo_detections(
            self.ctx, batch, anchors, classes, h, w, total, m, bs, netW, netH, imW, imH,
            float(thresh), int(bool(relative)), int(bool(letter)), _ptr(output), capacity,
            _iptr(counts), _ptr(boxes), _ptr(objectness), _ptr(probs)))

    def nmsSort(self, batch, capacity, classes, counts, boxes, objectness, probs, thresh):
        check(self.lib.tns_hip_nms_sort(self.ctx, batch, capacity, classes, _iptr(counts),
                                        _ptr(boxes), _ptr(objectness), _ptr(probs),
                                        float(thresh)))

    IMAGE_TABLES = {"fpc": 0, "255": 1}

    def imageToInput(self, src, geom, channels, netW, netH, dst, letter=False, table="fpc",
                     pixelStride=None):
        count = len(geom)
        g = (C.c_int64 * max(4 * count, 1))(*[int(v) for row in geom for v in row])
        placed = (C.c_int64 * max(4 * count, 1))()
        if src is not None and torch is not None and isinstance(src, torch.Tensor) \
                and src.dtype == torch.uint8:
            if not src.is_cuda or not src.is_contiguous():
                raise TnsError("TNNHip expects contiguous device (cuda) tensors")
            if isinstance(table, str):
                if table not in self.IMAGE_TABLES:
                    raise TnsError(f"imageToInput: table {table!r} (fpc, 255 or 256 floats)")
                kind, tab = self.IMAGE_TABLES[table], None
            else:
                vals = [float(v) for v in table]
                if len(vals) != 256:
                    raise TnsError(f"imageToInput: a table of {len(vals)} entries")
                kind, tab = 2, (C.c_float * 256)(*vals)
            check(self.lib.tns_image_bytes_to_input(
                self.ctx, count, src.data_ptr(), g, channels,
                channels if pixelStride is None else pixelStride, kind, tab, netW, netH,
                int(bool(letter)), _ptr(dst), placed))
        else:
            check(self.lib.tns_image_floats_to_input(
                self.ctx, count, _ptr(src), g, channels, netW, netH, int(bool(letter)), _ptr(dst),
                placed))
        return [tuple(placed[4 * i:4 * i + 4]) for i in range(count)]

    def conv2d(self, batch, C_, H, W, input, weights, filters, kH, kW, wPadding, hPadding,
               xStride, yStride, xDilation, yDilation, workspace, out):
        check(self.lib.tns_hip_conv2d(self.ctx, batch, C_, H, W, _ptr(input), _ptr(weights),
                                      filters, kH, kW, wPadding, hPadding, xStride, yStride,
                                      xDilation, yDilation, _ptr(workspace), _ptr(out)))

    def convForward(self, batch, C_, H, W, input, weights, biases, filters, kSize, stride,
                    padding, dilation, activation, workspace, out, fused=True):
        mode = int(fused) if not isinstance(fused, bool) else (CONV_FUSED if fused else 0)
        check(self.lib.tns_hip_conv_forward(self.ctx, batch, C_, H, W, _ptr(input),
                                            _ptr(weights), _ptr(biases), filters, kSize, stride,
                                            padding, dilation, int(activation), _ptr(workspace),
                                            _ptr(out), mode))

    def convBackward(self, batch, C_, H, W, input, weights, filters, kSize, stride, padding,
                     dilation, activation, output, delta, bias_updates, weight_updates,
                     workspace=None, state_delta=None):
        check(self.lib.tns_hip_conv_backward(
            self.ctx, batch, C_, H, W, _ptr(input), _ptr(weights), filters, kSize, stride,
            padding, dilation, int(activation), _ptr(output), _ptr(delta), _ptr(bias_updates),
            _ptr(weight_updates), _ptr(workspace), _ptr(state_delta)))

    def convForwardTrain(self, batch, C_, H, W, input, weights, filters, kSize, stride, padding,
                         dilation, activation, scales, biases, rolling_mean, rolling_variance,
                         bnMomentum, training, mean, variance, x, x_norm, workspace, out):
        check(self.lib.tns_hip_conv_forward_train(
            self.ctx, batch, C_, H, W, _ptr(input), _ptr(weights), filters, kSize, stride, padding,
            dilation, int(activation), _ptr(scales), _ptr(biases), _ptr(rolling_mean),
            _ptr(rolling_variance), float(bnMomentum), int(bool(training)), _ptr(mean),
            _ptr(variance), _ptr(x), _ptr(x_norm), _ptr(workspace), _ptr(out)))

    def convBackwardBN(self, batch, C_, H, W, input, weights, filters, kSize, stride, padding,
                       dilation, activation, output, delta, scales, x, x_norm, mean, variance,
                       scale_updates, mean_delta, variance_delta, weight_updates, workspace=None,
                       state_delta=None):
        check(self.lib.tns_hip_conv_backward_bn(
            self.ctx, batch, C_, H, W, _ptr(input), _ptr(weights), filters, kSize, stride, padding,
            dilation, int(activation), _ptr(output), _ptr(delta), _ptr(scales), _ptr(x),
            _ptr(x_norm), _ptr(mean), _ptr(variance), _ptr(scale_updates), _ptr(mean_delta),
            _ptr(variance_delta), _ptr(weight_updates), _ptr(workspace), _ptr(state_delta)))

    def setConvVariant(self, variant: int = -1):
        check(self.lib.tns_set_option(1, int(variant)))

    def setConvPad(self, mode: int = -1):
        check(self.lib.tns_set_option(2, int(mode)))

    def setSrssQuirk(self, on: bool = False):
        check(self.lib.tns_set_option(4, 1 if on else 0))

    def setNtSdot(self, on: bool = True):
        check(self.lib.tns_set_option(3, 1 if on else 0))

    def setSdotForm(self, form: int = -1):
        check(self.lib.tns_set_option(6, int(form)))

    def setDxFused(self, mode: int = 1):
        check(self.lib.tns_set_option(7, int(mode)))

    def setDxTile(self, form: int = -1):
        check(self.lib.tns_set_option(8, int(form)))

    def setDwTile(self, form: int = -1):
        check(self.lib.tns_set_option(9, int(form)))

    def setDxConv(self, form: int = -1):
        check(self.lib.tns_set_option(11, int(form)))

    def setDwRes(self, form: int = -1):
        check(self.lib.tns_set_option(12, int(form)))

    def convDwRes(self) -> int:
        return int(self.lib.tns_conv_dw_res_count())

    def convDxConvs(self) -> int:
        return int(self.lib.tns_conv_dx_conv_count())

    def setBwdOverlap(self, mode=True):
        m = int(mode) if not isinstance(mode, bool) else (1 if mode else 0)
        check(self.lib.tns_set_option(10, m))

    def setScratchCap(self, floats: int = 0):
        check(self.lib.tns_set_option(14, int(floats)))

    def setDeriveSums(self, on: bool = False):
        check(self.lib.tns_set_option(13, 1 if on else 0))

    def convDwTiles(self) -> int:
        return int(self.lib.tns_conv_dw_tile_count())

    def convDxTiles(self) -> int:
        return int(self.lib.tns_conv_dx_tile_count())

    def conv1x1Forms(self) -> int:
        return int(self.lib.tns_conv1x1_count())

    def convSlabForms(self) -> int:
        return int(self.lib.tns_conv_slab_count())

    def convTileVariants(self) -> int:
        return int(self.lib.tns_conv_tile_variant_count())

    def sdotChainsVariants(self) -> int:
        return int(self.lib.tns_sdot_chains_variant_count())

    def sdotRcVariants(self) -> int:
        return int(self.lib.tns_sdot_rc_variant_count())

    def setTtExact(self, on: bool = True):
        check(self.lib.tns_set_option(5, 1 if on else 0))

    def meansAndVars(self, srcSize, dstSize, groups, src, offset, means, vars_):
        check(self.lib.tns_hip_means_and_vars(self.ctx, srcSize, dstSize, groups, _ptr(src),
                                              offset, _ptr(means), _ptr(vars_)))

    def means(self, srcSize, dstSize, groups, src, offset, means):
        check(self.lib.tns_hip_means(self.ctx, srcSize, dstSize, groups, _ptr(src), offset,
                                     _ptr(means)))

    def variances(self, srcSize, dstSize, groups, src, offset, means, vars_):
        check(self.lib.tns_hip_variances(self.ctx, srcSize, dstSize, groups, _ptr(src), offset,
                                         _ptr(means), _ptr(vars_)))

    def normalize(self, srcSize, dstSize, groups, means, meansStride, vars_, varsStride, dst,
                  dstOffset):
        check(self.lib.tns_hip_normalize(self.ctx, srcSize, dstSize, groups, _ptr(means),
                                         meansStride, _ptr(vars_), varsStride, _ptr(dst),
                                         dstOffset))

    def forwardScale(self, dstSize, dst, offset, scaleSize, scale, incb, batch):
        check(self.lib.tns_hip_forward_scale(self.ctx, dstSize, _ptr(dst), offset, scaleSize,
                                             _ptr(scale), incb, batch))

    def forwardScaleAdd(self, dstSize, dst, offset, scaleSize, scales, biases, incb, batch):
        check(self.lib.tns_hip_forward_scale_add(self.ctx, dstSize, _ptr(dst), offset, scaleSize,
                                                 _ptr(scales), _ptr(biases), incb, batch))

    def meansAndVarsDelta(self, srcSize, dstSize, groups, delta, x, offset, mean, variance,
                          mean_delta, variance_delta):
        check(self.lib.tns_hip_means_and_vars_delta(
            self.ctx, srcSize, dstSize, groups, _ptr(delta), _ptr(x), offset, _ptr(mean),
            _ptr(variance), _ptr(mean_delta), _ptr(variance_delta)))

    def normalizeDelta(self, deltaSize, meanSize, groups, delta, x, offset, mean, variance,
                       mean_delta, variance_delta):
        check(self.lib.tns_hip_normalize_delta(
            self.ctx, deltaSize, meanSize, groups, _ptr(delta), _ptr(x), offset, _ptr(mean),
            _ptr(variance), _ptr(mean_delta), _ptr(variance_delta)))

    def addDots(self, N, dstSize, groups, src1, src2, srcOffset, dst):
        check(self.lib.tns_hip_add_dots(self.ctx, N, dstSize, groups, _ptr(src1), _ptr(src2),
                                        srcOffset, _ptr(dst)))

    def softmaxBatch(self, N, input, iOffset, batch, batch_size, groups, group_size, stride, temp,
                     output, oOffset):
        check(self.lib.tns_hip_softmax_batch(self.ctx, N, _ptr(input), iOffset, batch,
                                             batch_size, groups, group_size, stride, float(temp),
                                             _ptr(output), oOffset))

    def crossEntropySoftmax(self, N, pred, truth, delta, error):
        check(self.lib.tns_hip_cross_entropy_softmax(self.ctx, N, _ptr(pred), _ptr(truth),
                                                     _ptr(delta), _ptr(error)))

    def forwardDropout(self, N, src, probability, scale, rnd, dst, seed):
        check(self.lib.tns_hip_dropout_forward(self.ctx, N, int(seed), float(probability),
                                               float(scale), _ptr(src), _ptr(rnd), _ptr(dst)))

# ... 61 lines not shown
```

Baseline: 148,400 GFLOP/s.

## Fuse Darknet shortcut residual add into conv forward epilogue

Adds a conv-forward-with-shortcut entry point that adds the residual tensor and applies the shortcut activation inside the conv tile and slab kernel epilogues. Where the chosen kernel form has no residual epilogue, it falls back to a separate shortcut kernel launch. HipDarknet now routes conv layers that feed a shortcut through this path and skips the standalone shortcut layer. The aim is to save one kernel launch and a full read/write pass per residual block, at the cost of extra epilogue register pressure and more template instantiations. The headline SGEMM metric is not touched by any of this.

```diff
diff --git a/include/tns.h b/include/tns.h
--- a/include/tns.h
+++ b/include/tns.h
@@ -304,6 +304,13 @@
                          int64_t dilation, int32_t activation, float* workspace,
                          float* out, int32_t fused);
 
+int tns_conv_forward_shortcut(tns_ctx* ctx, int64_t batch, int64_t C, int64_t H, int64_t W,
+                              const float* input, const float* weights, const float* biases,
+                              int64_t filters, int64_t kSize, int64_t stride, int64_t padding,
+                              int64_t dilation, int32_t activation, float* workspace,
+                              float* out, int32_t fused, const float* residual, float* sum,
+                              int32_t sumActivation);
+
 int tns_hip_conv_forward_train(tns_ctx* ctx, int64_t batch, int64_t C, int64_t H, int64_t W,
                                const float* input, const float* weights, int64_t filters,
                                int64_t kSize, int64_t stride, int64_t padding, int64_t dilation,
diff --git a/tensorium_amd/_abi.py b/tensorium_amd/_abi.py
--- a/tensorium_amd/_abi.py
+++ b/tensorium_amd/_abi.py
@@ -86,6 +86,8 @@
                                  i64, i64, i64, i64, fptr, fptr]),
     "tns_hip_conv_forward": (C.c_int, [vp, i64, i64, i64, i64, fptr, fptr, fptr, i64, i64, i64,
                                        i64, i64, i32, fptr, fptr, i32]),
+    "tns_conv_forward_shortcut": (C.c_int, [vp, i64, i64, i64, i64, fptr, fptr, fptr, i64, i64,
+                                            i64, i64, i64, i32, fptr, fptr, i32, fptr, fptr, i32]),
     "tns_hip_conv_backward": (C.c_int, [vp, i64, i64, i64, i64, fptr, fptr, i64, i64, i64, i64,
                                         i64, i32, fptr, fptr, fptr, fptr, fptr, fptr]),
     "tns_hip_conv_forward_train": (C.c_int, [vp, i64, i64, i64, i64, fptr, fptr, i64, i64, i64,
diff --git a/tensorium_amd/csrc/conv_api.cpp b/tensorium_amd/csrc/conv_api.cpp
--- a/tensorium_amd/csrc/conv_api.cpp
+++ b/tensorium_amd/csrc/conv_api.cpp
@@ -38,7 +38,8 @@
 }
 }
 
-ConvFwdPlan plan_conv_forward(const ConvShape& s, int fused, bool bias_act, const Options& o) {
+namespace {
+ConvFwdPlan plan_fwd_layer(const ConvShape& s, int fused, bool bias_act, const Options& o) {
   ConvFwdPlan p;
   const int64_t batch = s.batch, C = s.C, H = s.H, W = s.W, filters = s.filters, kSize = s.kSize,
                 stride = s.stride, padding = s.padding, dilation = s.dilation;
@@ -136,6 +137,20 @@
   p.form = cvar == 99 ? -1 : (int)cvar;
   if (p.padded && padding > 0) p.stage1_elems = batch * img;
   p.chunk = images_per_launch(img, outImg);
+  return p;
+}
+}
+
+ConvFwdPlan plan_conv_forward(const ConvShape& s, int fused, bool bias_act, const Options& o,
+                              const ConvFwdResidual& r) {
+  ConvFwdPlan p = plan_fwd_layer(s, fused, bias_act, o);
+  if (!r.present) return p;
+  p.sum_act = r.sum_act;
+  const bool has = (p.path == FWD_TILE && s.kSize == 3 && conv_tile_has_res(p.form)) ||
+                   (p.path == FWD_SLAB && conv_slab_has_res(p.form));
+  p.res = has && !p.err && !p.act_tail && !act_transcendental(r.sum_act) ? RES_EPILOGUE : RES_TAIL;
+  if (p.res == RES_TAIL && !r.store_out)
+    p.res_scratch_elems = std::max<int64_t>(0, s.batch * s.filters * p.oh * p.ow);
   return p;
 }
 
@@ -277,6 +292,8 @@
 struct ConvFwdOps {
   const float *input, *weights, *biases;
   float *workspace, *out;
+  const float* residual = nullptr;
+  float* sum = nullptr;
 };
 
 int activate_tail(tns_ctx* c, const ConvFwdPlan& p, const ConvFwdOps& o) {
@@ -296,7 +313,8 @@
   a.alpha = 1.0f; a.beta = 0.0f; a.beta_mode = BETA_ZERO;
   a.A = o.weights; a.lda = k; a.strideA = 0;
   a.B = src + b0 * img; a.ldb = outImg; a.strideB = img;
-  a.C = o.out + b0 * outImg * p.s.filters; a.ldc = outImg; a.strideC = outImg * p.s.filters;
+  a.C = o.out ? o.out + b0 * outImg * p.s.filters : nullptr;
+  a.ldc = outImg; a.strideC = outImg * p.s.filters;
   a.batch = 1; a.epi = p.bias_act ? EPI_BIAS_ACT : EPI_NONE; a.bias = o.biases;
   a.act = p.epi_act;
   a.conv = mode; a.ktab = kt; a.ktab_n = kt ? (int)(k + KTAB_PAD) : 0;
@@ -351,6 +369,9 @@
   sa.K = s.C * s.kSize * s.kSize; sa.ks = s.kSize;
   sa.stride = s.stride; sa.pad = s.padding; sa.dil = s.dilation; sa.ow = p.ow; sa.ohw = p.oh * p.ow;
   sa.act = p.epi_act;
+  if (p.res == RES_EPILOGUE) {
+    sa.residual = o.residual; sa.sum = o.sum; sa.sum_act = p.sum_act;
+  }
   {
     OpTimer t(c, TNS_OP_GEMM);
     const hipError_t e = launch_conv_slab(p.form, sa, slab, c->stream);
@@ -367,7 +388,12 @@
     const GemmArgs a = conv_args(p, o, o.input, s.C * s.H * s.W, s.H, s.W, 2, nullptr, s.padding,
                                  b0, std::min(p.chunk, s.batch - b0));
     OpTimer t(c, TNS_OP_GEMM);
-    const hipError_t e = launch_conv_tile(p.form, a, (int)s.kSize, (int)s.dilation, c->stream);
+    const int64_t off = b0 * p.oh * p.ow * s.filters;
+    const hipError_t e =
+        p.res == RES_EPILOGUE
+            ? launch_conv_tile_res(p.form, a, (int)s.kSize, (int)s.dilation,
+                                   ConvResArgs{o.residual + off, o.sum + off, p.sum_act}, c->stream)
+            : launch_conv_tile(p.form, a, (int)s.kSize, (int)s.dilation, c->stream);
     if (e == hipErrorInvalidValue)
       return set_error(TNS_ERR_UNSUPPORTED, "conv tile %d does not fit this layer", p.form);
     if (int r = hip_status(e, "conv tile launch")) return r;
@@ -429,10 +455,24 @@
   return activate_tail(c, p, o);
 }
 
+int exec_conv_layer(tns_ctx* c, const ConvFwdPlan& p, const ConvFwdOps& o);
+
 int exec_conv_forward(tns_ctx* c, const ConvFwdPlan& p, const ConvFwdOps& o) {
+  if (p.res != RES_TAIL) return exec_conv_layer(c, p, o);
+  ConvFwdOps t = o;
+  if (!t.out && !p.err)
+    if (int r = ensure_scratch(c, SLOT_STAGE2, p.res_scratch_elems, &t.out)) return r;
+  if (int r = exec_conv_layer(c, p, t)) return r;
+  return hip_status(launch_shortcut(p.s.batch * p.s.filters * p.oh * p.ow, t.out, o.residual,
+                                    o.sum, p.sum_act, c->stream),
+                    "shortcut launch");
+}
+
+int exec_conv_layer(tns_ctx* c, const ConvFwdPlan& p, const ConvFwdOps& o) {
   if (p.path == FWD_UNFUSED) return run_fwd_unfused(c, p, o);
   if (p.err && !p.implicit) return set_error(p.err, "%s", p.msg);
-  if (p.implicit && (!o.input || !o.weights || !o.out || (p.bias_act && !o.biases)))
+  if (p.implicit && (!o.input || !o.weights || (!o.out && p.res != RES_EPILOGUE) ||
+                     (p.bias_act && !o.biases)))
     return set_error(TNS_ERR_ARG, "conv_forward: null operand");
   if (p.err) return set_error(p.err, "%s", p.msg);
   switch (p.path) {
@@ -461,6 +501,38 @@
                     aligned16(weights)};
   return exec_conv_forward(c, plan_conv_forward(s, fused, true, g_opt),
                            ConvFwdOps{input, weights, biases, workspace, out});
+}
+
+int tns_conv_forward_shortcut(tns_ctx* c, int64_t batch, int64_t C, int64_t H, int64_t W,
+                              const float* input, const float* weights, const float* biases,
+                              int64_t filters, int64_t kSize, int64_t stride, int64_t padding,
+                              int64_t dilation, int32_t activation, float* workspace, float* out,
+                              int32_t fused, const float* residual, float* sum,
+                              int32_t sumActivation) {
+  if (int r = check_ctx(c)) return r;
+  if (!act_supported(activation) || !act_supported(sumActivation))
+    return set_error(TNS_ERR_UNSUPPORTED, "activation %d not implemented",
+                     act_supported(activation) ? sumActivation : activation);
+  if (!residual || !sum) return set_error(TNS_ERR_ARG, "conv_forward_shortcut: null %s",
+                                          residual ? "sum" : "residual");
+  const ConvShape s{batch, C, H, W, filters, kSize, stride, padding, dilation, activation,
+                    aligned16(weights)};
+  const ConvFwdPlan p =
+      plan_conv_forward(s, fused, true, g_opt, ConvFwdResidual{true, out != nullptr, sumActivation});
+  const int64_t n = std::max<int64_t>(0, batch * filters * p.oh * p.ow);
+  const int64_t k = C * kSize * kSize;
+  const Span so = span(sum, n), sr = span(residual, n), sq = span(out, n);
+  auto meet = [](const Span& a, const Span& b) {
+    return a.lo < a.hi && b.lo < b.hi && a.lo < b.hi && b.lo < a.hi;
+  };
+  if (meet(so, sq) || meet(so, sr) || meet(so, span(input, batch * C * H * W)) ||
+      meet(so, span(weights, filters * k)) || meet(so, span(workspace, batch * k * p.oh * p.ow)) ||
+      meet(sq, sr))
+    return set_error(TNS_ERR_ARG, "conv_forward_shortcut: overlapping operands");
+  ConvFwdOps o{input, weights, biases, workspace, out};
+  o.residual = residual;
+  o.sum = sum;
+  return exec_conv_forward(c, p, o);
 }
 
 int tns_hip_conv_forward_train(tns_ctx* c, int64_t batch, int64_t C, int64_t H, int64_t W,
diff --git a/tensorium_amd/csrc/conv_slab.hip b/tensorium_amd/csrc/conv_slab.hip
--- a/tensorium_amd/csrc/conv_slab.hip
+++ b/tensorium_amd/csrc/conv_slab.hip
@@ -190,8 +190,13 @@
     asm volatile("s_waitcnt vmcnt(0)" ::: "memory");
 }
 
-template <class G>
-__global__ __launch_bounds__(G::NT, 1) void slab_gemm_kernel(SlabGemmArgs p) {
+__device__ __forceinline__ ConvResArgs res_args() { return ConvResArgs{nullptr, nullptr, 4}; }
+__device__ __forceinline__ ConvResArgs res_args(const ConvResArgs& r) { return r; }
+
+template <class G, class... R>
+__global__ __launch_bounds__(G::NT, 1) void slab_gemm_kernel(SlabGemmArgs p, R... res) {
+  constexpr bool RES = sizeof...(R) > 0;
+  static_assert(sizeof...(R) <= 1, "one residual");
   constexpr int BM = G::BM, BN = G::BN, BK = G::BK, NG = G::NG, NS = G::NS;
   constexpr int A_TILE = G::A_TILE, STAGE = G::STAGE, AU = G::AU, DPW = G::DPW;
   __shared__ __attribute__((aligned(16))) float smem[NS * STAGE];
@@ -350,6 +355,38 @@
     }
 
     const int row0 = m0 + wm * 16 + 4 * q;
+    if constexpr (RES) {
+      const ConvResArgs rz = res_args(res...);
+      const bool keep = p.C != nullptr;
+      float rv[JW][4];
+      int64_t off[JW];
+#pragma unroll
+      for (int j = 0; j < JW; ++j) {
+        const int n = n0 + coff * 16 + 16 * j + r16;
+        const int nc = n < N ? n : N - 1;
+        const int img = nc / p.ohw, pix = nc - img * p.ohw;
+        off[j] = ((int64_t)img * p.M + row0) * p.ohw + pix;
+#pragma unroll
+        for (int e = 0; e < 4; ++e)
+          rv[j][e] = n < N ? rz.residual[off[j] + (int64_t)e * p.ohw] : 0.0f;
+      }
+      float bias[4];
+#pragma unroll
+      for (int e = 0; e < 4; ++e) bias[e] = p.fuse ? p.bias[row0 + e] : 0.0f;
+#pragma unroll
+      for (int j = 0; j < JW; ++j) {
+        const int n = n0 + coff * 16 + 16 * j + r16;
+        if (n >= N) continue;
+#pragma unroll
+        for (int e = 0; e < 4; ++e) {
+          float v = acc[j][e];
+          if (p.fuse) v = act_apply_cheap(v + bias[e], p.act);
+          if (keep) p.C[off[j] + (int64_t)e * p.ohw] = v;
+          rz.sum[off[j] + (int64_t)e * p.ohw] = act_apply_cheap(v + rv[j][e], rz.act);
+        }
+      }
+      return;
+    }
     float bias[4];
 #pragma unroll
     for (int e = 0; e < 4; ++e) bias[e] = p.fuse ? p.bias[row0 + e] : 0.0f;
@@ -384,10 +421,11 @@
   const char* name;
 };
 
-template <class G>
-hipError_t launch_slab_gemm(const SlabGemmArgs& a, hipStream_t s) {
+template <class G, class... R>
+hipError_t launch_slab_gemm(const SlabGemmArgs& a, hipStream_t s, R... res) {
   const int64_t blocks = (int64_t)(a.M / G::BM) * ((a.N + G::BN - 1) / G::BN);
-  hipLaunchKernelGGL((slab_gemm_kernel<G>), dim3((unsigned)blocks), dim3(G::NT), 0, s, a);
+  hipLaunchKernelGGL((slab_gemm_kernel<G, R...>), dim3((unsigned)blocks), dim3(G::NT), 0, s, a,
+                     res...);
   return hipGetLastError();
 }
 
@@ -458,8 +496,12 @@
   return (N + bn - 1) / bn * bn * K;
 }
 
+bool conv_slab_has_res(int v) { return v == 3 || v == 4; }
+
 hipError_t launch_conv_slab(int v, const ConvSlabArgs& c, float* slab, hipStream_t s) {
   if (v < 0 || v >= kNumSlab) return hipErrorInvalidValue;
+  if (c.residual && (!conv_slab_has_res(v) || !c.sum)) return hipErrorInvalidValue;
+  if (!c.residual && !c.out) return hipErrorInvalidValue;
   const SlabForm& f = kSlab[v];
   const int64_t N = c.batch * c.ohw;
   if (c.M % f.bm || c.K % f.bk || (c.ks != 1 && c.ks != 3) || N >= (1LL << 22) ||
@@ -483,6 +525,11 @@
   ga.A = c.weights; ga.slab = slab; ga.C = c.out; ga.bias = c.bias;
   ga.M = (int)c.M; ga.N = (int)N; ga.K = (int)c.K; ga.KT = (int)KT;
   ga.tiles_m = (int)(c.M / f.bm); ga.ohw = (int)c.ohw; ga.act = c.act; ga.fuse = c.bias != nullptr;
+  if (c.residual) {
+    const ConvResArgs r{c.residual, c.sum, c.sum_act};
+    return v == 3 ? launch_slab_gemm<SG<32, 176, 64, 2, 4, 3, 3, 2>>(ga, s, r)
+                  : launch_slab_gemm<SG<64, 176, 64, 4, 2, 6, 1, 2>>(ga, s, r);
+  }
   return f.gemm(ga, s);
 }
 
diff --git a/tensorium_amd/csrc/conv_tile.hip b/tensorium_amd/csrc/conv_tile.hip
--- a/tensorium_amd/csrc/conv_tile.hip
+++ b/tensorium_amd/csrc/conv_tile.hip
@@ -321,4 +321,12 @@
   return kTiles[v].fn(a, ks, dil, s);
 }
 
-}
+bool conv_tile_has_res(int v) { return v >= kNumTiles && conv_tile4_has_res(v - kNumTiles); }
+
+hipError_t launch_conv_tile_res(int v, const GemmArgs& a, int ks, int dil, const ConvResArgs& r,
+                                hipStream_t s) {
+  if (!conv_tile_has_res(v)) return hipErrorInvalidValue;
+  return launch_conv_tile4_res(v - kNumTiles, a, ks, dil, r, s);
+}
+
+}
diff --git a/tensorium_amd/csrc/conv_tile4.hip b/tensorium_amd/csrc/conv_tile4.hip
--- a/tensorium_amd/csrc/conv_tile4.hip
+++ b/tensorium_amd/csrc/conv_tile4.hip
@@ -57,8 +57,13 @@
   static constexpr int BST = KI * J;
 };
 
-template <class G, int KS>
-__global__ __launch_bounds__(G::NT) void conv_tile4_kernel(GemmArgs p, int dil) {
+__device__ __forceinline__ ConvResArgs res_args() { return ConvResArgs{nullptr, nullptr, 4}; }
+__device__ __forceinline__ ConvResArgs res_args(const ConvResArgs& r) { return r; }
+
+template <class G, int KS, class... R>
+__global__ __launch_bounds__(G::NT) void conv_tile4_kernel(GemmArgs p, int dil, R... res) {
+  constexpr bool RES = sizeof...(R) > 0;
+  static_assert(sizeof...(R) <= 1 && !(RES && G::DX), "residual: forward forms only");
   constexpr int BM = G::BM, BN = G::BN, BK = G::BK, J = G::J, NG = G::NG;
   constexpr int A_TILE = G::A_TILE, STAGE = G::STAGE, AU = G::AU, KI = G::KI;
   __shared__ __attribute__((aligned(16))) float smem[2 * STAGE];
@@ -493,6 +498,38 @@
     }
     return;
   }
+  if constexpr (RES) {
+    const ConvResArgs rz = res_args(res...);
+    const int64_t row0 = m0 + wm * 16 + 4 * q;
+    const bool keep = p.C != nullptr;
+    float rv[JW][4];
+    int64_t off[JW];
+#pragma unroll
+    for (int j = 0; j < JW; ++j) {
+      const int n = n0 + coff * 16 + 16 * j + r16;
+      const int nc = n < N ? n : N - 1;
+      const int img = nc / p.conv_ohw, pix = nc - img * p.conv_ohw;
+      off[j] = (int64_t)img * p.strideC + pix + row0 * p.ldc;
+#pragma unroll
+      for (int e = 0; e < 4; ++e) rv[j][e] = n < N ? rz.residual[off[j] + e * p.ldc] : 0.0f;
+    }
+    float bias[4];
+#pragma unroll
+    for (int e = 0; e < 4; ++e) bias[e] = fuse ? p.bias[row0 + e] : 0.0f;
+#pragma unroll
+    for (int j = 0; j < JW; ++j) {
+      const int n = n0 + coff * 16 + 16 * j + r16;
+      if (n >= N) continue;
+#pragma unroll
+      for (int e = 0; e < 4; ++e) {
+        float v = acc[j][e];
+        if (fuse) v = act_apply_cheap(v + bias[e], act);
+        if (keep) p.C[off[j] + e * p.ldc] = v;
+        rz.sum[off[j] + e * p.ldc] = act_apply_cheap(v + rv[j][e], rz.act);
+      }
+    }
+    return;
+  }
   const bool add = p.epi == EPI_ADD;
   const int64_t row0 = m0 + wm * 16 + 4 * q;
   float bias[4];
@@ -533,8 +570,8 @@
 unsigned* g_ct4_stamps = nullptr;
 #endif
 
-template <class G>
-hipError_t launch_g4(const GemmArgs& a_in, int ks, int dil, hipStream_t s) {
+template <class G, class... R>
+hipError_t launch_g4(const GemmArgs& a_in, int ks, int dil, hipStream_t s, R... res) {
   GemmArgs a = a_in;
 #ifdef TNS_CT4_STAMPS
   a.stamps = g_ct4_stamps;
@@ -544,6 +581,12 @@
   if (G::TA && (a.lda < a.M || a.K * a.lda > 0x7fffffffLL)) return hipErrorInvalidValue;
   const int64_t tiles = (a.M / G::BM) * ((a.N + G::BN - 1) / G::BN);
   if (tiles > 0x7fffffff || a.N > 0x7fffffff || a.K > 0x7fffffff) return hipErrorInvalidValue;
+  if constexpr (sizeof...(R) > 0) {
+    if (ks != 3) return hipErrorInvalidValue;
+    hipLaunchKernelGGL((conv_tile4_kernel<G, 3, R...>), dim3((unsigned)tiles), dim3(G::NT), 0, s,
+                       a, dil, res...);
+    return hipGetLastError();
+  }
   if (ks == 3)
     hipLaunchKernelGGL((conv_tile4_kernel<G, 3>), dim3((unsigned)tiles), dim3(G::NT), 0, s, a, dil);
   else if (ks == 1)
@@ -859,4 +902,14 @@
   return kTiles4[v].fn(a, ks, dil, s);
 }
 
-}
+bool conv_tile4_has_res(int v) { return v == 3 || v == 8; }
+
+hipError_t launch_conv_tile4_res(int v, const GemmArgs& a, int ks, int dil, const ConvResArgs& r,
+                                 hipStream_t s) {
+  if (!r.residual || !r.sum || a.epi == EPI_ADD) return hipErrorInvalidValue;
+  if (v == 3) return launch_g4<Geo4<128, 176, 8, 1, 64, 1, 0, true, 2, false>>(a, ks, dil, s, r);
+  if (v == 8) return launch_g4<Geo4<64, 96, 4, 1, 32, 0, 0, false, 3, false>>(a, ks, dil, s, r);
+  return hipErrorInvalidValue;
+}
+
+}
diff --git a/tensorium_amd/csrc/tns_internal.hpp b/tensorium_amd/csrc/tns_internal.hpp
--- a/tensorium_amd/csrc/tns_internal.hpp
+++ b/tensorium_amd/csrc/tns_internal.hpp
@@ -88,6 +88,14 @@
 const char* conv_tile_name(int v);
 int conv_tile_pick(const GemmArgs& a, int ks);
 hipError_t launch_conv_tile(int v, const GemmArgs& a, int ks, int dil, hipStream_t s);
+struct ConvResArgs {
+  const float* residual;
+  float* sum;
+  int act;
+};
+bool conv_tile_has_res(int v);
+hipError_t launch_conv_tile_res(int v, const GemmArgs& a, int ks, int dil, const ConvResArgs& r,
+                                hipStream_t s);
 struct ConvSlabArgs {
   const float* input;
   const float* weights;
@@ -95,6 +103,9 @@
   float* out;
   int64_t batch, C, H, W, M, K, ks, stride, pad, dil, ow, ohw;
   int act;
+  const float* residual = nullptr;
+  float* sum = nullptr;
+  int sum_act = 4;
 };
 int conv1x1_count();
 const char* conv1x1_name(int v);
@@ -109,10 +120,14 @@
 int conv_slab_pick(int64_t M, int64_t N, int64_t K, int64_t ks);
 int64_t conv_slab_floats(int v, int64_t N, int64_t K);
 hipError_t launch_conv_slab(int v, const ConvSlabArgs& c, float* slab, hipStream_t s);
+bool conv_slab_has_res(int v);
 int conv_tile4_count();
 const char* conv_tile4_name(int v);
 int conv_tile4_bk(int v);
 hipError_t launch_conv_tile4(int v, const GemmArgs& a, int ks, int dil, hipStream_t s);
+bool conv_tile4_has_res(int v);
+hipError_t launch_conv_tile4_res(int v, const GemmArgs& a, int ks, int dil, const ConvResArgs& r,
+                                 hipStream_t s);
 int conv_tile4_ta_count();
 const char* conv_tile4_ta_name(int v);
 int conv_tile4_dx_pick(int64_t M, int64_t N, int64_t K, int64_t ks);
@@ -382,6 +397,7 @@
   FWD_TILE,
   FWD_IMPLICIT
 };
+enum ConvResPlace { RES_NONE = 0, RES_EPILOGUE, RES_TAIL };
 struct ConvFwdPlan {
   int err = 0;
   char msg[kPlanMsg] = {};
@@ -399,8 +415,17 @@
   int64_t col_elems = 0, stage1_elems = 0;
   int64_t conv_variant = -1;
   int srss_quirk = 0;
-};
-ConvFwdPlan plan_conv_forward(const ConvShape& s, int fused, bool bias_act, const Options& o);
+  int res = RES_NONE;
+  int sum_act = 4;
+  int64_t res_scratch_elems = 0;
+};
+struct ConvFwdResidual {
+  bool present = false;
+  bool store_out = true;
+  int32_t sum_act = 4;
+};
+ConvFwdPlan plan_conv_forward(const ConvShape& s, int fused, bool bias_act, const Options& o,
+                              const ConvFwdResidual& r = ConvFwdResidual{});
 
 enum ConvDwPath { DW_RES = 0, DW_TILE, DW_SDOT, DW_GEMM };
 struct ConvDwChoice {
diff --git a/tensorium_amd/darknet.py b/tensorium_amd/darknet.py
--- a/tensorium_amd/darknet.py
+++ b/tensorium_amd/darknet.py
@@ -1051,17 +1051,32 @@
 class HipDarknet(_RnnLayers, _LstmLayers):
 
     def __init__(self, hip, net: Network, params: list[ConvParams], torch,
-                 lstm_fused: bool = True, rnn_fused: bool = True):
+                 lstm_fused: bool = True, rnn_fused: bool = True, fuse_shortcut: bool = True,
+                 drop_unread: bool = False):
         self.hip, self.net, self.torch = hip, net, torch
         self.lstm_fused = bool(lstm_fused)
         self.rnn_fused = bool(rnn_fused)
         B = net.batch
         dev = "cuda"
         t = lambda a: torch.from_numpy(np.ascontiguousarray(a, dtype=np.float32)).to(dev)
+        self.fused_shortcut = {}
+        if fuse_shortcut:
+            for l in net.layers[1:]:
+                before = net.layers[l.index - 1]
+                if (l.kind == "shortcut" and before.kind == "convolutional"
+                        and l.inputs[0] != before.index):
+                    self.fused_shortcut[before.index] = l
+        read = {len(net.layers) - 1}
+        for l in net.layers:
+            if l.index and l.kind != "route" and l.index - 1 not in self.fused_shortcut:
+                read.add(l.index - 1)
+            read.update(l.inputs)
+        self.dropped = {i for i in self.fused_shortcut if i not in read} if drop_unread else set()
         self.out = []
         for l in net.layers:
             alias = l.kind == "dropout" and l.index > 0
-            self.out.append(self.out[-1] if alias else torch.empty(B * l.out_size, device=dev))
+            self.out.append(self.out[-1] if alias else None if l.index in self.dropped
+                            else torch.empty(B * l.out_size, device=dev))
         self.conv_params, self.fc_params = {}, {}
         blocks = list(zip(net.param_layers(), params))
         kind = lambda b: net.layers[b[0].index].kind if b[0].gate else ""
@@ -1084,10 +1099,18 @@
         prev = x
         for l in self.net.layers:
             out = self.out[l.index]
-            if l.kind == "convolutional":
+            sc = self.fused_shortcut.get(l.index)
+            if l.kind == "convolutional" and sc is not None:
+                w, b = self.conv_params[l.index]
+                hip.convForwardShortcut(B, l.c, l.h, l.w, prev, w, b, l.filters, l.size, l.stride,
+                                        l.pad, 1, l.activation, None, out, self.out[sc.inputs[0]],
+                                        self.out[sc.index], sc.activation, fused=True)
+            elif l.kind == "convolutional":
                 w, b = self.conv_params[l.index]
                 hip.convForward(B, l.c, l.h, l.w, prev, w, b, l.filters, l.size, l.stride, l.pad,
                                 1, l.activation, None, out, fused=True)
+            elif l.kind == "shortcut" and l.index - 1 in self.fused_shortcut:
+                pass
             elif l.kind == "shortcut":
                 src = self.out[l.inputs[0]]
                 hip.shortcut(B * l.out_size, prev, 0, src, 0, out, 0, l.activation)
diff --git a/tensorium_amd/nnhip.py b/tensorium_amd/nnhip.py
--- a/tensorium_amd/nnhip.py
+++ b/tensorium_amd/nnhip.py
@@ -347,6 +347,15 @@
                                             padding, dilation, int(activation), _ptr(workspace),
                                             _ptr(out), mode))
 
+    def convForwardShortcut(self, batch, C_, H, W, input, weights, biases, filters, kSize, stride,
+                            padding, dilation, activation, workspace, out, residual, sum,
+                            sumActivation=4, fused=True):
+        mode = int(fused) if not isinstance(fused, bool) else (CONV_FUSED if fused else 0)
+        check(self.lib.tns_conv_forward_shortcut(
+            self.ctx, batch, C_, H, W, _ptr(input), _ptr(weights), _ptr(biases), filters, kSize,
+            stride, padding, dilation, int(activation), _ptr(workspace), _ptr(out), mode,
+            _ptr(residual), _ptr(sum), int(sumActivation)))
+
     def convBackward(self, batch, C_, H, W, input, weights, filters, kSize, stride, padding,
                      dilation, activation, output, delta, bias_updates, weight_updates,
                      workspace=None, state_delta=None):
```

Result: no change. 148,400 GFLOP/s, median of 2 (-0.0%).
